# homopolymer/RAMBL

Measured on AMD Instinct MI355X. Metric: reads/sec into POA (150bp, ~1.5k-node graph), higher is better.
Workload: dtype f64

## Files before the change

rambl_amd/capi.py:

```python
import ctypes as C
import os

_HERE = os.path.dirname(os.path.abspath(__file__))
LIB_PATH = os.path.join(_HERE, "libstraincall_hip.so")

SC_OK = 0
ERRORS = {-1: "SC_ERR_NO_DEVICE", -2: "SC_ERR_HIP", -3: "SC_ERR_ARG", -4: "SC_ERR_UNSUPPORTED",
          -5: "SC_ERR_CAPACITY", -6: "SC_ERR_INTERNAL"}


class ScParams(C.Structure):
    _fields_ = [("error_rate", C.c_float), ("tau", C.c_float), ("diff_rate", C.c_float),
                ("sweeps_cap", C.c_int), ("draw_budget", C.c_int), ("max_candidates", C.c_int),
                ("graph_only", C.c_int), ("want_trace", C.c_int), ("want_timing", C.c_int), ("want_graph", C.c_int)]


class ScStats(C.Structure):
    _fields_ = [("graph_ms", C.c_double), ("cluster_ms", C.c_double), ("sampler_kernel_ms", C.c_double),
                ("sampler_launches", C.c_long), ("sampler_read_copies", C.c_long), ("level_launches", C.c_long), ("draws", C.c_long),
                ("slow_draws", C.c_long), ("exact_draws", C.c_long), ("sampler_strains", C.c_long), ("chain_passes", C.c_long), ("chain_cycles", C.c_long), ("chain_wall_ticks", C.c_long), ("level_kernel_ticks", C.c_long), ("sampler_level_ticks", C.c_long), ("xcd_levels", C.c_long * 8), ("msa_calls", C.c_long), ("n_nodes", C.c_int), ("n_levels", C.c_int),
                ("n_unique_reads", C.c_int), ("n_read_copies", C.c_long), ("setup_ms", C.c_double), ("queue_ms", C.c_double), ("place_ms", C.c_double), ("mailbox_ms", C.c_double), ("host_us", C.c_double * 3), ("wake_us", C.c_double * 2), ("kind_levels", C.c_long * 17)]

    def as_dict(self):
        return {k: (list(getattr(self, k)) if k in ("xcd_levels", "kind_levels", "host_us", "wake_us") else getattr(self, k)) for k, _ in self._fields_}


class ScAlignStats(C.Structure):
    _fields_ = [("upload_ms", C.c_double), ("score_ms", C.c_double), ("trace_ms", C.c_double), ("total_ms", C.c_double),
                ("score_cells", C.c_long), ("trace_cells", C.c_long), ("n_traced", C.c_long)]

    def as_dict(self):
        return {k: getattr(self, k) for k, _ in self._fields_}


class ScProfileStats(C.Structure):
    _fields_ = [("upload_ms", C.c_double), ("score_ms", C.c_double), ("trace_ms", C.c_double), ("total_ms", C.c_double),
                ("score_cells", C.c_long), ("trace_cells", C.c_long), ("n_tiles", C.c_long), ("n_candidates", C.c_long),
                ("n_traced", C.c_long), ("n_hits", C.c_long)]

    def as_dict(self):
        return {k: getattr(self, k) for k, _ in self._fields_}


class ScProfileSeedStats(C.Structure):
    _fields_ = ScProfileStats._fields_ + [("seed_k", C.c_int), ("n_gene_kmers", C.c_long), ("n_pairs", C.c_long),
                                          ("index_ms", C.c_double), ("lookup_ms", C.c_double)]

    def as_dict(self):
        return {k: getattr(self, k) for k, _ in self._fields_}


class ScProfileCountStats(C.Structure):
    _fields_ = ScProfileSeedStats._fields_ + [("n_rounds", C.c_int), ("n_stretches", C.c_int), ("n_reads_counted", C.c_long),
                                              ("select_ms", C.c_double), ("count_ms", C.c_double)]

    def as_dict(self):
        return {k: getattr(self, k) for k, _ in self._fields_}


class ScTaxaStats(C.Structure):
    _fields_ = [("upload_ms", C.c_double), ("words_ms", C.c_double), ("table_ms", C.c_double), ("score_ms", C.c_double), ("total_ms", C.c_double),
                ("n_seqs", C.c_long), ("n_words", C.c_long), ("n_genera", C.c_long), ("table_bytes", C.c_long)]

    def as_dict(self):
        return {k: getattr(self, k) for k, _ in self._fields_}


class StrainCallError(RuntimeError):
    def __init__(self, code, msg=""):
        super().__init__("%s (%d)%s" % (ERRORS.get(code, "error"), code, (": " + msg) if msg else ""))
        self.code = code


def load_library():
    if not os.path.exists(LIB_PATH):
        raise ImportError("%s is missing: build it with `python -c 'import __graft_entry__ as g; g.build()'` "
                          "(hipcc --offload-arch=gfx950). There is no CPU fallback for the StrainCall path." % LIB_PATH)
    lib = C.CDLL(LIB_PATH)
    vp, ip, cp = C.c_void_p, C.POINTER(C.c_int), C.c_char_p
    lib.sc_ctx_create.argtypes = [C.c_int, C.c_int, C.POINTER(vp)]
    lib.sc_ctx_destroy.argtypes = [vp]
    lib.sc_ctx_destroy.restype = None
    lib.sc_last_error.argtypes = [vp]
    lib.sc_last_error.restype = cp
    lib.sc_roi_error.argtypes = [vp, C.c_int]
    lib.sc_roi_error.restype = cp
    lib.sc_host_plan.argtypes = [C.c_int, C.c_int, C.c_double, ip]
    lib.sc_host_plan.restype = C.c_int
    lib.sc_host_bind.argtypes = [C.c_int]
    lib.sc_host_bind.restype = C.c_int
    lib.sc_roi_submit.argtypes = [vp, cp, C.c_int, ip, cp, ip, cp, ip, ip, ip, ip, C.c_int, C.POINTER(ScParams), ip]
    lib.sc_roi_wait.argtypes = [vp, C.c_int]
    lib.sc_roi_result.argtypes = [vp, C.c_int, C.c_char_p, C.c_long, ip, C.POINTER(C.c_double), C.c_int, ip]
    lib.sc_roi_graph_dump.argtypes = [vp, C.c_int, C.c_char_p, C.c_long, C.POINTER(C.c_long)]
    lib.sc_roi_trace.argtypes = [vp, C.c_int, C.c_char_p, C.c_long, C.POINTER(C.c_long)]
    lib.sc_roi_stats.argtypes = [vp, C.c_int, C.POINTER(ScStats)]
    lib.sc_roi_release.argtypes = [vp, C.c_int]
    lib.sc_roi_edge_support.argtypes = [vp, C.c_int, ip, C.c_int, ip]
    lib.sc_msa_align.argtypes = [vp, cp, ip, C.c_int, C.c_char_p, C.c_long, ip]
    lib.sc_roi_thread_tables.argtypes = [vp, C.c_int, ip, ip, C.c_int, ip, C.c_long, C.c_char_p, ip, C.POINTER(C.c_long)]
    lib.sc_roi_thread_edges.argtypes = [vp, C.c_int, ip, ip, ip, C.c_int, ip]
    lib.sc_edge_support_tables.argtypes = [vp, C.c_int, ip, ip, ip, C.POINTER(C.c_ubyte), C.c_int, ip, ip, C.c_int, ip]
    dp, up = C.POINTER(C.c_double), C.POINTER(C.c_uint)
    lib.sc_sample_level.argtypes = [vp, C.c_int, dp, C.c_int, dp, C.POINTER(C.c_ubyte), C.c_int, C.c_int, ip, ip, ip, ip, ip,
                                    C.c_int, dp, C.c_int, up, up, C.POINTER(C.c_long)]
    pi, pc, pu = C.POINTER(ip), C.POINTER(C.c_char_p), C.POINTER(C.c_ubyte)
    lib.sc_aln_open.argtypes = [cp, C.POINTER(vp)]
    lib.sc_aln_open_filtered.argtypes = [cp, C.POINTER(C.c_char_p), C.c_int, C.POINTER(vp)]
    lib.sc_aln_open_filtered.restype = C.c_int
    lib.sc_aln_close.argtypes = [vp]
    lib.sc_aln_close.restype = None
    lib.sc_aln_error.argtypes = [vp]
    lib.sc_aln_error.restype = cp
    lib.sc_aln_records.argtypes = [vp]
    lib.sc_aln_records.restype = C.c_long
    lib.sc_aln_ref_stats.argtypes = [vp, cp, C.POINTER(C.c_long), C.POINTER(C.c_long)]
    lib.sc_aln_ref_stats.restype = C.c_int
    lib.sc_aln_pileup_flags.argtypes = [vp, cp, C.c_int, C.c_int, C.c_int, pu, pu, pu]
    lib.sc_aln_load_reads.argtypes = [vp, cp, C.c_int, C.c_int, C.c_int, C.c_int, C.c_int, C.c_int, C.POINTER(vp)]
    lib.sc_reads_get.argtypes = [vp, ip, pi, pc, pi, pc, pi, pi, pi, pi, C.POINTER(C.c_long), ip]
    lib.sc_reads_free.argtypes = [vp]
    lib.sc_reads_free.restype = None
    lib.sc_aln_walk.argtypes = [vp, C.c_long, C.c_long, C.c_char_p, C.c_long, C.POINTER(C.c_long), C.POINTER(C.c_long)]
    lp = C.POINTER(C.c_long)
    lib.sc_align_reads.argtypes = [C.c_int, cp, lp, C.c_int, cp, cp, lp, C.c_int, ip, ip, ip, ip, ip, ip, up, C.c_int, ip,
                                   C.POINTER(ScAlignStats)]
    lib.sc_align_error.argtypes = []
    lib.sc_align_error.restype = cp
    lib.sc_profile_hits.argtypes = [C.c_int, cp, lp, C.c_int, cp, lp, C.c_int, C.c_double, C.c_double, C.c_double, C.c_double, ip, ip, ip,
                                    dp, ip, ip, ip, ip, ip, ip, dp, C.c_long, lp, C.POINTER(ScProfileStats)]
    lib.sc_profile_error.argtypes = []
    lib.sc_profile_error.restype = cp
    lib.sc_profile_hits_seeded.argtypes = lib.sc_profile_hits.argtypes[:-1] + [C.POINTER(ScProfileSeedStats)]
    lib.sc_profile_seed_length.argtypes = [ip, C.c_int, C.c_long, C.c_double, C.c_double, C.c_double, C.c_double, ip]
    lib.sc_profile_counts.argtypes = [C.c_int, cp, lp, C.c_int, cp, lp, C.c_int, ip, C.c_int, C.c_double, C.c_double, C.c_double, C.c_double,
                                      C.c_int, C.c_long, ip, ip, ip, lp, C.c_long, lp, C.POINTER(ScProfileCountStats)]
    lib.sc_profile_evalue6.argtypes = [C.c_int, C.c_long, C.c_int, C.c_double, C.c_double]
    lib.sc_profile_evalue6.restype = C.c_double
    u64, u64p = C.c_ulonglong, C.POINTER(C.c_ulonglong)
    lib.sc_taxa_train.argtypes = [C.c_int, cp, lp, C.c_int, ip, C.c_int, C.c_int, C.c_int, C.POINTER(vp), C.POINTER(ScTaxaStats)]
    lib.sc_taxa_classify.argtypes = [vp, cp, lp, C.c_int, u64p, u64, C.c_int, C.c_int, ip, ip, ip, C.POINTER(ScTaxaStats)]
    lib.sc_taxa_model_counts.argtypes = [vp, C.c_int, up, up]
    lib.sc_taxa_model_table.argtypes = [vp, C.c_int, ip]
    lib.sc_taxa_free.argtypes = [vp]
    lib.sc_taxa_free.restype = None
    lib.sc_taxa_error.argtypes = []
    lib.sc_taxa_error.restype = cp
    lib.sc_taxa_draw.argtypes = [u64, u64, C.c_int, C.c_int, C.c_int]
    lib.sc_taxa_draw.restype = C.c_long
    for f in ("sc_taxa_train", "sc_taxa_classify", "sc_taxa_model_counts", "sc_taxa_model_table"):
        getattr(lib, f).restype = C.c_int
    for f in ("sc_aln_open", "sc_aln_pileup_flags", "sc_aln_load_reads", "sc_reads_get", "sc_aln_walk", "sc_align_reads", "sc_profile_hits",
              "sc_profile_hits_seeded", "sc_profile_seed_length", "sc_profile_counts"):
        getattr(lib, f).restype = C.c_int
    for f in ("sc_ctx_create", "sc_roi_submit", "sc_roi_wait", "sc_roi_result", "sc_roi_graph_dump", "sc_roi_trace",
              "sc_roi_stats", "sc_roi_release", "sc_roi_edge_support", "sc_msa_align", "sc_roi_thread_tables", "sc_sample_level", "sc_roi_thread_edges", "sc_edge_support_tables"):
        getattr(lib, f).restype = C.c_int
    return lib


EXPORTS = ["sc_ctx_create", "sc_ctx_destroy", "sc_last_error", "sc_roi_error", "sc_host_plan", "sc_host_bind", "sc_roi_submit", "sc_roi_wait", "sc_roi_result",
           "sc_roi_graph_dump", "sc_roi_trace", "sc_roi_stats", "sc_roi_release", "sc_roi_edge_support", "sc_msa_align",
           "sc_roi_thread_tables", "sc_roi_thread_edges", "sc_edge_support_tables", "sc_sample_level", "sc_aln_open", "sc_aln_open_filtered", "sc_aln_close", "sc_aln_error", "sc_aln_records", "sc_aln_ref_stats", "sc_aln_pileup_flags",
           "sc_aln_load_reads", "sc_reads_get", "sc_reads_free", "sc_depth_scan", "sc_depth_scan_runs", "sc_aln_walk", "sc_align_reads",
           "sc_align_error", "sc_profile_hits", "sc_profile_error", "sc_profile_hits_seeded", "sc_profile_seed_length",
           "sc_profile_counts", "sc_taxa_train", "sc_taxa_classify", "sc_taxa_model_counts", "sc_taxa_model_table", "sc_taxa_free", "sc_taxa_error",
           "sc_taxa_draw"]


def default_params(error_rate=0.01, tau=0.02, diff_rate=0.01, graph_only=False, want_trace=False, want_timing=False, want_graph=False):
    return ScParams(error_rate, tau, diff_rate, 5000, 40000, 80, int(graph_only), int(want_trace), int(want_timing), int(want_graph))


def _pack(strings):
    off = (C.c_int * (len(strings) + 1))()
    n = 0
    for i, s in enumerate(strings):
        off[i] = n
        n += len(s)
    off[len(strings)] = n
    return "".join(strings).encode("ascii"), off


def host_bind(device=0):
    return int(lib().sc_host_bind(int(device)))


def host_plan(streams, local_world=0, cpus=0.0):
    out = (C.c_int * 3)()
    rc = lib().sc_host_plan(streams, local_world, cpus, out)
    if rc != SC_OK:
        raise StrainCallError(rc)
    return tuple(out)


_LIB = None


def lib():
    global _LIB
    if _LIB is None:
        _LIB = load_library()
    return _LIB


class NativeReads:

    def __init__(self, handle, gene_seq):
        self._h = handle
        self.gene_seq = gene_seq
        n, depth, n_in = C.c_int(), C.c_int(), C.c_long()
        ip = C.POINTER(C.c_int)
        self._pos, self._cig_off, self._seq_off, self._cn, self._mate_idx, self._mate_off = ip(), ip(), ip(), ip(), ip(), ip()
        self._cig, self._seq = C.c_char_p(), C.c_char_p()
        rc = lib().sc_reads_get(handle, C.byref(n), C.byref(self._pos), C.byref(self._cig), C.byref(self._cig_off), C.byref(self._seq),
                                C.byref(self._seq_off), C.byref(self._cn), C.byref(self._mate_idx), C.byref(self._mate_off),
                                C.byref(n_in), C.byref(depth))
        if rc != SC_OK:
            raise StrainCallError(rc)
        self.n = n.value
        self.n_input = n_in.value
        self.depth = depth.value

    def __len__(self):
        return self.n

    def __del__(self):
        if getattr(self, "_h", None):
            try:
                lib().sc_reads_free(self._h)
            except TypeError:
                pass
            self._h = None

    def _texts(self, text, off):
        raw = C.string_at(text, off[self.n]) if self.n else b""
        return [raw[off[i]:off[i + 1]].decode("ascii") for i in range(self.n)]

    def _view(self, name, build):
        cache = self.__dict__.setdefault("_views", {})
        if name not in cache:
            cache[name] = build()
        return cache[name]

    @property
    def pos(self):
        return self._view("pos", lambda: [self._pos[i] for i in range(self.n)])

    @property
    def copies(self):
        return self._view("copies", lambda: [self._cn[i] for i in range(self.n)])

    @property
    def cigar(self):
        return self._view("cigar", lambda: self._texts(self._cig, self._cig_off))

    @property
    def seq(self):
        return self._view("seq", lambda: self._texts(self._seq, self._seq_off))

    @property
    def mates(self):
        return self._view("mates", lambda: [[self._mate_idx[k] for k in range(self._mate_off[i], self._mate_off[i + 1])] for i in range(self.n)])


class NativeAln:

    def __init__(self, path, only=None):
        self.path = path
        self._h = C.c_void_p()
        if only is None:
            rc = lib().sc_aln_open(path.encode(), C.byref(self._h))
        else:
            names = (C.c_char_p * max(len(only), 1))(*[n.encode() for n in only])
            rc = lib().sc_aln_open_filtered(path.encode(), names, len(only), C.byref(self._h))
        if rc != SC_OK:
            msg = lib().sc_aln_error(self._h).decode() if self._h else "cannot open"
            self.close()
            raise StrainCallError(rc, "%s: %s" % (path, msg))

    def close(self):
        if getattr(self, "_h", None):
            try:
                lib().sc_aln_close(self._h)
            except TypeError:
                pass
            self._h = C.c_void_p()

    def __del__(self):
        self.close()

    def records(self):
        return lib().sc_aln_records(self._h)

    def walk(self, chunk=1 << 24):
        buf = C.create_string_buffer(chunk)
        first, n_out, used = 0, C.c_long(), C.c_long()
        while True:
            rc = lib().sc_aln_walk(self._h, first, 1 << 20, buf, len(buf), C.byref(n_out), C.byref(used))
            if rc == -5:
                buf = C.create_string_buffer(len(buf) * 4)
                continue
            if rc != SC_OK:
                raise StrainCallError(rc, self.path)
            if n_out.value == 0:
                return
            for line in buf.raw[:used.value].split(b"\n")[:-1]:
                q, f, seq, qual = line.split(b"\t")
                yield q, int(f), seq, qual
            first += n_out.value

    def ref_stats(self, gene):
        n, b = C.c_long(), C.c_long()
        lib().sc_aln_ref_stats(self._h, gene.encode(), C.byref(n), C.byref(b))
        return n.value, b.value

    def pileup_flags(self, mq, gene, P, Q):
        import numpy as np
        n = Q - P + 1
        if n <= 0:
            return {}
        cov, ins, dele = (np.zeros(n, dtype=np.uint8) for _ in range(3))
        pu = C.POINTER(C.c_ubyte)
        rc = lib().sc_aln_pileup_flags(self._h, gene.encode(), P, Q, mq, cov.ctypes.data_as(pu), ins.ctypes.data_as(pu),
                                       dele.ctypes.data_as(pu))
        if rc != SC_OK:
            raise StrainCallError(rc)
        idx = np.nonzero(cov)[0]
        return {int(k) + P: (bool(ins[k]), bool(dele[k])) for k in idx}

    def load_reads(self, gene_seq, gene, p0, p1, mq, rl, max_ins, max_depth):
        h = C.c_void_p()
        rc = lib().sc_aln_load_reads(self._h, gene.encode(), p0, p1, mq, rl, max_ins, max_depth, C.byref(h))
        if rc != SC_OK:
            raise StrainCallError(rc, lib().sc_aln_error(self._h).decode())
        return NativeReads(h, gene_seq)


class RegionResult:
    def __init__(self, seqs, abundance, graph, trace, stats):
        self.seqs = seqs
        self.abundance = abundance
        self.graph = graph
        self.trace = trace
        self.stats = stats


class Context:

    def __init__(self, device=0, streams=1):
        self.lib = load_library()
        self.h = C.c_void_p()
        rc = self.lib.sc_ctx_create(device, streams, C.byref(self.h))
        if rc != SC_OK:
            raise StrainCallError(rc, "no gfx950 HIP device %d (the StrainCall path has no CPU fallback)" % device)

    def close(self):
        if self.h:
            self.lib.sc_ctx_destroy(self.h)
            self.h = C.c_void_p()

    def __enter__(self):
        return self

    def __exit__(self, *a):
        self.close()

    def _err(self, rc):
        msg = self.lib.sc_last_error(self.h)
        return StrainCallError(rc, msg.decode("utf-8", "replace") if msg else "")

    def submit(self, region, params):
        n = len(region)
        if isinstance(region, NativeReads):
            ref = region.gene_seq.encode("ascii")
            handle = C.c_int()
            rc = self.lib.sc_roi_submit(self.h, ref, len(ref), region._pos, region._cig, region._cig_off, region._seq, region._seq_off,
                                        region._cn, region._mate_idx, region._mate_off, n, C.byref(params), C.byref(handle))
            if rc != SC_OK:
                raise self._err(rc)
            return handle.value
        pos = (C.c_int * max(n, 1))(*region.pos)
        cn = (C.c_int * max(n, 1))(*region.copies)
        cig, cig_off = _pack(region.cigar)
        seq, seq_off = _pack(region.seq)
        mate_off = (C.c_int * (n + 1))()
        flat = []
        for i, m in enumerate(region.mates):
            mate_off[i] = len(flat)
            flat.extend(m)
        mate_off[n] = len(flat)
        mate_idx = (C.c_int * max(len(flat), 1))(*flat)
        ref = region.gene_seq.encode("ascii")
        handle = C.c_int()
        rc = self.lib.sc_roi_submit(self.h, ref, len(ref), pos, cig, cig_off, seq, seq_off, cn, mate_idx, mate_off, n,
                                    C.byref(params), C.byref(handle))
        if rc != SC_OK:
            raise self._err(rc)
        return handle.value

    def wait(self, handle, want_graph=False, want_trace=False, release=True):
        rc = self.lib.sc_roi_wait(self.h, handle)
        graph = trace = None
        stats = ScStats()
        self.lib.sc_roi_stats(self.h, handle, C.byref(stats))
        if want_graph or rc != SC_OK:
            ln = C.c_long()
            self.lib.sc_roi_graph_dump(self.h, handle, None, 0, C.byref(ln))
            buf = C.create_string_buffer(ln.value + 1)
            if self.lib.sc_roi_graph_dump(self.h, handle, buf, ln.value, C.byref(ln)) == SC_OK:
                graph = buf.raw[:ln.value].decode("ascii")
        if rc != SC_OK:
            msg = self.lib.sc_roi_error(self.h, handle)
            err = StrainCallError(rc, msg.decode("utf-8", "replace") if msg else "")
            if release:
                self.lib.sc_roi_release(self.h, handle)
            err.graph = graph
            raise err
        nst = C.c_int()
        cap, maxs = 1 << 16, 256
        while True:
            buf = C.create_string_buffer(cap)
            off = (C.c_int * (maxs + 1))()
            ab = (C.c_double * maxs)()
            rc = self.lib.sc_roi_result(self.h, handle, buf, cap, off, ab, maxs, C.byref(nst))
            if rc == -5 and cap < (1 << 30):
                cap *= 8
                maxs *= 4
                continue
            break
        if rc != SC_OK:
            raise self._err(rc)
        seqs = [buf.raw[off[i]:off[i + 1]].decode("ascii") for i in range(nst.value)]
        abundance = [ab[i] for i in range(nst.value)]
        if want_trace:
            ln = C.c_long()
            self.lib.sc_roi_trace(self.h, handle, None, 0, C.byref(ln))
            tb = C.create_string_buffer(ln.value + 1)
            if self.lib.sc_roi_trace(self.h, handle, tb, ln.value, C.byref(ln)) == SC_OK:
                trace = tb.raw[:ln.value].decode("ascii")
        if release:
            self.lib.sc_roi_release(self.h, handle)
        return RegionResult(seqs, abundance, graph, trace, stats.as_dict())

    def run(self, region, params, want_graph=False, want_trace=False):
        return self.wait(self.submit(region, params), want_graph, want_trace)

    def edge_support(self, handle):
        n = C.c_int()
        self.lib.sc_roi_edge_support(self.h, handle, None, 0, C.byref(n))
        arr = (C.c_int * max(n.value, 1))()
        rc = self.lib.sc_roi_edge_support(self.h, handle, arr, n.value, C.byref(n))
        if rc != SC_OK:
            raise self._err(rc)
        return list(arr[:n.value])

    def thread_tables(self, handle):
        ncls, npool = C.c_int(), C.c_long()
        self.lib.sc_roi_thread_tables(self.h, handle, None, None, 0, None, 0, None, C.byref(ncls), C.byref(npool))
        cnt = (C.c_int * max(ncls.value, 1))()
        first = (C.c_int * max(ncls.value, 1))()
        pool = (C.c_int * max(npool.value, 1))()
        sym = C.create_string_buffer(8)
        rc = self.lib.sc_roi_thread_tables(self.h, handle, cnt, first, ncls.value, pool, npool.value, sym, C.byref(ncls),
                                           C.byref(npool))
        if rc != SC_OK:
            raise self._err(rc)
        return list(cnt[:ncls.value]), list(first[:ncls.value]), list(pool[:npool.value]), sym.raw

    def thread_edges(self, handle):
        ncls = C.c_int()
        self.lib.sc_roi_thread_edges(self.h, handle, None, None, None, 0, C.byref(ncls))
        n = ncls.value
        smin, emin, tmin = (C.c_int * max(n, 1))(), (C.c_int * max(n, 1))(), (C.c_int * max(8 * n, 1))()
        rc = self.lib.sc_roi_thread_edges(self.h, handle, smin, emin, tmin, n, C.byref(ncls))
        if rc != SC_OK:
            raise self._err(rc)
        return list(smin[:n]), list(emin[:n]), list(tmin[:8 * n])

    def edge_support_tables(self, pool_ptr, pool_rid, pool_cn, node_is_end, edge_src, edge_dst, sorted_pools):
        import numpy as np
        ptr_, rid, cn, src, dst = (np.ascontiguousarray(x, dtype=np.int32) for x in (pool_ptr, pool_rid, pool_cn, edge_src, edge_dst))
        end = np.ascontiguousarray(node_is_end, dtype=np.uint8)
        assert rid.shape == cn.shape and src.shape == dst.shape and ptr_.size == end.size + 1
        out = np.zeros(max(src.size, 1), dtype=np.int32)

        def ptr(x):
            return x.ctypes.data_as(C.POINTER(C.c_ubyte if x.dtype == np.uint8 else C.c_int))
        rc = self.lib.sc_edge_support_tables(self.h, end.size, ptr(ptr_), ptr(rid), ptr(cn), ptr(end), src.size, ptr(src), ptr(dst),
                                             int(sorted_pools), ptr(out))
        if rc != SC_OK:
            raise self._err(rc)
        return out[:src.size].tolist()

    def sample_level(self, a0, ll, has, ent_rid, ent_cn, ent_sym, mates, n_sweeps, U, e0=1):
        import numpy as np
        a0 = np.ascontiguousarray(a0, dtype=np.float64)
        ll = np.ascontiguousarray(ll, dtype=np.float64)
        S, n_reads = ll.shape
        assert a0.shape == (S,)
        has = np.ascontiguousarray(has, dtype=np.uint8)
        assert has.shape == (n_reads,)
        ent = [np.ascontiguousarray(x, dtype=np.int32) for x in (ent_rid, ent_cn, ent_sym)]
        assert ent[0].shape == ent[1].shape == ent[2].shape
        mate_off = np.zeros(n_reads + 1, dtype=np.int32)
        mate_off[1:] = np.cumsum([len(mates[r]) if r < len(mates) else 0 for r in range(n_reads)])
        mate_idx = np.array([m for r in range(min(len(mates), n_reads)) for m in mates[r]] or [0], dtype=np.int32)
        U = np.ascontiguousarray(U, dtype=np.float64)
        kdraw = np.zeros(S, dtype=np.uint32)
        cnt = np.zeros((S, 16), dtype=np.uint32)
        out = (C.c_long * 5)()

        def ptr(x, t):
            return x.ctypes.data_as(C.POINTER(t))
        rc = self.lib.sc_sample_level(self.h, S, ptr(a0, C.c_double), n_reads, ptr(ll, C.c_double), ptr(has, C.c_ubyte),
                                      len(ent[0]), e0, ptr(ent[0], C.c_int), ptr(ent[1], C.c_int), ptr(ent[2], C.c_int),
                                      ptr(mate_off, C.c_int), ptr(mate_idx, C.c_int), n_sweeps, ptr(U, C.c_double), len(U),
                                      ptr(kdraw, C.c_uint), ptr(cnt, C.c_uint), out)
        if rc != SC_OK:
            raise self._err(rc)
        return dict(kdraw=kdraw, cnt=cnt, n_draws=out[0], n_slow=out[1], n_exact=out[2], n_pass=out[3], kind=out[4])

    def msa_align(self, seqs):
        txt, off = _pack(seqs)
        cap = (len(txt) + 2) * max(len(seqs), 1) + 16
        out = C.create_string_buffer(cap)
        ncol = C.c_int()
        rc = self.lib.sc_msa_align(self.h, txt, off, len(seqs), out, cap, C.byref(ncol))
        if rc != SC_OK:
            raise self._err(rc)
        w = ncol.value + 1
        return [out.raw[i * w:i * w + ncol.value].decode("ascii") for i in range(len(seqs))]


class AlignResult:

    def __init__(self, as_, xs, seed, strand, pos, nm, cigar, stats):
        self.as_, self.xs, self.seed, self.strand, self.pos, self.nm, self.cigar, self.stats = as_, xs, seed, strand, pos, nm, cigar, stats


def align_reads(seeds, reads, quals=None, device=0):
    import numpy as np
    n = len(reads)
    sl = np.array([0] + [len(x) for x in seeds], dtype=np.int64).cumsum()
    rl = np.array([0] + [len(x) for x in reads], dtype=np.int64).cumsum()
    qtext = None
    if quals is not None:
        qtext = b"".join(q if (q != b"*" and len(q) == len(r)) else b"I" * len(r) for r, q in zip(reads, quals))
    stride = max([len(x) for x in reads] + [0]) // 2 + 4
    as_, xs, seed, strand, pos, nm, ncig = (np.zeros(max(n, 1), dtype=np.int32) for _ in range(7))
    cig = np.zeros(max(n, 1) * stride, dtype=np.uint32)
    st = ScAlignStats()
    ip, lp, up = C.POINTER(C.c_int), C.POINTER(C.c_long), C.POINTER(C.c_uint)
    rc = lib().sc_align_reads(device, b"".join(seeds), sl.ctypes.data_as(lp), len(seeds), b"".join(reads), qtext, rl.ctypes.data_as(lp), n,
                              as_.ctypes.data_as(ip), xs.ctypes.data_as(ip), seed.ctypes.data_as(ip), strand.ctypes.data_as(ip),
                              pos.ctypes.data_as(ip), nm.ctypes.data_as(ip), cig.ctypes.data_as(up), stride, ncig.ctypes.data_as(ip),
                              C.byref(st))
    if rc != SC_OK:
        raise StrainCallError(rc, lib().sc_align_error().decode())
    cigars = []
    for r in range(n):
        ops = cig[r * stride:r * stride + ncig[r]]
        cigars.append("".join("%d%s" % (int(v) >> 4, "MIDNSHP=X"[int(v) & 15]) for v in ops) if ncig[r] else "*")
    return AlignResult(as_[:n], xs[:n], seed[:n], strand[:n], pos[:n], nm[:n], cigars, st)


class ProfileHits:
    FIELDS = ("seg", "gene", "strand", "score", "identity", "align_len", "qfrom", "qto", "hfrom", "hto", "evalue")

    def __init__(self, arrays, stats):
        for k, v in zip(self.FIELDS, arrays):
            setattr(self, k, v)
        self.stats = stats

    def __len__(self):
        return len(self.seg)


def _profile_call(gtext, gl, n_genes, segs, thresholds, device, cap, seeded=False):
    import numpy as np
    n = len(segs)
    sl = np.array([0] + [len(x) for x in segs], dtype=np.int64).cumsum()
    stext = b"".join(segs)
    ip, lp, dp = C.POINTER(C.c_int), C.POINTER(C.c_long), C.POINTER(C.c_double)
    while True:
        ints = [np.zeros(max(cap, 1), dtype=np.int32) for _ in range(9)]
        score, ev = np.zeros(max(cap, 1), dtype=np.float64), np.zeros(max(cap, 1), dtype=np.float64)
        st, nh = (ScProfileSeedStats if seeded else ScProfileStats)(), C.c_long()
        iptr = [a.ctypes.data_as(ip) for a in ints]
        rc = (lib().sc_profile_hits_seeded if seeded else lib().sc_profile_hits)(device, gtext, gl.ctypes.data_as(lp), n_genes, stext, sl.ctypes.data_as(lp), n, *thresholds, iptr[0],
                                   iptr[1], iptr[2], score.ctypes.data_as(dp), iptr[3], iptr[4], iptr[5], iptr[6], iptr[7], iptr[8],
                                   ev.ctypes.data_as(dp), cap, C.byref(nh), C.byref(st))
        if rc == -5 and nh.value > cap:
            cap = nh.value
            continue
        if rc != SC_OK:
            raise StrainCallError(rc, lib().sc_profile_error().decode())
        k = nh.value
        seg, gene, strand, identity, align_len, qfrom, qto, hfrom, hto = (a[:k] for a in ints)
        return [seg, gene, strand, score[:k], identity, align_len, qfrom, qto, hfrom, hto, ev[:k]], st


def profile_seed_length(seg_lens, gene_bases, min_identity=95.0, max_evalue=1e-10, ka_lambda=1.28, ka_k=0.46, lossless=False):
    import numpy as np
    lens = np.ascontiguousarray(seg_lens, dtype=np.int32)
    raw = C.c_int()
    k = lib().sc_profile_seed_length(lens.ctypes.data_as(C.POINTER(C.c_int)), len(lens), int(gene_bases), float(min_identity), float(max_evalue),
                                     float(ka_lambda), float(ka_k), C.byref(raw))
    if k < 0:
        raise StrainCallError(k)
    return (raw.value or None) if lossless else k


def profile_hits(genes, segs, min_identity=95.0, max_evalue=1e-10, ka_lambda=1.28, ka_k=0.46, device=0, cap=None, seeded=False):
    import numpy as np
    gl = np.array([0] + [len(x) for x in genes], dtype=np.int64).cumsum()
    gtext = b"".join(genes)
    thresholds = (float(min_identity), float(max_evalue), float(ka_lambda), float(ka_k))
    step = max(1, (1 << 30) // (2 * max(len(genes), 1)))
    parts, total, seed_ks = [], (ScProfileSeedStats if seeded else ScProfileStats)(), []
    for a in range(0, max(len(segs), 1), step):
        chunk = segs[a:a + step]
        arrays, st = _profile_call(gtext, gl, len(genes), chunk, thresholds, device, max(1 << 16, 4 * len(chunk)) if cap is None else int(cap),
                                   seeded)
        arrays[0] = arrays[0] + a
        parts.append(arrays)
        for k, _ in total._fields_:
            setattr(total, k, getattr(total, k) + getattr(st, k))
        if seeded:
            seed_ks.append(st.seed_k)
    if seeded:
        total.seed_k = min(seed_ks)
    return ProfileHits([np.concatenate([p[f] for p in parts]) for f in range(11)], total)


class ProfileCounts:

    def __init__(self, triples, stats):
        self.triples = triples
        self.stats = stats

    def __len__(self):
        return len(self.triples)


def profile_evalue6(seg_len, gene_bases, score2, ka_lambda=1.28, ka_k=0.46):
    return float(lib().sc_profile_evalue6(int(seg_len), int(gene_bases), int(score2), float(ka_lambda), float(ka_k)))


def profile_counts(genes, segs, seg_read, min_identity=95.0, max_evalue=1e-10, ka_lambda=1.28, ka_k=0.46, device=0, cap=None, seeded=False,
                   cand_room=0):
    import numpy as np
    gl = np.array([0] + [len(x) for x in genes], dtype=np.int64).cumsum()
    sl = np.array([0] + [len(x) for x in segs], dtype=np.int64).cumsum()
    gtext, stext = b"".join(genes), b"".join(segs)
    reads = np.ascontiguousarray(seg_read, dtype=np.int32)
    if len(reads) != len(segs):
        raise ValueError("%d read indices for %d segments" % (len(reads), len(segs)))
    n_reads = int(reads.max()) + 1 if len(reads) else 0
    ip, lp = C.POINTER(C.c_int), C.POINTER(C.c_long)
    cap = 1 << 16 if cap is None else int(cap)
    while True:
        gene, times, share = (np.zeros(max(cap, 1), dtype=np.int32) for _ in range(3))
        n_behind = np.zeros(max(cap, 1), dtype=np.int64)
        st, n = ScProfileCountStats(), C.c_long()
        rc = lib().sc_profile_counts(device, gtext, gl.ctypes.data_as(lp), len(genes), stext, sl.ctypes.data_as(lp), len(segs),
                                     reads.ctypes.data_as(ip), n_reads, float(min_identity), float(max_evalue), float(ka_lambda), float(ka_k),
                                     int(bool(seeded)), int(cand_room), gene.ctypes.data_as(ip), times.ctypes.data_as(ip),
                                     share.ctypes.data_as(ip), n_behind.ctypes.data_as(lp), cap, C.byref(n), C.byref(st))
        if rc == -5 and n.value > cap:
            cap = n.value
            continue
        if rc != SC_OK:
            raise StrainCallError(rc, lib().sc_profile_error().decode())
        k = n.value
        return ProfileCounts([(int(gene[i]), int(times[i]), int(share[i]), int(n_behind[i])) for i in range(k)], st)


TAXA_WORDS = 65536
TAXA_TRIALS = 100


def taxa_draw(seed, key, trial, draw, n_words):
    return int(lib().sc_taxa_draw(int(seed), int(key), int(trial), int(draw), int(n_words)))


def _pack_long(seqs):
    import numpy as np
    return b"".join(seqs), np.array([0] + [len(x) for x in seqs], dtype=np.int64).cumsum()


class TaxaModel:

    def __init__(self, seqs, genus, n_genera, device=0, grid_cap=0, keep_counts=False):
        import numpy as np
        if len(genus) != len(seqs):
            raise ValueError("%d genus indices for %d sequences" % (len(genus), len(seqs)))
        text, off = _pack_long(seqs)
        gi = np.ascontiguousarray(genus, dtype=np.int32)
        self.n_genera = int(n_genera)
        self._h = C.c_void_p()
        self.stats = ScTaxaStats()
        rc = lib().sc_taxa_train(int(device), text, off.ctypes.data_as(C.POINTER(C.c_long)), len(seqs), gi.ctypes.data_as(C.POINTER(C.c_int)),
                                 self.n_genera, int(grid_cap), int(bool(keep_counts)), C.byref(self._h), C.byref(self.stats))
        if rc != SC_OK:
            raise StrainCallError(rc, lib().sc_taxa_error().decode())

    def close(self):
        if getattr(self, "_h", None):
            try:
                lib().sc_taxa_free(self._h)
            except TypeError:
                pass
            self._h = C.c_void_p()

    def __del__(self):
        self.close()

    def __enter__(self):
        return self

    def __exit__(self, *a):
        self.close()

    def classify(self, queries, keys, seed=0, n_trials=TAXA_TRIALS, grid_cap=0):
        import numpy as np
        n = len(queries)
        if len(keys) != n:
            raise ValueError("%d keys for %d queries" % (len(keys), n))
        text, off = _pack_long(queries)
        key = np.ascontiguousarray(keys, dtype=np.uint64)
        best, words = np.zeros(max(n, 1), dtype=np.int32), np.zeros(max(n, 1), dtype=np.int32)
        winner = np.zeros((max(n, 1), max(int(n_trials), 1)), dtype=np.int32)
        st = ScTaxaStats()
        ip = C.POINTER(C.c_int)
        rc = lib().sc_taxa_classify(self._h, text, off.ctypes.data_as(C.POINTER(C.c_long)), n, key.ctypes.data_as(C.POINTER(C.c_ulonglong)),
                                    int(seed), int(n_trials), int(grid_cap), best.ctypes.data_as(ip), winner.ctypes.data_as(ip),
                                    words.ctypes.data_as(ip), C.byref(st))
        if rc != SC_OK:
            raise StrainCallError(rc, lib().sc_taxa_error().decode())
        return best[:n], winner[:n], words[:n], st

    def counts(self, genus):
        import numpy as np
        m, n = np.zeros(TAXA_WORDS, dtype=np.uint32), np.zeros(TAXA_WORDS, dtype=np.uint32)
        up = C.POINTER(C.c_uint)
        rc = lib().sc_taxa_model_counts(self._h, int(genus), m.ctypes.data_as(up), n.ctypes.data_as(up))
        if rc != SC_OK:
            raise StrainCallError(rc, lib().sc_taxa_error().decode())
        return m, n

    def table(self, genus):
        import numpy as np
        q = np.zeros(TAXA_WORDS, dtype=np.int32)
        rc = lib().sc_taxa_model_table(self._h, int(genus), q.ctypes.data_as(C.POINTER(C.c_int)))
        if rc != SC_OK:
            raise StrainCallError(rc, lib().sc_taxa_error().decode())
        return q
```

rambl_amd/csrc/sc_api.cpp:

```cpp
#include <malloc.h>

#include <cmath>

#include "sc_ctx.hpp"

using namespace sc;
struct sc_ctx { Ctx c; sc_ctx(int device, const CtxPlan& plan) : c(device, plan) {} };

extern "C" {

int sc_host_plan(int stream_count, int local_world, double cpus, int* out) {
    if (!out || stream_count < 1) return SC_ERR_ARG;
    host_plan(stream_count, local_world > 0 ? local_world : local_world_size(), cpus > 0 ? cpus : cpu_budget_host(), out);
    return SC_OK;
}

int sc_ctx_create(int device, int stream_count, sc_ctx** out) {
    if (!out) return SC_ERR_ARG;
    *out = nullptr;
    setenv("GPU_MAX_HW_QUEUES", "16", 0);
    int ndev = 0;
    if (hipGetDeviceCount(&ndev) != hipSuccess || ndev <= 0 || device < 0 || device >= ndev) return SC_ERR_NO_DEVICE;
    hipDeviceProp_t prop;
    if (hipGetDeviceProperties(&prop, device) != hipSuccess) return SC_ERR_NO_DEVICE;
    if (std::strncmp(prop.gcnArchName, "gfx950", 6) != 0) return SC_ERR_NO_DEVICE;
    if (hipSetDevice(device) != hipSuccess) return SC_ERR_HIP;
    if (init_kernels() != 0) return SC_ERR_HIP;
    const Options opt = read_options();
    struct Near {
        cpu_set_t before; bool moved = false;
        Near(int dev, bool bind) {
            cpu_set_t local;
            if (bind && sched_getaffinity(0, sizeof before, &before) == 0 && sc::gpu_local_cpus(dev, &local)) moved = sched_setaffinity(0, sizeof local, &local) == 0;
        }
        ~Near() { if (moved) (void)sched_setaffinity(0, sizeof before, &before); }
    } near{device, !opt.off(opt.numa_bind)};
    {
        static std::once_flag once;
        std::call_once(once, [&opt] {
            if (opt.off(opt.malloc_tune)) return;
            mallopt(M_MMAP_THRESHOLD, 32 << 20);
            mallopt(M_TRIM_THRESHOLD, 1 << 30);
            mallopt(M_TOP_PAD, 64 << 20);
        });
    }
    try {
        *out = new sc_ctx(device, plan_context(opt, stream_count, prop.multiProcessorCount, cpu_budget_host(), local_world_size()));
    } catch (const std::exception&) {
        return SC_ERR_HIP;
    }
    return SC_OK;
}

void sc_ctx_destroy(sc_ctx* h) { delete h; }

const char* sc_last_error(sc_ctx* h) {
    if (!h) return "";
    std::lock_guard<std::mutex> lk(h->c.mu);
    static thread_local std::string copy;
    copy = h->c.last_error;
    return copy.c_str();
}

const char* sc_roi_error(sc_ctx* h, int handle) {
    if (!h) return "";
    std::lock_guard<std::mutex> lk(h->c.mu);
    auto it = h->c.jobs.find(handle);
    return (it == h->c.jobs.end() || it->second->status != 1) ? "" : it->second->err.c_str();
}

int sc_roi_submit(sc_ctx* h, const char* ref_bases, int ref_len, const int* read_pos, const char* cigar_text,
                  const int* cigar_off, const char* seq_text, const int* seq_off, const int* read_copies,
                  const int* mate_idx, const int* mate_off, int n_reads, const sc_params* params, int* handle_out) {
    if (!h || !ref_bases || ref_len < 0 || n_reads < 0 || !params || !handle_out) return SC_ERR_ARG;
    if (n_reads > 0 && (!read_pos || !cigar_text || !cigar_off || !seq_text || !seq_off || !read_copies || !mate_off)) return SC_ERR_ARG;
    if (params->draw_budget < 1 || params->draw_budget > MAX_DRAWS || params->sweeps_cap < 0 || params->max_candidates < 1 ||
        params->max_candidates > MAXS)
        return SC_ERR_ARG;
    if (n_reads > 0 && (cigar_off[0] < 0 || seq_off[0] < 0 || mate_off[0] != 0)) return SC_ERR_ARG;
    for (int i = 0; i < n_reads; i++)
        if (read_copies[i] < 1 || cigar_off[i + 1] < cigar_off[i] || seq_off[i + 1] < seq_off[i] || mate_off[i + 1] < mate_off[i])
            return SC_ERR_ARG;
    auto job = std::make_shared<Job>();
    job->t_submit = now_ms();
    job->ref.assign(ref_bases, (size_t)ref_len);
    job->reads.resize((size_t)n_reads);
    for (int i = 0; i < n_reads; i++) {
        if (read_pos[i] < 0 || read_pos[i] > ref_len) return SC_ERR_ARG;
        job->reads[i].pos = read_pos[i];
        job->reads[i].cigar.assign(cigar_text + cigar_off[i], (size_t)(cigar_off[i + 1] - cigar_off[i]));
        job->reads[i].seq.assign(seq_text + seq_off[i], (size_t)(seq_off[i + 1] - seq_off[i]));
        job->reads[i].cn = read_copies[i];
    }
    job->mate_off.assign(mate_off ? mate_off : nullptr, mate_off ? mate_off + n_reads + 1 : nullptr);
    if (job->mate_off.empty()) job->mate_off.assign(1, 0);
    const int nm = job->mate_off.back();
    if (nm > 0 && !mate_idx) return SC_ERR_ARG;
    job->mate_idx.assign(mate_idx, mate_idx + nm);
    for (int v : job->mate_idx) if (v < -1 || v >= n_reads) return SC_ERR_ARG;
    job->params = *params;
    Ctx* ctx = &h->c;
    Worker* wake = nullptr;
    {
        std::lock_guard<std::mutex> lk(ctx->mu);
        job->handle = ctx->next_handle++;
        ctx->jobs[job->handle] = job;
        ctx->queue.push_back(job);
        ctx->regions_active.fetch_add(1, std::memory_order_acq_rel);
        *handle_out = job->handle;
        if (!ctx->idle.empty()) { wake = ctx->idle.back(); ctx->idle.pop_back(); }
    }
    if (wake) ctx->pool->make_ready(wake->fib);
    return SC_OK;
}

static std::shared_ptr<Job> find_job(sc_ctx* h, int handle) {
    std::lock_guard<std::mutex> lk(h->c.mu);
    auto it = h->c.jobs.find(handle);
    return it == h->c.jobs.end() ? nullptr : it->second;
}

int sc_roi_wait(sc_ctx* h, int handle) {
    if (!h) return SC_ERR_ARG;
    auto job = find_job(h, handle);
    if (!job) return SC_ERR_ARG;
    std::unique_lock<std::mutex> lk(h->c.mu);
    h->c.cv_done.wait(lk, [&] { return job->status == 1; });
    if (job->rc != SC_OK) h->c.last_error = job->err;
    return job->rc;
}

int sc_roi_result(sc_ctx* h, int handle, char* seq_buf, long seq_cap, int* seq_off, double* abundance, int max_strains,
                  int* n_strains) {
    if (!h || !n_strains) return SC_ERR_ARG;
    auto job = find_job(h, handle);
    if (!job || job->status != 1) return SC_ERR_ARG;
    if (job->rc != SC_OK) return job->rc;
    const int n = (int)job->seqs.size();
    *n_strains = n;
    long tot = 0;
    for (auto& s : job->seqs) tot += (long)s.size();
    if (n > max_strains || tot > seq_cap || !seq_buf || !seq_off || !abundance) return SC_ERR_CAPACITY;
    long o = 0;
    for (int i = 0; i < n; i++) {
        seq_off[i] = (int)o;
        std::memcpy(seq_buf + o, job->seqs[i].data(), job->seqs[i].size());
        o += (long)job->seqs[i].size();
        abundance[i] = job->abund[i];
    }
    seq_off[n] = (int)o;
    return SC_OK;
}

static int copy_text(const std::string& s, char* buf, long cap, long* len_out) {
    if (len_out) *len_out = (long)s.size();
    if (!buf || cap < (long)s.size()) return SC_ERR_CAPACITY;
    std::memcpy(buf, s.data(), s.size());
    return SC_OK;
}
int sc_roi_graph_dump(sc_ctx* h, int handle, char* buf, long cap, long* len_out) {
    if (!h) return SC_ERR_ARG;
    auto job = find_job(h, handle);
    if (!job || job->status != 1) return SC_ERR_ARG;
    if (job->rc != SC_OK && job->graph_dump.empty()) return job->rc;
    return copy_text(job->graph_dump, buf, cap, len_out);
}
int sc_roi_trace(sc_ctx* h, int handle, char* buf, long cap, long* len_out) {
    if (!h) return SC_ERR_ARG;
    auto job = find_job(h, handle);
    if (!job || job->status != 1) return SC_ERR_ARG;
    if (job->rc != SC_OK) return job->rc;
    return copy_text(job->trace, buf, cap, len_out);
}
int sc_roi_stats(sc_ctx* h, int handle, sc_stats* out) {
    if (!h || !out) return SC_ERR_ARG;
    auto job = find_job(h, handle);
    if (!job || job->status != 1) return SC_ERR_ARG;
    *out = job->stats;
    return SC_OK;
}
int sc_roi_edge_support(sc_ctx* h, int handle, int* support, int cap, int* n_edges) {
    if (!h || !n_edges) return SC_ERR_ARG;
    auto job = find_job(h, handle);
    if (!job || job->status != 1) return SC_ERR_ARG;
    if (job->rc != SC_OK) return job->rc;
    *n_edges = (int)job->edge_support.size();
    if (!support || cap < *n_edges) return SC_ERR_CAPACITY;
    std::memcpy(support, job->edge_support.data(), sizeof(int) * job->edge_support.size());
    return SC_OK;
}
int sc_roi_thread_tables(sc_ctx* h, int handle, int* count, int* first_read, int cls_cap, int* pool, long pool_cap,
                         char* symbols, int* n_cls, long* n_pool) {
    if (!h || !n_cls || !n_pool) return SC_ERR_ARG;
    auto job = find_job(h, handle);
    if (!job || job->status != 1) return SC_ERR_ARG;
    *n_cls = (int)job->thr_count.size();
    *n_pool = (long)job->thr_pool.size();
    if (!count || !first_read || !pool || !symbols || cls_cap < *n_cls || pool_cap < *n_pool) return SC_ERR_CAPACITY;
    std::memcpy(count, job->thr_count.data(), sizeof(int) * job->thr_count.size());
    std::memcpy(first_read, job->thr_first.data(), sizeof(int) * job->thr_first.size());
    std::memcpy(pool, job->thr_pool.data(), sizeof(int) * job->thr_pool.size());
    std::memset(symbols, 0, 8);
    std::memcpy(symbols, job->thr_sym.data(), std::min<size_t>(8, job->thr_sym.size()));
    return SC_OK;
}
int sc_roi_thread_edges(sc_ctx* h, int handle, int* smin, int* emin, int* tmin, int cls_cap, int* n_cls) {
    if (!h || !n_cls) return SC_ERR_ARG;
    auto job = find_job(h, handle);
    if (!job || job->status != 1) return SC_ERR_ARG;
    *n_cls = (int)job->thr_smin.size();
    if (!smin || !emin || !tmin || cls_cap < *n_cls) return SC_ERR_CAPACITY;
    std::memcpy(smin, job->thr_smin.data(), sizeof(int) * job->thr_smin.size());
    std::memcpy(emin, job->thr_emin.data(), sizeof(int) * job->thr_emin.size());
    std::memcpy(tmin, job->thr_tmin.data(), sizeof(int) * job->thr_tmin.size());
    return SC_OK;
}
int sc_edge_support_tables(sc_ctx* h, int n_nodes, const int* pool_ptr, const int* pool_rid, const int* pool_cn,
                           const unsigned char* node_is_end, int n_edges, const int* edge_src, const int* edge_dst, int sorted,
                           int* support_out) {
    if (!h || n_nodes < 1 || n_edges < 0 || !pool_ptr || !node_is_end || (sorted != 0 && sorted != 1)) return SC_ERR_ARG;
    if (n_edges > 0 && (!edge_src || !edge_dst || !support_out)) return SC_ERR_ARG;
    if (pool_ptr[0] != 0) return SC_ERR_ARG;
    for (int a = 0; a < n_nodes; a++) if (pool_ptr[a + 1] < pool_ptr[a]) return SC_ERR_ARG;
    const int np = pool_ptr[n_nodes];
    if (np > 0 && (!pool_rid || !pool_cn)) return SC_ERR_ARG;
    for (int e = 0; e < n_edges; e++)
        if (edge_src[e] < 0 || edge_src[e] >= n_nodes || edge_dst[e] < 0 || edge_dst[e] >= n_nodes) return SC_ERR_ARG;
    if (sorted)
        for (int a = 0; a < n_nodes; a++)
            for (int x = pool_ptr[a] + 1; x < pool_ptr[a + 1]; x++) if (pool_rid[x] < pool_rid[x - 1]) return SC_ERR_ARG;
    if (n_edges == 0) return SC_OK;
    Ctx* ctx = &h->c;
    try {
        Worker w;
        w.init_private(ctx);
        const hipStream_t st = w.st;
        const std::vector<int> pptr(pool_ptr, pool_ptr + n_nodes + 1), prid(pool_rid, pool_rid + np), pcn(pool_cn, pool_cn + np);
        const std::vector<int> esrc(edge_src, edge_src + n_edges), edst(edge_dst, edge_dst + n_edges);
        const std::vector<uint8_t> isend(node_is_end, node_is_end + n_nodes);
        DevBuf b_ptr, b_rid, b_cn, b_end, b_src, b_dst, b_sup;
        const int* d_ptr = upload(w.passthrough, b_ptr, pptr, st);
        const int* d_rid = upload(w.passthrough, b_rid, prid, st);
        const int* d_cn = upload(w.passthrough, b_cn, pcn, st);
        const uint8_t* d_end = upload(w.passthrough, b_end, isend, st);
        const int* d_src = upload(w.passthrough, b_src, esrc, st);
        const int* d_dst = upload(w.passthrough, b_dst, edst, st);
        int* d_sup = (int*)b_sup.ensure(sizeof(int) * (size_t)n_edges);
        launch_edge_support(st, nullptr, d_dst, d_ptr, d_rid, d_cn, d_end, d_src, n_edges, sorted, d_sup);
        HIPCHK(hipGetLastError());
        HIPCHK(hipMemcpyAsync(support_out, d_sup, sizeof(int) * (size_t)n_edges, hipMemcpyDeviceToHost, st));
        HIPCHK(hipStreamSynchronize(st));
        return SC_OK;
    } catch (const ScError& ex) { std::lock_guard<std::mutex> lk(ctx->mu); ctx->last_error = ex.what(); return ex.code; }
    catch (const std::exception& ex) { std::lock_guard<std::mutex> lk(ctx->mu); ctx->last_error = ex.what(); return SC_ERR_HIP; }
}
int sc_sample_level(sc_ctx* h, int S, const double* a0, int n_reads, const double* ll, const unsigned char* has, int n_ent,
                    int e0, const int* ent_rid, const int* ent_cn, const int* ent_sym, const int* mate_off, const int* mate_idx,
                    int n_sweeps, const double* U, int n_u, unsigned* kdraw, unsigned* cnt, long* out) {
    if (!h || !a0 || !ll || !has || !ent_rid || !ent_cn || !ent_sym || !mate_off || !U || !kdraw || !cnt || !out) return SC_ERR_ARG;
    Ctx* ctx = &h->c;
    if (ctx->resident || ctx->workers.size() != 1) return SC_ERR_ARG;
    if (S < 2 || S > MAXS || n_reads < 1 || n_ent < 1 || e0 < 0 || e0 > (1 << 20) || n_sweeps < 1) return SC_ERR_ARG;
    for (int s = 0; s < S; s++) if (!(a0[s] >= 0.0) || !std::isfinite(a0[s])) return SC_ERR_ARG;
    long Q = 0;
    for (int r = 0; r < n_ent; r++) {
        const bool sym_ok = (ent_sym[r] >= 0 && ent_sym[r] < KMAX) || ent_sym[r] == 0xFF;
        if (ent_rid[r] < 0 || ent_rid[r] >= n_reads || ent_cn[r] < 1 || !sym_ok) return SC_ERR_ARG;
        Q += ent_cn[r];
    }
    if (Q * n_sweeps > MAX_DRAWS || n_u < Q * n_sweeps) return SC_ERR_ARG;
    for (long t = 0; t < Q * n_sweeps; t++) if (!(U[t] >= 0.0 && U[t] <= 1.0)) return SC_ERR_ARG;
    if (mate_off[0] != 0) return SC_ERR_ARG;
    for (int r = 0; r < n_reads; r++) if (mate_off[r + 1] < mate_off[r]) return SC_ERR_ARG;
    const int nm = mate_off[n_reads];
    if (nm > 0 && !mate_idx) return SC_ERR_ARG;
    for (int i = 0; i < nm; i++) if (mate_idx[i] < -1 || mate_idx[i] >= n_reads) return SC_ERR_ARG;
    try {
        Worker w;
        w.init_private(ctx);
        const int E = e0 + n_ent;
        FlatGraph f;
        f.K = KMAX; f.code_N = KMAX;
        f.ent_rid.resize((size_t)E); f.ent_cn.assign((size_t)E, 1); f.ent_lab_off.resize((size_t)E); f.ent_lab_len.assign((size_t)E, 1);
        f.ent_first.assign((size_t)E, 1);
        f.labels.assign((size_t)E + 1, 0);
        std::vector<int> qoff((size_t)E, 0);
        for (int e = 0; e < E; e++) {
            const int r = e - e0;
            f.ent_rid[(size_t)e] = r >= 0 ? ent_rid[r] : n_reads - 1 - e % n_reads;
            f.ent_lab_off[(size_t)e] = e;
            f.labels[(size_t)e] = (uint8_t)(r >= 0 ? ent_sym[r] : 0);
        }
        for (int r = 0, q = 0; r < n_ent; r++) { f.ent_cn[(size_t)(e0 + r)] = ent_cn[r]; qoff[(size_t)(e0 + r)] = q; q += ent_cn[r]; }
        const hipStream_t st = w.st;
        const std::vector<int> mptr(mate_off, mate_off + n_reads + 1), midx(mate_idx, mate_idx + nm);
        JobDev jd = w.job_dev(w.passthrough, f, qoff, mptr, midx, n_reads, std::max<long>(Q, 1), n_ent, Q * n_sweeps);
        auto slot = [](int s) { return (s * 37 + 5) % MAXS; };
        std::vector<double> rows((size_t)jd.ll_stride * MAXS, 0.0);
        for (int s = 0; s < S; s++) std::memcpy(&rows[(size_t)slot(s) * jd.ll_stride], ll + (size_t)s * n_reads, sizeof(double) * n_reads);
        jd.ll = upload(w.passthrough, w.b_ll, rows, st);
        std::vector<uint8_t> hv(has, has + n_reads);
        hv.resize((size_t)n_reads + 8, 0);
        jd.has = upload(w.passthrough, w.b_has, hv, st);
        std::vector<double> u(U, U + Q * n_sweeps);
        u.resize((size_t)(Q * n_sweeps + 2048), 0.5);
        std::vector<float> uf(u.begin(), u.end());
        DevBuf b_u, b_uf;
        jd.U = upload(w.passthrough, b_u, u, st);
        jd.Uf = upload(w.passthrough, b_uf, uf, st);
        const JobDev* jd_dev = (const JobDev*)w.b_jobdev.ensure(sizeof(JobDev));
        HIPCHK(hipMemcpyAsync((void*)jd_dev, &jd, sizeof jd, hipMemcpyHostToDevice, st));

        LevelParams& P = *w.Ph;
        for (int s = 0; s < S; s++) P.sp[s] = StrainParam{slot(s), E, 1, 0, a0[s], 0.0};
        LevelHdr H{};
        H.mode = MODE_SAMPLE; H.S = S; H.e0 = e0; H.e1 = E; H.Q = (int)Q; H.n_sweeps = n_sweeps;
        H.n_copy = 0; H.do_update = 0; H.seq = 1;
        std::memset(w.Rh, 0, sizeof(LevelResult));
        LevelBatch batch;
        batch.it[0] = w.level_item(jd_dev, H, KMAX);
        const int kind = item_kind(batch.it[0].kind);
        launch_level_batch(st, kind, batch, 1);
        HIPCHK(hipGetLastError());
        HIPCHK(hipStreamSynchronize(st));
        const LevelResult& R = *w.Rh;
        if (R.seq != 1u || R.error) throw ScError(SC_ERR_INTERNAL, "the sampler level did not complete");
        for (int s = 0; s < S; s++) kdraw[s] = R.kdraw[s];
        std::memcpy(cnt, R.cnt, sizeof(unsigned) * (size_t)S * KMAX);
        out[0] = (long)R.n_draws; out[1] = (long)R.n_slow; out[2] = (long)R.n_exact; out[3] = (long)R.n_pass; out[4] = kind;
        return SC_OK;
    } catch (const ScError& ex) { std::lock_guard<std::mutex> lk(ctx->mu); ctx->last_error = ex.what(); return ex.code; }
    catch (const std::exception& ex) { std::lock_guard<std::mutex> lk(ctx->mu); ctx->last_error = ex.what(); return SC_ERR_HIP; }
}
int sc_roi_release(sc_ctx* h, int handle) {
    if (!h) return SC_ERR_ARG;
    std::lock_guard<std::mutex> lk(h->c.mu);
    auto it = h->c.jobs.find(handle);
    if (it == h->c.jobs.end() || it->second->status != 1) return SC_ERR_ARG;
    h->c.jobs.erase(it);
    return SC_OK;
}

int sc_msa_align(sc_ctx* h, const char* seq_text, const int* seq_off, int n, char* rows_out, long cap, int* ncol_out) {
    if (!h || !seq_text || !seq_off || n < 1 || !ncol_out) return SC_ERR_ARG;
    Ctx* ctx = &h->c;
    try {
        Worker w;
        w.init_private(ctx);
        std::vector<std::string> seqs((size_t)n), rows;
        for (int i = 0; i < n; i++) seqs[i].assign(seq_text + seq_off[i], (size_t)(seq_off[i + 1] - seq_off[i]));
        int ncol;
        if (n == 1) { ncol = (int)seqs[0].size(); rows = seqs; }
        else ncol = w.msa_device(seqs, rows);
        *ncol_out = ncol;
        int rc = SC_OK;
        if (!rows_out || (long)n * (ncol + 1) > cap) rc = SC_ERR_CAPACITY;
        else for (int i = 0; i < n; i++) { std::memcpy(rows_out + (long)i * (ncol + 1), rows[i].data(), (size_t)ncol); rows_out[(long)i * (ncol + 1) + ncol] = 0; }
        return rc;
    } catch (const ScError& ex) { std::lock_guard<std::mutex> lk(ctx->mu); ctx->last_error = ex.what(); return ex.code; }
    catch (const std::exception& ex) { std::lock_guard<std::mutex> lk(ctx->mu); ctx->last_error = ex.what(); return SC_ERR_HIP; }
}

}
```

rambl_amd/csrc/sc_ctx.hpp:

```cpp
#pragma once
#include <atomic>
#include <condition_variable>
#include <deque>
#include <map>
#include <memory>
#include <mutex>
#include <thread>

#include "../../include/straincall_hip.h"
#include "sc_device.hpp"
#include "sc_fiber.hpp"
#include "sc_graph.hpp"
#include "sc_host.hpp"
#include "sc_plan.hpp"

namespace sc {

void launch_edge_support(hipStream_t st, const int* out_ptr, const int* out_node, const int* pool_ptr, const int* pool_rid,
                         const int* pool_cn, const uint8_t* node_is_end, const int* edge_src, int n_edges, int sorted,
                         int* support);
void launch_msa(hipStream_t st, const MsaDev& d);
void launch_thread(hipStream_t st, const ThreadDev& d, int* pool_sorted);
int init_graph_kernels();
bool level_wants_grid(const JobDev& job, const LevelHdr& h);
int launch_level_grid(hipStream_t st, const JobDev& job, const LevelHdr& h, const LevelParams* Pd, LevelResult* R);
int level_kind(const LevelHdr& h);
int level_lds_kb(const LevelHdr& h, int K);
int level_table_capacity();
void launch_level_batch(hipStream_t st, int kind, const LevelBatch& b, int n);
void launch_level_any(hipStream_t st, const LevelBatch& b, int n);
void launch_resident(hipStream_t st, const ResidentArgs& a, int slots);
int init_level_kernels();
inline int init_kernels() { return init_level_kernels() | init_graph_kernels(); }

struct Job {
    int handle = 0;
    std::string ref;
    std::vector<AlignedRead> reads;
    std::vector<int> mate_off, mate_idx;
    sc_params params{};
    std::vector<std::string> seqs;
    std::vector<double> abund;
    std::string graph_dump, trace;
    std::vector<int> edge_support;
    std::vector<int> thr_count, thr_first, thr_pool;
    std::vector<int> thr_smin, thr_emin, thr_tmin;
    std::string thr_sym;
    sc_stats stats{};
    double t_submit = 0;
    int status = 0;
    int rc = SC_OK;
    std::string err;
};

typedef long double ld;

struct Ctx;
struct Worker;
struct ArenaPool {
    explicit ArenaPool(int limit) : limit(limit) {}
    PinnedArena* lease(PinnedArena* passthrough);
    void release(PinnedArena* a);
private:
    const int limit;
    std::mutex mu;
    std::vector<std::unique_ptr<PinnedArena>> arenas;
    std::vector<PinnedArena*> free_arenas;
};
struct SetupGate {
    SetupGate(int limit, bool split_exec, const std::unique_ptr<FiberPool>& pool) : split_exec(split_exec), limit(limit), pool(pool) {}
    void enter(Worker* w);
    void leave();
    const bool split_exec;
private:
    const int limit;
    const std::unique_ptr<FiberPool>& pool;
    std::mutex mu;
    int setups = 0;
    std::deque<Worker*> waiters;
};
struct LevelRequest { Worker* w; LevelItem item; int kind; bool timed; };
struct LevelServer {
    LevelServer(int device, int n_streams, bool sweep_log);
    ~LevelServer();
    void submit(const LevelRequest& rq);
private:
    struct LaunchStream { Stream s; int busy = 0; int unretired = 0; };
    struct Flying { Worker* w; int stream; };
    void serve();
    const int device;
    const bool sweep_log;
    std::vector<LaunchStream> lstreams;
    sc::SpinLock plk;
    std::deque<LevelRequest> pending;
    std::atomic<int> n_pending{0};
    std::mutex dmu;
    std::condition_variable dcv;
    std::atomic<bool> asleep{false};
    std::atomic<bool> stop{false};
    std::thread thread;
};
struct ResidentGrid {
    ResidentGrid(Ctx& ctx, int slots, bool watch_stamps, int n_workers);
    ~ResidentGrid();
    void ensure(int m);
    void idle();
    void shutdown();
    int acquire_mailbox(Worker* w);
    void release_mailbox(int m);
    bool poll_stamps();
    void poll_health();
    const int slots;
    HostMapped<Mailbox> mail;
    std::vector<unsigned> mail_seq, mail_done;
    const std::unique_ptr<StampWatch> watch;
private:
    enum { GEN_STOPPED = 0, GEN_RUNNING = 1, GEN_STOPPING = 2 };
    Ctx& ctx;
    Stream rstream;
    HostMapped<ResidentCtl> ctl;
    std::mutex mmu;
    std::vector<int> free_mail;
    std::deque<Worker*> mail_waiters;
    std::mutex gen_mu;
    std::atomic<int> gen_state{GEN_STOPPED};
    std::thread heart;
    std::atomic<bool> heart_stop{false};
};
struct ServerLog {
    double t_created = 0; int n_fast = 0, n_long = 0;
    std::atomic<long> wake_hist[24] = {};
};

struct Uniforms {
    DevMem<double> d; DevMem<float> f;
    explicit Uniforms(const std::vector<double>& u) : d(u), f(std::vector<float>(u.begin(), u.end())) {}
};
struct Ctx {
    Ctx(int device, const CtxPlan& plan);
    ~Ctx();
    const int device;
    const CtxPlan plan;
    const bool resident;
    const Uniforms U;
    ArenaPool arenas;
    std::vector<Stream> setup_streams;
    std::unique_ptr<Stream> launch;
    HostMapped<LevelParams> P_all;
    HostMapped<LevelResult> R_all;
    DevMem<LevelParams> Pd_all;
    std::string last_error;
    std::mutex mu;
    std::condition_variable cv_done;
    std::deque<std::shared_ptr<Job>> queue;
    std::map<int, std::shared_ptr<Job>> jobs;
    int next_handle = 1;
    bool stop = false;
    std::atomic<int> regions_active{0};
    std::vector<std::unique_ptr<Worker>> workers;
    std::vector<Worker*> idle;
    std::atomic<int> fibers_left{0};
    std::unique_ptr<ResidentGrid> grid;
    std::unique_ptr<FiberPool> pool;
    std::unique_ptr<LevelServer> server;
    SetupGate gate;
    std::unique_ptr<ServerLog> log;
};

struct Worker {
    Ctx* ctx = nullptr;
    ResidentGrid* grid = nullptr;
    Fiber* fib = nullptr;
    int slot = 0;
    hipStream_t st = nullptr;
    bool own_stream = false;
    hipEvent_t sync_ev = nullptr;
    std::atomic<int> level_state{0};
    std::string level_err;
    double t_seen = 0, wake_acc[2] = {0, 0};
    std::atomic<int> mslot{-1};
    std::atomic<double> t_posted{0};
    double t_batch_launched = 0;
    int batch_n = 0;
    hipEvent_t ev0 = nullptr, ev1 = nullptr;
    std::vector<hipEvent_t> ev_pool;
    size_t ev_used = 0;
    LevelParams* Ph = nullptr;
    LevelParams* Pm = nullptr;
    LevelParams* Pd = nullptr;
    LevelResult* Rh = nullptr;
    LevelResult* Rd = nullptr;
    bool own_blocks = false;
    unsigned seq = 0;
    DevBuf b_ent_rid, b_ent_cn, b_ent_lab_off, b_ent_lab_len, b_ent_first, b_ent_qoff, b_labels, b_mate_ptr, b_mate_idx,
        b_ll, b_has, b_isnew, b_tabA, b_tabLf, b_qcode, b_qent, b_quid, b_dlog, b_out_ptr, b_out_node, b_pool_ptr, b_pool_rid,
        b_pool_cn, b_isend, b_esrc, b_support, b_jobdev;
    DevBuf m_seqs, m_off, m_cols0, m_cols1, m_counts, m_moves, m_trace, m_out, m_edge;
    PinnedArena* stage = nullptr;
    PinnedArena passthrough;
    DevBuf t_ref, t_pos, t_seqoff, t_seq, t_cigoff, t_cigop, t_ciglen, t_lut, t_tabs, t_pool, t_pool2;
    FlatGraph flat;
    std::vector<int> ent_qoff_buf;
    bool setup_held = false;
    std::vector<ld> cnt_scratch;

    ~Worker();
    void init();
    void init_private(Ctx* c);
    void run();
    void process(Job& job);
    void complete_level(const LevelItem& it, bool timed);
    void wait_level();
    void finish_level(int state, const char* err = nullptr);
    void sync_stream();
    int msa_device(const std::vector<std::string>& seqs, std::vector<std::string>& rows);
    void thread_device(const std::string& G, const std::vector<AlignedRead>& R, const std::vector<std::vector<CigarOp>>& cig,
                       ThreadTables& T);
    JobDev job_dev(PinnedArena& ar, const FlatGraph& f, const std::vector<int>& ent_qoff, const std::vector<int>& mate_off,
                   const std::vector<int>& mate_idx, int n_reads, long qcap, int max_entries, long max_draws);
    LevelItem level_item(const JobDev* job, const LevelHdr& H, int K) const {
        return LevelItem{job, H, pack_kind(level_kind(H), level_lds_kb(H, K)), Pm, Rd};
    }
    void cluster(Job& job, const PoGraph& g, FlatGraph& f);
};
inline int level_sweeps(const sc_params& pa, long Q) { return (int)std::min<long>(pa.sweeps_cap, pa.draw_budget / std::max<long>(Q, 1)); }
struct MailHold {
    Worker* w;
    void drop() { const int m = w->mslot.load(std::memory_order_relaxed); if (m >= 0) { w->mslot.store(-1, std::memory_order_release); w->grid->release_mailbox(m); } }
    ~MailHold() { drop(); }
};

void walk_levels(Worker& w, Job& job, const FlatGraph& f, const JobDev& jd, const JobDev* jd_dev, const std::vector<int>& level_hi,
                 int final_e0, long total_copies, MailHold& mail);
bool gpu_local_cpus(int device, cpu_set_t* out);

}
```

rambl_amd/csrc/sc_device.hpp:

```cpp
#pragma once
#include <hip/hip_runtime.h>

#include <cstdint>
#include <type_traits>

namespace sc {

constexpr int MAXS = 128;
constexpr int KMAX = 16;
constexpr int KK = KMAX * KMAX;
constexpr int MAX_DRAWS = 40000;

enum LevelMode { MODE_HARD = 0, MODE_SAMPLE = 1 };

struct JobDev {
    const int* ent_rid;
    const int* ent_cn;
    const int* ent_lab_off;
    const int* ent_lab_len;
    const uint8_t* ent_first;
    const int* ent_qoff;
    const uint8_t* labels;
    const int* mate_ptr;
    const int* mate_idx;
    int n_reads;
    int K;
    int code_N;
    double* ll;
    long ll_stride;
    uint8_t* has;
    const double* U;
    const float* Uf;
    uint8_t* isnew;
    double* tabA;
    float* tabLf;
    uint8_t* qcode;
    int* qent;
    int* quid;
    long qcap;
    uint8_t* dlog;
    long dlog_cap;
};

struct LevelHdr {
    int mode;
    int S;
    int e0, e1;
    int has_dups;
    int any_multi;
    int Q;
    int n_sweeps;
    int n_copy;
    int do_update;
    int done;
    int copy_n;
    unsigned seq;
};
struct StrainParam {
    int slot;
    int lab_off, lab_len;
    int pad;
    double a0;
    double logpri;
};
struct LevelParams {
    int copy_src[MAXS], copy_dst[MAXS];
    StrainParam sp[MAXS];
    double lpt[MAXS * KK];
};

constexpr int N_SAMPLER_KINDS = 16;
__host__ __device__ constexpr int sampler_kind(int nb, bool rows_lds) { return 2 * nb - 1 + (rows_lds ? 1 : 0); }
__host__ __device__ constexpr bool kind_has_sampler(int kind) { return kind != 0; }
__host__ __device__ constexpr int kind_nb(int kind) { return (kind + 1) / 2; }
__host__ __device__ constexpr bool kind_rows_lds(int kind) { return kind % 2 == 0; }
__host__ __device__ constexpr int pack_kind(int kind, int lds_kb) { return kind | (lds_kb << 8); }
__host__ __device__ constexpr int item_kind(int word) { return word & 0xFF; }
__host__ __device__ constexpr int item_lds_kb(int word) { return (word >> 8) & 0xFFFF; }
static_assert(sampler_kind(1, false) == 1 && sampler_kind(8, true) == N_SAMPLER_KINDS && kind_nb(sampler_kind(5, true)) == 5 &&
              kind_rows_lds(sampler_kind(5, true)) && !kind_rows_lds(sampler_kind(5, false)) &&
              item_kind(pack_kind(13, 157)) == 13 && item_lds_kb(pack_kind(13, 157)) == 157, "level kind");
template <int NB = 1, class F>
__host__ __device__ __forceinline__ void with_sampler_variant(int kind, F&& f) {
    if constexpr (NB < 8) {
        if (kind_nb(kind) != NB) { with_sampler_variant<NB + 1>(kind, f); return; }
    }
    if (kind_rows_lds(kind)) f(std::integral_constant<int, NB>{}, std::true_type{});
    else f(std::integral_constant<int, NB>{}, std::false_type{});
}

struct LevelResult;
struct LevelItem {
    const JobDev* job;
    LevelHdr h;
    int kind;
    const LevelParams* P;
    LevelResult* R;
};
constexpr int MAXB = 48;
struct LevelBatch { LevelItem it[MAXB]; };
static_assert(sizeof(LevelItem) == 80 && sizeof(LevelBatch) <= 4096, "kernel-argument segment");

struct alignas(128) Mailbox {
    LevelItem item;
    unsigned seq;
    unsigned ack;
    unsigned state;
    unsigned levels;
    unsigned pad[8];
};
static_assert(sizeof(Mailbox) == 128, "one mailbox per 128 bytes");
struct ResidentCtl {
    unsigned stop;
    unsigned heartbeat;
    unsigned pad[30];
};
struct ResidentArgs {
    Mailbox* mail;
    const ResidentCtl* ctl;
    unsigned long long idle_ticks;
    const LevelParams* P_base;
    LevelResult* R_base;
    int n_blocks;
};

struct LevelResult {
    double abund[MAXS];
    double subst[MAXS * KK];
    unsigned cnt[MAXS * KMAX];
    unsigned kdraw[MAXS];
    unsigned long long n_draws;
    unsigned long long n_slow;
    unsigned long long n_pass;
    unsigned long long chain_cycles, chain_wall;
    unsigned long long n_exact;
    unsigned long long level_wall;
    unsigned phase_ticks[6];
    int error;
    int xcc;
    unsigned seq;
};

struct ThreadDev {
    const char* ref; int glen;
    int n_reads;
    const int* pos; const int* seq_off; const char* seq;
    const int* cig_off; const char* cig_op; const int* cig_len;
    const uint8_t* lut;
    int* count; int* minrid;
    int* tmin;
    int* smin; int* emin;
    int* off; int* cursor;
    int* pool;
    int* err;
    int* big;
};

struct MsaDev {
    const char* seqs;
    const int* seq_off;
    int n;
    int cmax;
    char* cols[2];
    int* counts;
    uint8_t* moves;
    int mv_stride;
    int* edge;
    int* trace;
    int* ncol_out;
    int* err_out;
};

}
```

rambl_amd/csrc/sc_level.hip:

```cpp
#include <hip/hip_runtime.h>
#include <math.h>
#include <stdint.h>
#include <stdlib.h>

#include <type_traits>

#include "sc_device.hpp"
#include "sc_sampler.hpp"

namespace sc {

constexpr int LDS_TOTAL = 160 * 1024 - 256;
constexpr int LDS_SMALL = 18 * 1024;
constexpr int LDS_BIG = LDS_TOTAL - LDS_SMALL;
static_assert(LDS_SMALL >= (int)(sizeof(double) * 2 * MAXS + sizeof(StrainParam) * MAXS + sizeof(unsigned) * MAXS * KMAX + sizeof(int) * 6 * MAXS + 64), "LDS_SMALL");
static_assert(LDS_BIG >= (int)(sizeof(double) * MAXS * 64), "LDS_BIG");

enum { LV_COPIES_DONE = 1, LV_ITEMS_DONE = 2, LV_HAS_DONE = 4, LV_HARD_DONE = 8 };
typedef const __attribute__((address_space(4))) JobDev KJob;

__device__ __forceinline__ void stage_params(const LevelHdr& h, const LevelParams* __restrict__ P, StrainParam* s_sp, int* s_copy,
                                             double* s_lpt, bool want_lpt, int K2, int tid, int nt) {
    const i4v* src_sp = reinterpret_cast<const i4v*>(P->sp);
    i4v* dst_sp = reinterpret_cast<i4v*>(s_sp);
    for (int i = tid; i < h.S * 2; i += nt) dst_sp[i] = src_sp[i];
    for (int i = tid; i < h.n_copy; i += nt) { s_copy[i] = P->copy_src[i]; s_copy[MAXS + i] = P->copy_dst[i]; }
    if (want_lpt) {
        const double2* s = reinterpret_cast<const double2*>(P->lpt);
        double2* d = reinterpret_cast<double2*>(s_lpt);
        for (int i = tid; i < (h.S * K2 + 1) / 2; i += nt) d[i] = s[i];
    }
}

template <class JD>
__device__ __forceinline__ void phase_copies(const JD& job, const LevelHdr& h, const int* s_copy, int tid, int nt) {
    const long stride = job.ll_stride;
    for (int c = 0; c < ((h.done & LV_COPIES_DONE) ? 0 : h.n_copy); c++) {
        const double2* src = reinterpret_cast<const double2*>(job.ll + (long)s_copy[c] * stride);
        double2* dst = reinterpret_cast<double2*>(job.ll + (long)s_copy[MAXS + c] * stride);
        const int n2 = ((h.copy_n < job.n_reads ? h.copy_n : job.n_reads) + 1) >> 1;
        int i = tid;
        for (; i + 3 * nt < n2; i += 4 * nt) {
            const double2 v0 = src[i], v1 = src[i + nt], v2 = src[i + 2 * nt], v3 = src[i + 3 * nt];
            dst[i] = v0; dst[i + nt] = v1; dst[i + 2 * nt] = v2; dst[i + 3 * nt] = v3;
        }
        for (; i < n2; i += nt) dst[i] = src[i];
    }
    __syncthreads();
}


template <class JD>
__device__ __forceinline__ void mark_present(const JD& job, const LevelHdr& h, int first, int step) {
    const int e0 = h.e0, Rn = h.e1 - h.e0;
    for (int r = first; r < Rn; r += step) job.has[job.ent_rid[e0 + r]] = 1;
}

template <class JD>
__device__ __forceinline__ void phase_update(const JD& job, const LevelHdr& h, const StrainParam* s_sp, const int* s_lab,
                                             const double* s_lpt, int tid, int nt) {
    const int S = h.S, K = job.K, K2 = K * K, e0 = h.e0, Rn = h.e1 - h.e0;
    const long stride = job.ll_stride;
    const bool plain_labels = !h.has_dups && !h.any_multi && !(h.done & LV_ITEMS_DONE);
    if (!plain_labels && !(h.done & LV_ITEMS_DONE)) {
        for (int r = tid; r < Rn; r += nt) {
            const int e = e0 + r;
            job.isnew[r] = (job.ent_first[e] && !job.has[job.ent_rid[e]]) ? 1 : 0;
        }
        __syncthreads();
    }
    const int codeN = job.code_N;
    auto item = [&](int s, int r) {
        const int e = e0 + r;
        const int rid = job.ent_rid[e];
        const uint8_t* sb = job.labels + s_sp[s].lab_off;
        const uint8_t* rb = job.labels + job.ent_lab_off[e];
        const int ls = s_sp[s].lab_len, lr = job.ent_lab_len[e];
        const double* lp = s_lpt + s * K2;
        double val;
        if (ls == 1) {
            int a = sb[0], b = rb[0];
            if (lr == 1) {
                if (a == codeN) a = b;
                val = (a < K && b < K) ? lp[a * K + b] : __longlong_as_double(0x7ff8000000000000ll);
            } else {
                val = (a < 6 && a != codeN) ? -INFINITY : __longlong_as_double(0x7ff8000000000000ll);
            }
        } else {
            val = 0.0;
            if (job.isnew[r]) {
                int ii = ls, jj = lr;
                while (ii > 0 && jj > 0) {
                    int a = sb[--ii], b = rb[--jj];
                    if (a == codeN) a = b;
                    val += lp[a * K + b];
                }
            } else {
                int ii = 0, jj = 0;
                while (ii < ls && jj < lr) {
                    int a = sb[ii++], b = rb[jj++];
                    if (a == codeN) a = b;
                    val += lp[a * K + b];
                }
            }
        }
        double* cell = job.ll + (long)s_sp[s].slot * stride + rid;
        const bool fresh = job.ent_first[e] && !job.has[rid];
        *cell = fresh ? val : (*cell + val);
    };
    if (h.done & LV_ITEMS_DONE) {
    } else if (!h.has_dups && !h.any_multi) {
        constexpr int U = 16;
        const double qnan = __longlong_as_double(0x7ff8000000000000ll);
        const int nch = (S + U - 1) / U;
        const int items = Rn * nch;
        for (int idx = tid; idx < items; idx += nt) {
            const int ch = idx / Rn, r = idx - ch * Rn;
            const int e = e0 + r;
            const int rid = job.ent_rid[e];
            const int b = job.labels[job.ent_lab_off[e]];
            const bool fresh = job.ent_first[e] && !job.has[rid];
            if (ch == 0) job.isnew[r] = fresh ? 1 : 0;
            const int s0 = ch * U;
            long off[U];
            double old[U];
#pragma unroll
            for (int k = 0; k < U; k++) {
                const int sx = (s0 + k < S) ? s0 + k : S - 1;
                off[k] = (long)s_sp[sx].slot * stride + rid;
                old[k] = fresh ? 0.0 : job.ll[off[k]];
            }
#pragma unroll
            for (int k = 0; k < U; k++) {
                const int sx = s0 + k;
                if (sx < S) {
                    int a = s_lab[sx];
                    if (a == codeN) a = b;
                    const double val = (a < K && b < K) ? s_lpt[sx * K2 + a * K + b] : qnan;
                    job.ll[off[k]] = fresh ? val : (old[k] + val);
                }
            }
        }
    } else if (!h.has_dups) {
        const long total = (long)S * Rn;
        for (long idx = tid; idx < total; idx += nt) item((int)(idx / Rn), (int)(idx % Rn));
    } else {
        if (tid < S) for (int r = 0; r < Rn; r++) item(tid, r);
    }
    if (h.done & LV_HAS_DONE) { __syncthreads(); return; }
    __syncthreads();
    mark_present(job, h, tid, nt);
    __syncthreads();
}

template <bool BARRIER = true, class JD>
__device__ __forceinline__ void phase_slots(const JD& job, const LevelHdr& h, int tid, int nt) {
    const int e0 = h.e0, Rn = h.e1 - h.e0;
    for (int r = tid; r < Rn; r += nt) {
        const int e = e0 + r;
        const int rid = job.ent_rid[e], cn = job.ent_cn[e];
        const int qb = job.ent_qoff[e];
        const int mb = job.mate_ptr[rid], mn = job.mate_ptr[rid + 1] - mb;
        const uint8_t code = (job.ent_lab_len[e] == 1) ? job.labels[job.ent_lab_off[e]] : (uint8_t)0xFF;
        for (int i = 0; i < cn; i++) {
            const int k = cn - 1 - i;
            const int uid = (k < mn) ? job.mate_idx[mb + k] : -1;
            job.qent[qb + i] = r;
            job.quid[qb + i] = uid;
            job.qcode[qb + i] = code;
        }
    }
    if (BARRIER) __syncthreads();
}

__device__ __forceinline__ void finish_level(const LevelHdr& h, LevelResult* __restrict__ R, unsigned long long wall0, int tid) {
    __threadfence_system();
    __syncthreads();
    if (tid == 0) {
        R->level_wall = wall_clock64() - wall0;
        R->xcc = (int)(__builtin_amdgcn_s_getreg(20 | (3 << 11)) & 0xF);
        __hip_atomic_store(&R->seq, h.seq, __ATOMIC_RELEASE, __HIP_MEMORY_SCOPE_SYSTEM);
    }
}


template <class JD>
__device__ __forceinline__ void zero_unseen_mates(const JD& job, const LevelHdr& h, const StrainParam* sp, int first, int step) {
    const long stride = job.ll_stride;
    for (int q = first; q < h.Q; q += step) {
        const int uid = job.quid[q];
        if (uid >= 0 && !job.has[uid])
            for (int s = 0; s < h.S; s++) job.ll[(long)sp[s].slot * stride + uid] = 0.0;
    }
}

__device__ __forceinline__ void normalise_column(double* col, long cs, int S, double m) {
    double norm = 0;
    for (int s = 0; s < S; s++) norm += exp(col[(long)s * cs] - m);
    for (int s = 0; s < S; s++) {
        double* cell = col + (long)s * cs;
        *cell = exp(*cell - m) / norm;
    }
}

__device__ __forceinline__ void strain_sums(const double* prow, const uint8_t* qcode, int Q, int lane, double (&acc)[KMAX + 1]) {
#pragma unroll
    for (int b = 0; b <= KMAX; b++) acc[b] = 0.0;
    for (int q = lane; q < Q; q += 64) {
        const double p = prow[q];
        const int code = qcode[q];
        acc[KMAX] += p;
#pragma unroll
        for (int b = 0; b < KMAX; b++) acc[b] += (code == b) ? p : 0.0;
    }
#pragma unroll
    for (int b = 0; b <= KMAX; b++) {
        double v = acc[b];
        for (int off = 32; off > 0; off >>= 1) v += __shfl_down(v, off);
        acc[b] = v;
    }
}

struct LevelLds {
    double* s_a; double* s_p; unsigned* s_cnt; int* s_slot; unsigned* s_kf; float* s_a0f; int* s_x; int* s_copy; int* s_lab;
    StrainParam* s_sp; unsigned char* s_big;
};
__device__ __forceinline__ LevelLds level_lds(unsigned char* raw) {
    LevelLds l;
    l.s_a = reinterpret_cast<double*>(raw);
    l.s_p = l.s_a + MAXS;
    l.s_sp = reinterpret_cast<StrainParam*>(l.s_p + MAXS);
    l.s_cnt = reinterpret_cast<unsigned*>(l.s_sp + MAXS);
    l.s_slot = reinterpret_cast<int*>(l.s_cnt + MAXS * KMAX);
    l.s_kf = reinterpret_cast<unsigned*>(l.s_slot + MAXS);
    l.s_a0f = reinterpret_cast<float*>(l.s_kf + MAXS);
    l.s_copy = reinterpret_cast<int*>(l.s_a0f + MAXS);
    l.s_lab = l.s_copy + 2 * MAXS;
    l.s_x = l.s_lab + MAXS;
    l.s_big = raw + LDS_SMALL;
    return l;
}

constexpr int CHAINW_ROWS_BYTES = LDS_BIG - UWIN * 4;
constexpr int CHAIN_THREADS = 512;
template <class IT>
__device__ __forceinline__ LevelHdr load_hdr(const IT& it) {
    LevelHdr h;
    h.mode = it.h.mode; h.S = it.h.S; h.e0 = it.h.e0; h.e1 = it.h.e1; h.has_dups = it.h.has_dups; h.any_multi = it.h.any_multi;
    h.Q = it.h.Q; h.n_sweeps = it.h.n_sweeps; h.n_copy = it.h.n_copy; h.do_update = it.h.do_update; h.done = it.h.done;
    h.copy_n = it.h.copy_n; h.seq = it.h.seq;
    return h;
}
template <class IT>
__device__ __forceinline__ LevelHdr begin_level(const IT& it, const LevelLds& l, unsigned long long wall0, int tid, int nt) {
    const LevelHdr h = load_hdr(it);
    KJob& job = *(KJob*)it.job;
    LevelResult* __restrict__ R = it.R;
    const bool upd = h.do_update && h.e1 > h.e0;
    stage_params(h, it.P, l.s_sp, l.s_copy, reinterpret_cast<double*>(l.s_big), upd && !(h.done & LV_ITEMS_DONE), job.K * job.K, tid, nt);
    if (tid == 0) { R->error = 0; R->n_draws = 0; R->n_exact = 0; R->n_slow = 0; R->n_pass = 0; R->chain_cycles = 0; R->chain_wall = 0; }
    __syncthreads();
    if (tid == 0) R->phase_ticks[0] = (unsigned)(wall_clock64() - wall0);
    return h;
}
template <int NB, bool ROWS_LDS, bool STAY, class IT>
__device__ __forceinline__ void level_sample_body(const IT& it, unsigned char* s_raw) {
    const unsigned long long wall0 = wall_clock64();
    KJob& job = *(KJob*)it.job;
    LevelResult* __restrict__ R = it.R;
    const LevelLds l = level_lds(s_raw);
    float* s_uwin = reinterpret_cast<float*>(l.s_big);
    float* s_rows = s_uwin + UWIN;
    const int tid = threadIdx.x;
    int nt = blockDim.x;
    const LevelHdr h = begin_level(it, l, wall0, tid, nt);
    const int S = h.S, Q = h.Q, e0 = h.e0, Rn = h.e1 - h.e0;
    const int stride = chain_w_stride(S);
    const bool upd = h.do_update && Rn > 0;
    for (int i = tid; i < MAXS * KMAX; i += nt) l.s_cnt[i] = 0;
    if (tid < MAXS) {
        l.s_slot[tid] = tid < S ? l.s_sp[tid].slot : 0;
        l.s_kf[tid] = 0u;
        l.s_a0f[tid] = tid < S ? (float)l.s_sp[tid].a0 : 0.0f;
        l.s_lab[tid] = tid < S ? (int)job.labels[l.s_sp[tid].lab_off] : 0;
    }
    phase_copies(job, h, l.s_copy, tid, nt);
    if (tid == 0) R->phase_ticks[1] = (unsigned)(wall_clock64() - wall0);
    if (upd) {
        phase_slots<false>(job, h, tid, nt);
        phase_update(job, h, l.s_sp, l.s_lab, reinterpret_cast<const double*>(l.s_big), tid, nt);
    }
    if (tid == 0) R->phase_ticks[2] = (unsigned)(wall_clock64() - wall0);
    if (!upd) phase_slots(job, h, tid, nt);
    if (tid == 0) R->phase_ticks[3] = (unsigned)(wall_clock64() - wall0);

    {
        constexpr int SR = (NB <= 2) ? 16 * NB : 16;
        const long lstride = job.ll_stride;
        SC_GLOBAL float* rows_g = (SC_GLOBAL float*)job.tabLf;
        auto put4 = [&](long idx, f4v v) __attribute__((always_inline)) {
            if (ROWS_LDS) *(f4v*)(s_rows + idx) = v; else *(SC_GLOBAL f4v*)(rows_g + idx) = v;
        };
        const float qnanf = __int_as_float(0x7fc00000);
        for (int q = tid; q < Q; q += nt) {
            const int rid = job.ent_rid[e0 + job.qent[q]], uid = job.quid[q];
            const bool hr = h.do_update ? true : job.has[rid] != 0;
            const bool hu = uid >= 0 && job.has[uid] != 0;
            const long Lf = (long)q * stride;
            auto cell = [&](int sx) __attribute__((always_inline)) -> double {
                const double* row = job.ll + (long)l.s_slot[sx] * lstride;
                double v = hr ? row[rid] : 0.0;
                if (hu) v += row[uid];
                return v;
            };
            double m = -INFINITY;
            double x[SR];
            if (NB <= 2) {
#pragma unroll
                for (int i = 0; i < SR; i++) { x[i] = -INFINITY; if (i < S) { x[i] = cell(i); m = fmax(m, x[i]); } }
            } else {
                for (int s0 = 0; s0 < S; s0 += SR) {
#pragma unroll
                    for (int i = 0; i < SR; i++) if (s0 + i < S) m = fmax(m, cell(s0 + i));
                }
            }
            const bool flag = !(m >= -600.0);
            for (int s0 = 0; s0 < stride; s0 += SR) {
                if (NB > 2) {
#pragma unroll
                    for (int i = 0; i < SR; i++) x[i] = (s0 + i < S) ? cell(s0 + i) : -INFINITY;
                }
#pragma unroll
                for (int i = 0; i < SR; i += 4) {
                    if (s0 + i < stride) {
                        f4v w;
#pragma unroll
                        for (int k = 0; k < 4; k++) {
                            const int sx = s0 + i + k;
                            const float wk = sx < S ? (flag ? qnanf : exp_weight(x[i + k] - m)) : 0.0f;
                            if (k == 0) w.x = wk; else if (k == 1) w.y = wk; else if (k == 2) w.z = wk; else w.w = wk;
                        }
                        put4(Lf + s0 + i, w);
                    }
                }
            }
            if (q == Q - 1) for (int i = 0; i < 16; i += 4) put4(Lf + stride + i, f4v{0.0f, 0.0f, 0.0f, 0.0f});
        }
    }
    __syncthreads();
    if (tid == 0) R->phase_ticks[4] = (unsigned)(wall_clock64() - wall0);
    constexpr int NW = chain_nw(NB);
    if (tid >= 64 * NW) {
        if (!STAY) return;
        urn_chain_shadow<NW>(h, l.s_x);
    } else {
        urn_chain_q<NB, ROWS_LDS, NW>(job, h, l.s_sp, R, l.s_slot, l.s_a, l.s_p, l.s_kf, l.s_a0f, l.s_x, s_uwin, s_rows, stride, tid);
    }
    if (!STAY) nt = 64 * NW;
    draw_log_counts(job, h, l.s_cnt, tid, nt);
    __syncthreads();
    for (int i = tid; i < S * KMAX; i += nt) R->cnt[i] = l.s_cnt[i];
    finish_level(h, R, wall0, tid);
}

template <class IT>
__device__ __forceinline__ void level_plain_body(const IT& it, unsigned char* s_raw) {
    const unsigned long long wall0 = wall_clock64();
    KJob& job = *(KJob*)it.job;
    LevelResult* __restrict__ R = it.R;
    const LevelLds l = level_lds(s_raw);
    double* s_tab = reinterpret_cast<double*>(l.s_big);
    const int tid = threadIdx.x, nt = blockDim.x;
    const LevelHdr h = begin_level(it, l, wall0, tid, nt);
    const int S = h.S, K = job.K, K2 = K * K, e0 = h.e0, Rn = h.e1 - h.e0;
    const long stride = job.ll_stride;
    const bool upd = h.do_update && Rn > 0;
    if (tid < S) l.s_lab[tid] = (int)job.labels[l.s_sp[tid].lab_off];
    phase_copies(job, h, l.s_copy, tid, nt);
    if (tid == 0) R->phase_ticks[1] = (unsigned)(wall_clock64() - wall0);
    if (upd) phase_update(job, h, l.s_sp, l.s_lab, s_tab, tid, nt);
    if (tid == 0) R->phase_ticks[2] = (unsigned)(wall_clock64() - wall0);
    if (Rn <= 0 || S <= 0 || h.mode != MODE_HARD || (h.done & LV_HARD_DONE)) { finish_level(h, R, wall0, tid); return; }
    phase_slots(job, h, tid, nt);
    if (tid == 0) R->phase_ticks[3] = (unsigned)(wall_clock64() - wall0);

    const int Q = h.Q;
    zero_unseen_mates(job, h, l.s_sp, tid, nt);
    __syncthreads();
    for (int q = tid; q < Q; q += nt) { const int uid = job.quid[q]; if (uid >= 0) job.has[uid] = 1; }
    __syncthreads();
    for (long idx = tid; idx < (long)S * Q; idx += nt) {
        const int s = (int)(idx / Q), q = (int)(idx % Q);
        const int rid = job.ent_rid[e0 + job.qent[q]], uid = job.quid[q];
        const double* row = job.ll + (long)l.s_sp[s].slot * stride;
        double x = l.s_sp[s].logpri + row[rid];
        if (uid >= 0) x += row[uid];
        job.tabA[(long)s * job.qcap + q] = x;
    }
    __syncthreads();
    for (int q = tid; q < Q; q += nt) {
        double* col = job.tabA + q;
        double m = -INFINITY;
        for (int s = 0; s < S; s++) m = fmax(m, col[(long)s * job.qcap]);
        normalise_column(col, job.qcap, S, m);
    }
    for (int i = tid; i < S * K2; i += nt) s_tab[i] = 0.0;
    __syncthreads();
    if (tid == 0) R->phase_ticks[4] = (unsigned)(wall_clock64() - wall0);
    if (!h.any_multi) {
        const int lane = tid & 63, wv = tid >> 6, nw = nt >> 6;
        for (int s = wv; s < S; s += nw) {
            double acc[KMAX + 1];
            strain_sums(job.tabA + (long)s * job.qcap, job.qcode, Q, lane, acc);
            if (lane == 0) {
                R->abund[s] = acc[KMAX];
                const int a = l.s_lab[s];
                if (a < K)
                    for (int b = 0; b < K; b++) s_tab[s * K2 + a * K + b] = acc[b];
            }
        }
    } else {
        if (tid < S) {
            const int s = tid;
            const double* prow = job.tabA + (long)s * job.qcap;
            double* hist = s_tab + s * K2;
            const uint8_t* sb = job.labels + l.s_sp[s].lab_off;
            const int ls = l.s_sp[s].lab_len;
            double acc = 0;
            for (int q = 0; q < Q; q++) {
                const double p = prow[q];
                acc += p;
                const int r = job.qent[q], e = e0 + r;
                const uint8_t* rb = job.labels + job.ent_lab_off[e];
                const int lr = job.ent_lab_len[e];
                if (lr == 1) {
                    if (ls == 1) hist[sb[0] * K + rb[0]] += p;
                } else if (job.isnew[r]) {
                    int i = ls, j = lr;
                    while (i > 0 && j > 0) { int a = sb[--i], b = rb[--j]; hist[a * K + b] += p; }
                } else {
                    int i = 0, j = 0;
                    while (i < ls && j < lr) { int a = sb[i++], b = rb[j++]; hist[a * K + b] += p; }
                }
            }
            R->abund[s] = acc;
        }
    }
    __syncthreads();
    for (int i = tid; i < S * K2; i += nt) R->subst[i] = s_tab[i];
    finish_level(h, R, wall0, tid);
}

template <int NB, bool ROWS_LDS>
__global__ __launch_bounds__(CHAIN_THREADS) void k_level_sample(LevelBatch batch) {
    extern __shared__ __attribute__((aligned(16))) unsigned char s_raw[];
    level_sample_body<NB, ROWS_LDS, false>(batch.it[blockIdx.x], s_raw);
}
__global__ __launch_bounds__(512) void k_level(LevelBatch batch) {
    extern __shared__ __attribute__((aligned(16))) unsigned char s_raw[];
    level_plain_body(batch.it[blockIdx.x], s_raw);
}
typedef const __attribute__((address_space(4))) LevelItem KItem;
template <int NB, bool ROWS_LDS>
__device__ __noinline__ void level_sample_call(const LevelItem* it) {
    extern __shared__ __attribute__((aligned(16))) unsigned char s_raw[];
    level_sample_body<NB, ROWS_LDS, true>(*it, s_raw);
}
__device__ __noinline__ void level_plain_call(const LevelItem* it) {
    extern __shared__ __attribute__((aligned(16))) unsigned char s_raw[];
    level_plain_body(*it, s_raw);
}
__device__ __forceinline__ void level_dispatch(const LevelItem* it) {
    const int kind = item_kind(it->kind);
    if (!kind_has_sampler(kind)) { level_plain_call(it); return; }
    with_sampler_variant(kind, [&](auto nb, auto rows_lds) { level_sample_call<decltype(nb)::value, decltype(rows_lds)::value>(it); });
}
__global__ __launch_bounds__(CHAIN_THREADS) void k_level_any(LevelBatch batch) {
    __shared__ LevelItem s_item;
    KItem* it = (KItem*)__builtin_amdgcn_kernarg_segment_ptr() + blockIdx.x;
    if (threadIdx.x < sizeof(LevelItem) / 4) reinterpret_cast<unsigned*>(&s_item)[threadIdx.x] = reinterpret_cast<const __attribute__((address_space(4))) unsigned*>(it)[threadIdx.x];
    __syncthreads();
    level_dispatch(&s_item);
    (void)batch;
}

__global__ __launch_bounds__(CHAIN_THREADS) void k_level_resident(ResidentArgs a) {
    __shared__ __attribute__((aligned(16))) LevelItem s_item;
    __shared__ int s_cmd;
    Mailbox* mb = a.mail + blockIdx.x;
    const int tid = threadIdx.x;
    unsigned last = 0, served = 0;
    if (tid == 0) {
        last = __hip_atomic_load(&mb->ack, __ATOMIC_RELAXED, __HIP_MEMORY_SCOPE_SYSTEM);
        __hip_atomic_store(&mb->state, 1u, __ATOMIC_RELAXED, __HIP_MEMORY_SCOPE_SYSTEM);
    }
    for (;;) {
        if (tid == 0) {
            int cmd = 0;
            unsigned naps = 0;
            unsigned long long t_hb = wall_clock64();
            unsigned hb0 = __hip_atomic_load(&a.ctl->heartbeat, __ATOMIC_RELAXED, __HIP_MEMORY_SCOPE_SYSTEM);
            for (;;) {
                const unsigned sq = __hip_atomic_load(&mb->seq, __ATOMIC_RELAXED, __HIP_MEMORY_SCOPE_SYSTEM);
                if (sq != last) { cmd = 1; break; }
                if ((naps & 15u) == 15u) {
                    if (__hip_atomic_load(&a.ctl->stop, __ATOMIC_RELAXED, __HIP_MEMORY_SCOPE_SYSTEM)) break;
                    const unsigned hb = __hip_atomic_load(&a.ctl->heartbeat, __ATOMIC_RELAXED, __HIP_MEMORY_SCOPE_SYSTEM);
                    const unsigned long long now = wall_clock64();
                    if (hb != hb0) { hb0 = hb; t_hb = now; }
                    else if (now - t_hb > a.idle_ticks) break;
                }
                naps++;
                if (naps < 32) __builtin_amdgcn_s_sleep(4);
                else if (naps < 256) __builtin_amdgcn_s_sleep(32);
                else __builtin_amdgcn_s_sleep(127);
            }
            if (cmd) {
                __builtin_amdgcn_fence(__ATOMIC_ACQUIRE, "");
                __builtin_amdgcn_s_dcache_inv();
                asm volatile("s_waitcnt vmcnt(0) lgkmcnt(0)" ::: "memory");
                const volatile u4v* src = reinterpret_cast<const volatile u4v*>(&mb->item);
                u4v* dst = reinterpret_cast<u4v*>(&s_item);
                static_assert(sizeof(LevelItem) == 80 && alignof(Mailbox) >= 8, "mailbox item");
#pragma unroll
                for (int i = 0; i < 5; i++) dst[i] = src[i];
                last = s_item.h.seq;
                served++;
                const long ip = s_item.P - a.P_base, ir = s_item.R - a.R_base;
                if (ip < 0 || ip >= a.n_blocks || ir != ip || a.P_base + ip != s_item.P || s_item.job == nullptr) cmd = 2;
            }
            s_cmd = cmd;
        }
        __syncthreads();
        if (s_cmd != 1) break;
        level_dispatch(&s_item);
        __syncthreads();
    }
    if (tid == 0) {
        __hip_atomic_store(&mb->levels, served, __ATOMIC_RELAXED, __HIP_MEMORY_SCOPE_SYSTEM);
        __hip_atomic_store(&mb->state, s_cmd == 2 ? 3u : 2u, __ATOMIC_RELEASE, __HIP_MEMORY_SCOPE_SYSTEM);
    }
}
__global__ __launch_bounds__(256) void k_level_copy(JobDev job, const LevelParams* __restrict__ P) {
    const int c = blockIdx.y;
    const double2* src = reinterpret_cast<const double2*>(job.ll + (long)P->copy_src[c] * job.ll_stride);
    double2* dst = reinterpret_cast<double2*>(job.ll + (long)P->copy_dst[c] * job.ll_stride);
    const int n2 = (job.n_reads + 1) >> 1;
    for (int i = blockIdx.x * blockDim.x + threadIdx.x; i < n2; i += gridDim.x * blockDim.x) dst[i] = src[i];
}

__global__ __launch_bounds__(256) void k_level_update(JobDev job, LevelHdr h, const LevelParams* __restrict__ P) {
    __shared__ double s_row[MAXS * KMAX];
    __shared__ double s_diag[MAXS * KMAX];
    __shared__ int s_slot[MAXS], s_lab[MAXS];
    const int tid = threadIdx.x;
    const int S = h.S, K = job.K, e0 = h.e0, Rn = h.e1 - h.e0, codeN = job.code_N;
    for (int s = tid; s < S; s += blockDim.x) { s_slot[s] = P->sp[s].slot; s_lab[s] = job.labels[P->sp[s].lab_off]; }
    __syncthreads();
    for (int i = tid; i < S * KMAX; i += blockDim.x) {
        const int sx = i / KMAX, b = i % KMAX, a = s_lab[sx];
        const double* lp = P->lpt + (long)sx * K * K;
        s_row[i] = (a < K && b < K) ? lp[a * K + b] : 0.0;
        s_diag[i] = (b < K) ? lp[b * K + b] : 0.0;
    }
    __syncthreads();
    const long total = (long)S * Rn;
    const long stride = job.ll_stride;
    for (long idx = (long)blockIdx.x * blockDim.x + tid; idx < total; idx += (long)gridDim.x * blockDim.x) {
        const int sx = (int)(idx / Rn), e = e0 + (int)(idx % Rn);
        const int rid = job.ent_rid[e];
        const int b = job.labels[job.ent_lab_off[e]];
        const bool fresh = job.ent_first[e] && !job.has[rid];
        if (sx == 0) job.isnew[e - e0] = fresh ? 1 : 0;
        int a = s_lab[sx];
        const bool wild = (a == codeN);
        if (wild) a = b;
        const double val = (a < K && b < K) ? (wild ? s_diag[sx * KMAX + b] : s_row[sx * KMAX + b]) : __longlong_as_double(0x7ff8000000000000ll);
        double* cell = job.ll + (long)s_slot[sx] * stride + rid;
        *cell = fresh ? val : (*cell + val);
    }
}

__global__ __launch_bounds__(256) void k_level_has(JobDev job, LevelHdr h) {
    mark_present(job, h, blockIdx.x * blockDim.x + threadIdx.x, gridDim.x * blockDim.x);
}

__global__ __launch_bounds__(256) void k_hard_slots(JobDev job, LevelHdr h) {
    phase_slots<false>(job, h, blockIdx.x * blockDim.x + threadIdx.x, gridDim.x * blockDim.x);
}
__global__ __launch_bounds__(256) void k_hard_mates(JobDev job, LevelHdr h, const LevelParams* __restrict__ P) {
    zero_unseen_mates(job, h, P->sp, blockIdx.x * blockDim.x + threadIdx.x, gridDim.x * blockDim.x);
}
__global__ __launch_bounds__(256) void k_hard_resp(JobDev job, LevelHdr h, const LevelParams* __restrict__ P) {
    __shared__ int s_slot[MAXS];
    __shared__ double s_logpri[MAXS];
    const int S = h.S, e0 = h.e0;
    for (int s = threadIdx.x; s < S; s += blockDim.x) { s_slot[s] = P->sp[s].slot; s_logpri[s] = P->sp[s].logpri; }
    __syncthreads();
    const long stride = job.ll_stride;
    for (int q = blockIdx.x * blockDim.x + threadIdx.x; q < h.Q; q += gridDim.x * blockDim.x) {
        const int rid = job.ent_rid[e0 + job.qent[q]], uid = job.quid[q];
        if (uid >= 0) job.has[uid] = 1;
        double* col = job.tabA + q;
        double m = -INFINITY;
        for (int s = 0; s < S; s++) {
            const double* row = job.ll + (long)s_slot[s] * stride;
            double x = s_logpri[s] + row[rid];
            if (uid >= 0) x += row[uid];
            col[(long)s * job.qcap] = x;
            m = fmax(m, x);
        }
        normalise_column(col, job.qcap, S, m);
    }
}
__global__ __launch_bounds__(64) void k_hard_sums(JobDev job, LevelHdr h, const LevelParams* __restrict__ P, LevelResult* __restrict__ R) {
    const int s = blockIdx.x, lane = threadIdx.x, K = job.K, K2 = K * K, Q = h.Q;
    double acc[KMAX + 1];
    strain_sums(job.tabA + (long)s * job.qcap, job.qcode, Q, lane, acc);
    const int a = (int)job.labels[P->sp[s].lab_off];
    double row[KMAX];
#pragma unroll
    for (int b = 0; b < KMAX; b++) row[b] = __shfl(acc[b], 0);
    for (int i = lane; i < K2; i += 64) {
        double v = 0.0;
#pragma unroll
        for (int b = 0; b < KMAX; b++) if (a < K && b < K && i == a * K + b) v = row[b];
        R->subst[(long)s * K2 + i] = v;
    }
    if (lane == 0) R->abund[s] = acc[KMAX];
}

static int allow_lds(const void* kernel) { return (int)hipFuncSetAttribute(kernel, hipFuncAttributeMaxDynamicSharedMemorySize, LDS_TOTAL); }
int init_level_kernels() {
    int rc = allow_lds(reinterpret_cast<const void*>(k_level));
    rc |= allow_lds(reinterpret_cast<const void*>(k_level_any));
    rc |= allow_lds(reinterpret_cast<const void*>(k_level_resident));
    for (int kind = 1; kind <= N_SAMPLER_KINDS; kind++)
        with_sampler_variant(kind, [&](auto nb, auto rows_lds) { rc |= allow_lds(reinterpret_cast<const void*>(&k_level_sample<decltype(nb)::value, decltype(rows_lds)::value>)); });
    return rc;
}
int level_table_capacity() { return LDS_BIG / (int)sizeof(double); }
constexpr long GRID_ITEMS = 1L << 17;
constexpr long GRID_COPY_WORDS = 1L << 19;
constexpr long GRID_HARD = 1L << 18;
static long grid_min(long dflt) {
    static const long forced = [] { const char* e = getenv("SC_GRID_MIN"); return e ? atol(e) : -1L; }();
    return forced >= 0 ? forced : dflt;
}
static bool hard_on_grid(const LevelHdr& h) {
    return h.mode == MODE_HARD && h.do_update && (long)h.S * (h.e1 - h.e0) > grid_min(GRID_ITEMS) && !h.has_dups && !h.any_multi &&
           (long)h.S * h.Q > grid_min(GRID_HARD) && h.e1 > h.e0;
}
bool level_wants_grid(const JobDev& job, const LevelHdr& h) {
    const long items = (long)h.S * (h.e1 - h.e0);
    return (h.do_update && items > grid_min(GRID_ITEMS) && !h.has_dups && !h.any_multi) || (long)h.n_copy * job.n_reads > grid_min(GRID_COPY_WORDS);
}
int launch_level_grid(hipStream_t st, const JobDev& job, const LevelHdr& h, const LevelParams* Pd, LevelResult* R) {
    const int S = h.S, Rn = h.e1 - h.e0;
    int done = 0;
    const bool update_on_grid = h.do_update && (long)S * Rn > grid_min(GRID_ITEMS) && !h.has_dups && !h.any_multi;
    if (h.n_copy > 0 && ((long)h.n_copy * job.n_reads > grid_min(GRID_COPY_WORDS) || update_on_grid)) {
        const int n2 = (job.n_reads + 1) >> 1;
        int bx = (n2 + 1023) / 1024;
        bx = bx < 1 ? 1 : (bx > 256 ? 256 : bx);
        hipLaunchKernelGGL(k_level_copy, dim3(bx, h.n_copy), dim3(256), 0, st, job, Pd);
        done |= LV_COPIES_DONE;
    }
    const long items = (long)S * Rn;
    if (update_on_grid) {
        int g = (int)((items + 511) / 512);
        g = g < 1 ? 1 : (g > 1024 ? 1024 : g);
        hipLaunchKernelGGL(k_level_update, dim3(g), dim3(256), 0, st, job, h, Pd);
        done |= LV_ITEMS_DONE;
        int gh = (Rn + 255) / 256;
        hipLaunchKernelGGL(k_level_has, dim3(gh < 1 ? 1 : (gh > 1024 ? 1024 : gh)), dim3(256), 0, st, job, h);
        done |= LV_HAS_DONE;
        if (hard_on_grid(h)) {
            int gq = (h.Q + 255) / 256;
            gq = gq < 1 ? 1 : (gq > 2048 ? 2048 : gq);
            hipLaunchKernelGGL(k_hard_slots, dim3(gh < 1 ? 1 : (gh > 1024 ? 1024 : gh)), dim3(256), 0, st, job, h);
            hipLaunchKernelGGL(k_hard_mates, dim3(gq), dim3(256), 0, st, job, h, Pd);
            hipLaunchKernelGGL(k_hard_resp, dim3(gq), dim3(256), 0, st, job, h, Pd);
            hipLaunchKernelGGL(k_hard_sums, dim3(S), dim3(64), 0, st, job, h, Pd, R);
            done |= LV_HARD_DONE;
        }
    }
    return done;
}
int level_kind(const LevelHdr& h) {
    const int S = h.S, Q = h.Q, Rn = h.e1 - h.e0;
    const bool chain = h.mode == MODE_SAMPLE && h.n_sweeps > 0 && S > 1 && Rn > 0;
    if (!chain) return 0;
    const bool wl = ((long)Q * chain_w_stride(S) + 16) * 4 <= (long)CHAINW_ROWS_BYTES;
    int nb = (S + 15) / 16;
    nb = nb < 1 ? 1 : (nb > 8 ? 8 : nb);
    return sampler_kind(nb, wl);
}
int level_lds_kb(const LevelHdr& h, int K) {
    const int kind = level_kind(h);
    const long S = h.S, Rn = h.e1 - h.e0;
    long big = 0;
    if ((h.do_update && Rn > 0) || h.mode == MODE_HARD) big = (long)sizeof(double) * S * K * K;
    if (kind_has_sampler(kind)) {
        long rows = (long)UWIN * 4;
        if (kind_rows_lds(kind)) rows += ((long)h.Q * chain_w_stride(h.S) + 16) * 4;
        if (rows > big) big = rows;
    }
    long need = LDS_SMALL + big + 64;
    if (need > LDS_TOTAL) need = LDS_TOTAL;
    return (int)((need + 1023) / 1024);
}
static size_t batch_lds(const LevelBatch& b, int n) {
    int kb = 0;
    for (int i = 0; i < n; i++) { const int k = item_lds_kb(b.it[i].kind); kb = k > kb ? k : kb; }
    size_t bytes = (size_t)kb * 1024;
    if (kb == 0 || bytes > (size_t)LDS_TOTAL) bytes = LDS_TOTAL;
    return bytes;
}
void launch_level_any(hipStream_t st, const LevelBatch& b, int n) {
    hipLaunchKernelGGL(k_level_any, dim3(n), dim3(CHAIN_THREADS), batch_lds(b, n), st, b);
}
void launch_level_batch(hipStream_t st, int kind, const LevelBatch& b, int n) {
    const size_t lds = batch_lds(b, n);
    if (!kind_has_sampler(kind)) {
        hipLaunchKernelGGL(k_level, dim3(n), dim3(512), lds, st, b);
        return;
    }
    with_sampler_variant(kind, [&](auto nb, auto rows_lds) {
        hipLaunchKernelGGL((k_level_sample<decltype(nb)::value, decltype(rows_lds)::value>), dim3(n), dim3(CHAIN_THREADS), lds, st, b);
    });
}
void launch_resident(hipStream_t st, const ResidentArgs& a, int slots) {
    hipLaunchKernelGGL(k_level_resident, dim3(slots), dim3(CHAIN_THREADS), LDS_TOTAL, st, a);
}
}
#ifdef SC_CHAIN_PROF
extern "C" int sc_debug_chain_prof(unsigned long long* out) {
    return (int)hipMemcpyFromSymbol(out, HIP_SYMBOL(sc::g_chain_prof), sizeof(unsigned long long) * 12);
}
#endif
```

rambl_amd/csrc/sc_region.cpp:

```cpp
#include "sc_ctx.hpp"

namespace sc {

int Worker::msa_device(const std::vector<std::string>& seqs, std::vector<std::string>& rows) {
    const int n = (int)seqs.size();
    std::vector<int> off(n + 1, 0);
    std::string packed;
    for (int i = 0; i < n; i++) { packed += seqs[i]; off[i + 1] = (int)packed.size(); }
    const int cmax = (int)packed.size() + 1;
    size_t longest = 0;
    for (int i = 1; i < n; i++) longest = std::max(longest, seqs[i].size());
    MsaDev d;
    char* dseq = (char*)m_seqs.ensure(packed.size() + 1);
    int* doff = (int*)m_off.ensure(sizeof(int) * (n + 1));
    stage->h2d(dseq, packed.data(), packed.size(), st);
    stage->h2d(doff, off.data(), sizeof(int) * (n + 1), st);
    d.seqs = dseq; d.seq_off = doff; d.n = n; d.cmax = cmax;
    d.cols[0] = (char*)m_cols0.ensure((size_t)cmax * n);
    d.cols[1] = (char*)m_cols1.ensure((size_t)cmax * n);
    d.counts = (int*)m_counts.ensure(sizeof(int) * 11 * (size_t)cmax);
    d.mv_stride = (int)((longest + 1 + 63) / 64) * 64;
    d.moves = (uint8_t*)m_moves.ensure((size_t)(cmax + 1) * (size_t)d.mv_stride);
    d.edge = (int*)m_edge.ensure(sizeof(int) * 2 * (size_t)(cmax + 1));
    d.trace = (int*)m_trace.ensure(sizeof(int) * 2 * (size_t)(cmax + 64));
    int* dout = (int*)m_out.ensure(sizeof(int) * 2);
    d.ncol_out = dout; d.err_out = dout + 1;
    launch_msa(st, d);
    int out[2];
    stage->d2h(out, dout, sizeof(out), st);
    sync_stream();
    stage->land();
    if (out[1] & 0xFF) {
        size_t longest = 0;
        for (auto& q : seqs) longest = std::max(longest, q.size());
        throw ScError(SC_ERR_UNSUPPORTED, "MSA kernel capacity exceeded (" + std::string((out[1] & 1) ? "a sequence longer than 63; " : "") +
                      std::string((out[1] & 2) ? "more than 1024 columns; " : "") + std::string((out[1] & 4) ? "column buffer; " : "") +
                      std::string((out[1] & 8) ? "more than 65535 sequences; " : "") + std::to_string(n) + " sequences, longest " +
                      std::to_string(longest) + ", columns so far " + std::to_string(out[0]) + ")");
    }
    const int ncol = out[0], cur = out[1] >> 8;
    std::vector<char> cols((size_t)ncol * n);
    if (ncol > 0) {
        stage->d2h(cols.data(), d.cols[cur], (size_t)ncol * n, st);
        sync_stream();
        stage->land();
    }
    rows.assign(n, std::string((size_t)ncol, '-'));
    for (int c = 0; c < ncol; c++)
        for (int k = 0; k < n; k++) rows[k][c] = cols[(size_t)c * n + k];
    return ncol;
}


void Worker::thread_device(const std::string& G, const std::vector<AlignedRead>& R, const std::vector<std::vector<CigarOp>>& cig,
                           ThreadTables& T) {
    const int glen = (int)G.size(), n = (int)R.size();
#ifdef SC_GRAPH_TIMING
    double tdp_ = now_ms();
#define SC_DPHASE(name) do { HIPCHK(hipStreamSynchronize(st)); const double t_ = now_ms(); fprintf(stderr, "      thread_device %-12s %.2f ms\n", name, t_ - tdp_); tdp_ = t_; } while (0)
#else
#define SC_DPHASE(name) do {} while (0)
#endif
    bool present[256] = {false};
    for (const auto& r : R) for (unsigned char c : r.seq) present[c] = true;
    std::memset(T.lut, 0xFF, sizeof T.lut);
    T.sym.clear();
    for (char c : {'A', 'C', 'G', 'T'}) { T.lut[(unsigned char)c] = (uint8_t)T.sym.size(); T.sym.push_back(c); }
    for (int c = 0; c < 256; c++)
        if (present[c] && T.lut[c] == 0xFF) {
            if (T.sym.size() >= 8) throw ScError(SC_ERR_UNSUPPORTED, "more than 8 distinct symbols in the reads");
            T.lut[c] = (uint8_t)T.sym.size(); T.sym.push_back((char)c);
        }
    std::vector<int> pos(n), seq_off(n + 1, 0), cig_off(n + 1, 0), cig_len;
    std::string seq, cig_op;
    long m_bases = 0;
    for (int r = 0; r < n; r++) {
        pos[r] = R[r].pos;
        seq += R[r].seq; seq_off[r + 1] = (int)seq.size();
        for (const CigarOp& c : cig[r]) { cig_op.push_back(c.op); cig_len.push_back(c.len); if (c.op == 'M') m_bases += c.len; }
        cig_off[r + 1] = (int)cig_op.size();
    }
    SC_DPHASE("pack");
    const int ncls = glen * 8;
    ThreadDev d{};
    d.glen = glen; d.n_reads = n;
    char* dref = (char*)t_ref.ensure((size_t)glen + 1);
    stage->h2d(dref, G.data(), (size_t)glen, st);
    d.ref = dref;
    d.pos = upload(*stage, t_pos, pos, st);
    d.seq_off = upload(*stage, t_seqoff, seq_off, st);
    char* dseq = (char*)t_seq.ensure(seq.size() + 1);
    stage->h2d(dseq, seq.data(), seq.size(), st);
    d.seq = dseq;
    d.cig_off = upload(*stage, t_cigoff, cig_off, st);
    char* dop = (char*)t_cigop.ensure(cig_op.size() + 1);
    stage->h2d(dop, cig_op.data(), cig_op.size(), st);
    d.cig_op = dop;
    d.cig_len = upload(*stage, t_ciglen, cig_len, st);
    uint8_t* dlut = (uint8_t*)t_lut.ensure(256);
    stage->h2d(dlut, T.lut, 256, st);
    d.lut = dlut;
    const size_t words = (size_t)ncls * 4 + (size_t)ncls * 8 + (size_t)ncls + 1 + (size_t)ncls + 1 + 1 + (size_t)ncls;
    int* tabs = (int*)t_tabs.ensure(sizeof(int) * words);
    d.count = tabs; d.minrid = tabs + ncls; d.smin = tabs + 2 * (size_t)ncls; d.emin = tabs + 3 * (size_t)ncls;
    d.tmin = tabs + 4 * (size_t)ncls; d.off = tabs + 12 * (size_t)ncls; d.cursor = d.off + ncls + 1; d.err = d.cursor + ncls; d.big = d.err + 1;
    HIPCHK(hipMemsetAsync(d.count, 0, sizeof(int) * (size_t)ncls, st));
    HIPCHK(hipMemsetAsync(d.minrid, 0x7f, sizeof(int) * (size_t)ncls * 11, st));
    HIPCHK(hipMemsetAsync(d.off, 0, sizeof(int) * ((size_t)ncls * 2 + 3), st));
    d.pool = (int*)t_pool.ensure(sizeof(int) * (size_t)std::max<long>(m_bases, 1));
    int* pool_sorted = (int*)t_pool2.ensure(sizeof(int) * (size_t)std::max<long>(m_bases, 1));
    SC_DPHASE("uploads");
    launch_thread(st, d, pool_sorted);
    SC_DPHASE("kernels");
    T.count.resize(ncls); T.minrid.resize(ncls); T.smin.resize(ncls); T.emin.resize(ncls);
    T.tmin.resize((size_t)ncls * 8); T.off.resize((size_t)ncls + 1); T.pool.resize((size_t)m_bases);
    int err = 0;
    stage->d2h(T.count.data(), d.count, sizeof(int) * (size_t)ncls, st);
    stage->d2h(T.minrid.data(), d.minrid, sizeof(int) * (size_t)ncls, st);
    stage->d2h(T.smin.data(), d.smin, sizeof(int) * (size_t)ncls, st);
    stage->d2h(T.emin.data(), d.emin, sizeof(int) * (size_t)ncls, st);
    stage->d2h(T.tmin.data(), d.tmin, sizeof(int) * (size_t)ncls * 8, st);
    stage->d2h(T.off.data(), d.off, sizeof(int) * ((size_t)ncls + 1), st);
    stage->d2h(T.pool.data(), pool_sorted, sizeof(int) * (size_t)std::max<long>(m_bases, 0), st);
    stage->d2h(&err, d.err, sizeof(int), st);
    const double t_sync0 = now_ms();
    sync_stream();
    stage->land();
    if (ctx->plan.opt.sync_log) fprintf(stderr, "sync thread_device %.3f ms\n", now_ms() - t_sync0);
    SC_DPHASE("downloads");
#undef SC_DPHASE
    if (err) throw ScError(SC_ERR_ARG, "a read runs outside the window or past its own bases");
    const int INF = 0x7fffffff;
    auto fix = [&](std::vector<int>& v) { for (int& x : v) if (x == 0x7f7f7f7f) x = INF; };
    fix(T.minrid); fix(T.smin); fix(T.emin); fix(T.tmin);
}

JobDev Worker::job_dev(PinnedArena& ar, const FlatGraph& f, const std::vector<int>& ent_qoff, const std::vector<int>& mate_off,
                       const std::vector<int>& mate_idx, int n_reads, long qcap, int max_entries, long max_draws) {
    JobDev jd{};
    jd.ent_rid = upload(ar, b_ent_rid, f.ent_rid, st);
    jd.ent_cn = upload(ar, b_ent_cn, f.ent_cn, st);
    jd.ent_lab_off = upload(ar, b_ent_lab_off, f.ent_lab_off, st);
    jd.ent_lab_len = upload(ar, b_ent_lab_len, f.ent_lab_len, st);
    jd.ent_first = upload(ar, b_ent_first, f.ent_first, st);
    jd.ent_qoff = upload(ar, b_ent_qoff, ent_qoff, st);
    jd.labels = upload(ar, b_labels, f.labels, st);
    jd.mate_ptr = upload(ar, b_mate_ptr, mate_off, st);
    jd.mate_idx = upload(ar, b_mate_idx, mate_idx, st);
    jd.n_reads = n_reads; jd.K = f.K; jd.code_N = f.code_N;
    jd.ll_stride = ((long)n_reads + 3) & ~3L;
    jd.isnew = (uint8_t*)b_isnew.ensure((size_t)max_entries + 8);
    jd.qcap = qcap;
    jd.tabA = (double*)b_tabA.ensure(sizeof(double) * (size_t)qcap * MAXS);
    jd.tabLf = (float*)b_tabLf.ensure(sizeof(float) * (size_t)(std::min<long>(qcap, MAX_DRAWS) + 4) * 136);
    jd.qcode = (uint8_t*)b_qcode.ensure((size_t)qcap + 8);
    jd.qent = (int*)b_qent.ensure(sizeof(int) * (size_t)qcap);
    jd.quid = (int*)b_quid.ensure(sizeof(int) * (size_t)qcap);
    jd.dlog_cap = std::max<long>(max_draws, 1);
    jd.dlog = (uint8_t*)b_dlog.ensure((size_t)jd.dlog_cap + 8);
    return jd;
}

void Worker::cluster(Job& job, const PoGraph& g, FlatGraph& f) {
    const int n_reads = (int)job.reads.size();
    const double t_cluster0 = now_ms();

    const int final_e0 = (int)f.ent_rid.size();
    long total_copies = 0;
    {
        int qo = 0;
        for (int i = 0; i < n_reads; i++) {
            f.ent_rid.push_back(i); f.ent_cn.push_back(job.reads[i].cn); f.ent_lab_off.push_back(0);
            f.ent_lab_len.push_back(0); f.ent_first.push_back(1);
            qo += job.reads[i].cn;
        }
        total_copies = qo;
    }
    std::vector<int>& ent_qoff = ent_qoff_buf;
    ent_qoff.assign(f.ent_rid.size(), 0);
    int max_level_entries = n_reads, max_level_q = 0;
    for (int l = 0; l < f.n_levels; l++) {
        int qo = 0;
        for (int x = f.level_ent_ptr[l]; x < f.level_ent_ptr[l + 1]; x++) { ent_qoff[x] = qo; qo += f.ent_cn[x]; }
        max_level_entries = std::max(max_level_entries, f.level_ent_ptr[l + 1] - f.level_ent_ptr[l]);
        max_level_q = std::max(max_level_q, qo);
    }
    { int qo = 0; for (int i = 0; i < n_reads; i++) { ent_qoff[final_e0 + i] = qo; qo += job.reads[i].cn; } }
    const long qcap = std::max<long>(std::max<long>(max_level_q, total_copies), 1);
    auto level_draws = [&](long Q) { return (long)level_sweeps(job.params, Q) * Q; };
    long max_draws = level_draws(total_copies);
    for (int l = 0; l < f.n_levels; l++) max_draws = std::max(max_draws, level_draws(f.level_read_count[(size_t)l]));
    std::vector<int> level_hi((size_t)f.n_levels + 1, 0);
    for (int l = 0; l < f.n_levels; l++) {
        int hi = level_hi[(size_t)l];
        for (int x = f.level_ent_ptr[l]; x < f.level_ent_ptr[l + 1]; x++) {
            const int rid = f.ent_rid[x];
            hi = std::max(hi, rid + 1);
            for (int k = job.mate_off[(size_t)rid]; k < job.mate_off[(size_t)rid + 1]; k++) hi = std::max(hi, job.mate_idx[(size_t)k] + 1);
        }
        level_hi[(size_t)l + 1] = hi;
    }

    JobDev jd = job_dev(*stage, f, ent_qoff, job.mate_off, job.mate_idx, n_reads, qcap, max_level_entries, max_draws);
    jd.ll = (double*)b_ll.ensure(sizeof(double) * (size_t)jd.ll_stride * MAXS);
    jd.has = (uint8_t*)b_has.ensure((size_t)n_reads + 8);
    HIPCHK(hipMemsetAsync(jd.has, 0, (size_t)n_reads + 8, st));
    jd.U = ctx->U.d.p;
    jd.Uf = ctx->U.f.p;
    const JobDev* jd_dev = (const JobDev*)b_jobdev.ensure(sizeof(JobDev));
    stage->h2d((void*)jd_dev, &jd, sizeof jd, st);

    {
        std::vector<int> esrc(f.out_node.size());
        for (int a = 0; a < f.n_nodes; a++) for (int x = f.out_ptr[a]; x < f.out_ptr[a + 1]; x++) esrc[x] = a;
        int* d_out_ptr = upload(*stage, b_out_ptr, f.out_ptr, st);
        int* d_out_node = upload(*stage, b_out_node, f.out_node, st);
        int* d_pool_ptr = upload(*stage, b_pool_ptr, f.pool_ptr, st);
        int* d_pool_rid = upload(*stage, b_pool_rid, f.pool_rid, st);
        int* d_pool_cn = upload(*stage, b_pool_cn, f.pool_cn, st);
        uint8_t* d_isend = upload(*stage, b_isend, f.node_is_end, st);
        int* d_esrc = upload(*stage, b_esrc, esrc, st);
        int* d_sup = (int*)b_support.ensure(sizeof(int) * std::max<size_t>(esrc.size(), 1));
        launch_edge_support(st, d_out_ptr, d_out_node, d_pool_ptr, d_pool_rid, d_pool_cn, d_isend, d_esrc, (int)esrc.size(),
                            f.pools_sorted ? 1 : 0, d_sup);
        if (!esrc.empty())
            stage->d2h(f.out_support.data(), d_sup, sizeof(int) * esrc.size(), st);
        const double t_sync0 = now_ms();
        sync_stream();
        stage->land();
        if (stage != &passthrough) ctx->arenas.release(stage);
        stage = &passthrough;
        if (ctx->plan.opt.sync_log) fprintf(stderr, "sync uploads+edge_support %.3f ms (since cluster start %.3f)\n", now_ms() - t_sync0, now_ms() - t_cluster0);
        job.edge_support = f.out_support;
    }

    if (setup_held) { ctx->gate.leave(); setup_held = false; }
    job.stats.setup_ms = now_ms() - t_cluster0;
    MailHold mail_hold{this};
    if (grid) {
        const double t_m0 = now_ms();
        mslot.store(grid->acquire_mailbox(this), std::memory_order_release);
        job.stats.mailbox_ms = now_ms() - t_m0;
        __atomic_store_n(&Rh->seq, 0u, __ATOMIC_RELEASE);
    }
    walk_levels(*this, job, f, jd, jd_dev, level_hi, final_e0, total_copies, mail_hold);
}

void Worker::process(Job& job) {
    const double t0 = now_ms();
    struct Lease {
        Worker* w;
        ~Lease() { if (w->stage && w->stage != &w->passthrough) w->ctx->arenas.release(w->stage); w->stage = nullptr; }
    } lease{this};
    struct Setup {
        Worker* w;
        ~Setup() { if (w->setup_held) { w->ctx->gate.leave(); w->setup_held = false; } }
    } setup{this};
    job.stats.queue_ms = t0 - job.t_submit;
    if (ctx->gate.split_exec) FiberPool::yield();
    ctx->gate.enter(this);
    setup_held = true;
    job.stats.place_ms = now_ms() - t0;
    stage = ctx->arenas.lease(&passthrough);
    MsaFn msa = [this](const std::vector<std::string>& seqs, std::vector<std::string>& rows) { return msa_device(seqs, rows); };
    ThreadFn thr = [this, &job](const std::string& G, const std::vector<AlignedRead>& R, const std::vector<std::vector<CigarOp>>& cg,
                          ThreadTables& T) {
        thread_device(G, R, cg, T);
        if (job.params.graph_only || job.params.want_graph) {
            job.thr_count = T.count; job.thr_first = T.minrid; job.thr_pool = T.pool; job.thr_sym.assign(T.sym.begin(), T.sym.end());
            job.thr_smin = T.smin; job.thr_emin = T.emin; job.thr_tmin = T.tmin;
        }
    };
    sc::set_graph_threads(ctx->workers.size() == 1 ? std::min(8, std::max(1, (int)(sc::cpu_budget_host() / sc::local_world_size()))) : 1);
    PoGraph g(job.ref, job.reads, msa, thr);
    job.stats.msa_calls = g.msa_calls;
    if (job.params.graph_only || job.params.want_graph) job.graph_dump = g.dump();
    FlatGraph& f = flat;
    f.reset();
    flatten(g, (int)job.reads.size(), f);
    job.stats.n_nodes = f.n_nodes; job.stats.n_levels = f.n_levels; job.stats.n_unique_reads = (int)job.reads.size();
    long copies = 0;
    for (auto& r : job.reads) copies += r.cn;
    job.stats.n_read_copies = copies;
    const double t1 = now_ms();
    job.stats.graph_ms = t1 - t0;
    if (!job.params.graph_only) {
        if (!f.unsupported.empty()) throw ScError(SC_ERR_UNSUPPORTED, f.unsupported);
        cluster(job, g, f);
    }
    job.stats.cluster_ms = now_ms() - t1;
}

}
```

rambl_amd/csrc/sc_sched.cpp:

```cpp
#include "sc_ctx.hpp"

namespace sc {

PinnedArena* ArenaPool::lease(PinnedArena* passthrough) {
    if (limit <= 0) { passthrough->on = false; return passthrough; }
    for (;;) {
        {
            std::lock_guard<std::mutex> lk(mu);
            if (!free_arenas.empty()) { PinnedArena* a = free_arenas.back(); free_arenas.pop_back(); a->reset(); return a; }
            if ((int)arenas.size() < limit) { arenas.emplace_back(new PinnedArena()); return arenas.back().get(); }
        }
        if (FiberPool::in_fiber()) FiberPool::yield(); else std::this_thread::yield();
    }
}
void ArenaPool::release(PinnedArena* a) {
    std::lock_guard<std::mutex> lk(mu);
    free_arenas.push_back(a);
}
void SetupGate::enter(Worker* w) {
    {
        std::lock_guard<std::mutex> lk(mu);
        if (setups < limit) { setups++; return; }
        waiters.push_back(w);
    }
    FiberPool::park();
}
void SetupGate::leave() {
    Worker* next = nullptr;
    {
        std::lock_guard<std::mutex> lk(mu);
        if (!waiters.empty()) { next = waiters.front(); waiters.pop_front(); }
        else setups--;
    }
    if (next) pool->make_ready(next->fib, split_exec);
}

LevelServer::LevelServer(int device, int n_streams, bool sweep_log) : device(device), sweep_log(sweep_log), lstreams((size_t)n_streams) {
    thread = std::thread([this] { serve(); });
}
LevelServer::~LevelServer() {
    { std::lock_guard<std::mutex> lk(dmu); stop.store(true, std::memory_order_seq_cst); }
    dcv.notify_all();
    if (thread.joinable()) thread.join();
}
void LevelServer::serve() {
    (void)hipSetDevice(device);
    std::deque<LevelRequest> waiting;
    std::vector<Flying> flying;
    std::string dead;
    auto stamped = [](Worker* w) { return __atomic_load_n(&w->Rh->seq, __ATOMIC_ACQUIRE) == w->seq; };
    unsigned idle_spins = 0;
    double sweep_t0 = 0, sweep_sum = 0, sweep_max = 0; long sweep_n = 0, sweep_fly = 0;
    for (;;) {
        if (n_pending.load(std::memory_order_seq_cst) > 0) {
            plk.lock();
            const int took = (int)pending.size();
            waiting.insert(waiting.end(), pending.begin(), pending.end());
            pending.clear();
            plk.unlock();
            n_pending.fetch_sub(took, std::memory_order_seq_cst);
        } else if (waiting.empty() && flying.empty()) {
            std::unique_lock<std::mutex> lk(dmu);
            asleep.store(true, std::memory_order_seq_cst);
            if (n_pending.load(std::memory_order_seq_cst) == 0 && !stop.load(std::memory_order_seq_cst)) dcv.wait_for(lk, std::chrono::milliseconds(50));
            asleep.store(false, std::memory_order_seq_cst);
            if (stop.load(std::memory_order_seq_cst)) break;
            continue;
        }
        bool progressed = false;
        if (sweep_log) {
            const double t = now_ms();
            if (sweep_t0 > 0 && !flying.empty()) { const double d = t - sweep_t0; sweep_sum += d; sweep_max = std::max(sweep_max, d); sweep_n++; sweep_fly += (long)flying.size(); }
            sweep_t0 = t;
        }
        for (size_t i = 0; i < flying.size();) {
            Worker* w = flying[i].w;
            if (stamped(w)) {
                lstreams[(size_t)flying[i].stream].busy--;
                flying[i] = flying.back(); flying.pop_back();
                w->finish_level(2);
                progressed = true;
            } else {
                ++i;
            }
        }
        while (!waiting.empty()) {
            if (!dead.empty()) { waiting.front().w->finish_level(3, dead.c_str()); waiting.pop_front(); progressed = true; continue; }
            int fs = -1;
            for (size_t i = 0; i < lstreams.size(); i++) if (lstreams[i].busy == 0) { fs = (int)i; break; }
            if (fs < 0) break;
            const int kind = waiting.front().kind;
            LevelBatch batch;
            Worker* who[MAXB];
            int n = 0;
            bool timed = false, mixed = false;
            for (auto it = waiting.begin(); it != waiting.end() && n < MAXB;) {
                mixed = mixed || it->kind != kind;
                batch.it[n] = it->item;
                who[n++] = it->w;
                timed = timed || it->timed;
                it = waiting.erase(it);
            }
            hipStream_t st = lstreams[(size_t)fs].s.st;
            (void)hipGetLastError();
            if (timed) for (int i = 0; i < n; i++) (void)hipEventRecord(who[i]->ev0, st);
            if (mixed) launch_level_any(st, batch, n);
            else launch_level_batch(st, kind, batch, n);
            const hipError_t le = hipGetLastError();
            if (le != hipSuccess) {
                const std::string msg = std::string("level kernel launch: ") + hipGetErrorString(le);
                for (int i = 0; i < n; i++) who[i]->finish_level(3, msg.c_str());
                progressed = true;
                continue;
            }
            if (timed) for (int i = 0; i < n; i++) (void)hipEventRecord(who[i]->ev1, st);
            lstreams[(size_t)fs].busy = n;
            lstreams[(size_t)fs].unretired++;
            const double tl = now_ms();
            for (int i = 0; i < n; i++) { who[i]->t_batch_launched = tl; who[i]->batch_n = n; flying.push_back(Flying{who[i], fs}); }
            progressed = true;
        }
        if (progressed) { idle_spins = 0; continue; }
        if (idle_spins % 256u == 0) {
            for (auto& ls : lstreams)
                if (ls.busy == 0 && ls.unretired > 0) { if (hipStreamQuery(ls.s.st) == hipSuccess) ls.unretired = 0; break; }
        }
        __builtin_ia32_pause();
        if (++idle_spins % (1u << 20) == 0) {
            for (size_t si = 0; si < lstreams.size(); si++) {
                LaunchStream& ls = lstreams[si];
                if (ls.busy == 0) continue;
                const hipError_t e = hipStreamQuery(ls.s.st);
                if (e == hipErrorNotReady) continue;
                if (e != hipSuccess) { dead = std::string("level kernel: ") + hipGetErrorString(e); break; }
                for (size_t i = 0; i < flying.size();) {
                    Worker* w = flying[i].w;
                    if (flying[i].stream != (int)si || stamped(w)) { ++i; continue; }
                    ls.busy--;
                    flying[i] = flying.back(); flying.pop_back();
                    w->finish_level(3, "a level kernel ended without its completion stamp");
                }
            }
            if (!dead.empty()) {
                for (const Flying& fl : flying) { lstreams[(size_t)fl.stream].busy = 0; fl.w->finish_level(3, dead.c_str()); }
                flying.clear();
            }
        }
    }
    if (sweep_log && sweep_n) fprintf(stderr, "level server: %ld rounds with levels flying, %.2f us each (longest %.1f us), %.1f levels flying on average\n",
                                      sweep_n, 1e3 * sweep_sum / sweep_n, 1e3 * sweep_max, (double)sweep_fly / sweep_n);
    for (const Flying& fl : flying) fl.w->finish_level(3, "context destroyed");
    for (auto& rq : waiting) rq.w->finish_level(3, "context destroyed");
}
void LevelServer::submit(const LevelRequest& rq) {
    rq.w->level_state.store(1, std::memory_order_release);
    plk.lock();
    pending.push_back(rq);
    plk.unlock();
    n_pending.fetch_add(1, std::memory_order_seq_cst);
    if (asleep.load(std::memory_order_seq_cst)) {
        { std::lock_guard<std::mutex> lk(dmu); }
        dcv.notify_one();
    }
}

static int top_priority() {
    int lo = 0, hi = 0;
    (void)hipDeviceGetStreamPriorityRange(&lo, &hi);
    return hi;
}
ResidentGrid::ResidentGrid(Ctx& ctx, int slots, bool watch_stamps, int n_workers)
    : slots(slots), mail((size_t)slots), mail_seq((size_t)slots, 0u), mail_done((size_t)slots, 0u),
      watch(watch_stamps ? new StampWatch((size_t)n_workers) : nullptr), ctx(ctx), rstream(top_priority()), ctl(1) {
    for (int m = slots - 1; m >= 0; m--) free_mail.push_back(m);
    std::memset(mail.p, 0, (size_t)slots * sizeof(Mailbox));
    std::memset(ctl.p, 0, sizeof(ResidentCtl));
    heart = std::thread([this] {
        unsigned beats = 0;
        while (!heart_stop.load(std::memory_order_acquire)) {
            __atomic_fetch_add(&ctl.p->heartbeat, 1u, __ATOMIC_RELEASE);
            if (watch && (++beats % 50u) == 0) poll_health();
            std::this_thread::sleep_for(std::chrono::milliseconds(20));
        }
    });
}
ResidentGrid::~ResidentGrid() {
    shutdown();
    heart_stop.store(true, std::memory_order_release);
    if (heart.joinable()) heart.join();
}
int ResidentGrid::acquire_mailbox(Worker* w) {
    {
        std::lock_guard<std::mutex> lk(mmu);
        if (!free_mail.empty()) { const int m = free_mail.back(); free_mail.pop_back(); return m; }
        w->mslot.store(-1, std::memory_order_release);
        mail_waiters.push_back(w);
    }
    FiberPool::park();
    return w->mslot.load(std::memory_order_acquire);
}
void ResidentGrid::release_mailbox(int m) {
    Worker* next = nullptr;
    {
        std::lock_guard<std::mutex> lk(mmu);
        if (!mail_waiters.empty()) { next = mail_waiters.front(); mail_waiters.pop_front(); next->mslot.store(m, std::memory_order_release); }
        else free_mail.push_back(m);
    }
    if (next) ctx.pool->make_ready(next->fib);
}
void ResidentGrid::ensure(int m) {
    if (gen_state.load(std::memory_order_acquire) == GEN_RUNNING && __atomic_load_n(&mail.p[m].state, __ATOMIC_ACQUIRE) < 2u) return;
    const double t0 = now_ms();
    for (;;) {
        if (now_ms() - t0 > 60000.0) throw HipError("resident level workers: the previous grid has not left after a minute");
        {
            std::lock_guard<std::mutex> lk(gen_mu);
            if (gen_state == GEN_RUNNING) {
                if (__atomic_load_n(&mail.p[m].state, __ATOMIC_ACQUIRE) < 2u) return;
                __atomic_store_n(&ctl.p->stop, 1u, __ATOMIC_RELEASE);
                gen_state = GEN_STOPPING;
            }
            if (gen_state == GEN_STOPPING) {
                const hipError_t e = hipStreamQuery(rstream.st);
                if (e == hipSuccess) gen_state = GEN_STOPPED;
                else if (e != hipErrorNotReady) throw HipError(std::string("resident level workers: ") + hipGetErrorString(e));
            }
            if (gen_state == GEN_STOPPED) {
                __atomic_store_n(&ctl.p->stop, 0u, __ATOMIC_RELEASE);
                for (int i = 0; i < slots; i++) { mail.p[i].ack = __atomic_load_n(&mail_done[(size_t)i], __ATOMIC_ACQUIRE); mail.p[i].state = 0; }
                __atomic_thread_fence(__ATOMIC_RELEASE);
                ResidentArgs ra{mail.d, ctl.d, 300000000ull, ctx.workers[0]->Pm, ctx.workers[0]->Rd, (int)ctx.workers.size()};
                (void)hipGetLastError();
                launch_resident(rstream.st, ra, slots);
                const hipError_t le = hipGetLastError();
                if (le != hipSuccess) throw HipError(std::string("resident level workers, launch: ") + hipGetErrorString(le));
                gen_state = GEN_RUNNING;
                return;
            }
        }
        if (FiberPool::in_fiber() && ctx.workers.size() > 1) FiberPool::yield(); else std::this_thread::yield();
    }
}
void ResidentGrid::idle() {
    std::lock_guard<std::mutex> lk(gen_mu);
    if (gen_state == GEN_RUNNING && ctx.regions_active.load(std::memory_order_acquire) == 0) {
        __atomic_store_n(&ctl.p->stop, 1u, __ATOMIC_RELEASE);
        gen_state = GEN_STOPPING;
    }
}
void ResidentGrid::shutdown() {
    {
        std::lock_guard<std::mutex> lk(gen_mu);
        __atomic_store_n(&ctl.p->stop, 1u, __ATOMIC_RELEASE);
        if (gen_state == GEN_RUNNING) gen_state = GEN_STOPPING;
    }
    const double t0 = now_ms();
    while (hipStreamQuery(rstream.st) == hipErrorNotReady && now_ms() - t0 < 10000.0) std::this_thread::sleep_for(std::chrono::microseconds(100));
    gen_state = GEN_STOPPED;
}
static const char* resident_failure(const Mailbox& mb, const unsigned* stamp, unsigned want, double t_posted) {
    const unsigned ms = __atomic_load_n(&mb.state, __ATOMIC_ACQUIRE);
    const bool never = ms == 0u && now_ms() - t_posted > 20000.0;
    if ((ms < 2u && !never) || __atomic_load_n(stamp, __ATOMIC_ACQUIRE) == want) return nullptr;
    return never ? "the slot's resident level worker has not started within 20 s (more slots than the GPU holds resident workgroups?)"
         : ms == 3u ? "the slot's resident level worker received an item that was not its own"
                    : "the slot's resident level worker has left before the level was done";
}
bool ResidentGrid::poll_stamps() {
    Ctx* c = &ctx;
    return watch->poll([c](size_t i) { return &c->workers[i]->Rh->seq; }, [c](size_t i) { c->workers[i]->finish_level(2); });
}
void ResidentGrid::poll_health() {
    watch->check(
        [this](size_t i, unsigned want) -> const char* {
            const Worker* w = ctx.workers[i].get();
            const int m = w->mslot.load(std::memory_order_acquire);
            return m < 0 ? nullptr : resident_failure(mail.p[m], &w->Rh->seq, want, w->t_posted.load(std::memory_order_acquire));
        },
        [this](size_t i, const char* why) { ctx.workers[i]->finish_level(3, why); });
}

void Worker::init() {
    HIPCHK(hipSetDevice(ctx->device));
    if (!st) { HIPCHK(hipStreamCreateWithFlags(&st, hipStreamNonBlocking)); own_stream = true; }
    HIPCHK(hipEventCreateWithFlags(&sync_ev, hipEventDisableTiming));
    if (!Ph) {
        own_blocks = true;
        HIPCHK(hipHostMalloc((void**)&Ph, sizeof(LevelParams), hipHostMallocMapped | hipHostMallocCoherent));
        HIPCHK(hipMalloc((void**)&Pd, sizeof(LevelParams)));
        HIPCHK(hipHostMalloc((void**)&Rh, sizeof(LevelResult), hipHostMallocMapped | hipHostMallocCoherent));
    }
    HIPCHK(hipHostGetDevicePointer((void**)&Pm, Ph, 0));
    HIPCHK(hipHostGetDevicePointer((void**)&Rd, Rh, 0));
    std::memset(Rh, 0, sizeof(LevelResult));
    cnt_scratch.assign((size_t)MAXS * KMAX, 0);
}
void Worker::init_private(Ctx* c) {
    ctx = c;
    init();
    stage = &passthrough;
    passthrough.on = false;
}
Worker::~Worker() {
    for (hipEvent_t e : ev_pool) (void)hipEventDestroy(e);
    if (sync_ev) (void)hipEventDestroy(sync_ev);
    if (st && own_stream) (void)hipStreamDestroy(st);
    if (own_blocks) { (void)hipHostFree(Ph); (void)hipFree(Pd); (void)hipHostFree(Rh); }
}

void Worker::sync_stream() {
    if (!FiberPool::in_fiber() || ctx->workers.size() <= 1) { HIPCHK(hipStreamSynchronize(st)); return; }
    HIPCHK(hipEventRecord(sync_ev, st));
    const double t0 = now_ms();
    for (unsigned spins = 0;; spins++) {
        const hipError_t e = hipEventQuery(sync_ev);
        if (e == hipSuccess) return;
        if (e != hipErrorNotReady) throw HipError(std::string("set-up stream: ") + hipGetErrorString(e));
        if ((spins & 0x3FFu) == 0x3FFu && now_ms() - t0 > 180000.0) throw HipError("set-up stream: no progress for 3 minutes");
        if (ctx->pool->ready_now() == 0) std::this_thread::sleep_for(std::chrono::microseconds(40));
        FiberPool::yield();
    }
}

void Worker::wait_level() {
    const double t_park = now_ms();
    FiberPool::park();
    const double t_back = now_ms();
    wake_acc[0] += t_park - t_posted.load(std::memory_order_relaxed);
    wake_acc[1] += t_back - t_seen;
    if (ctx->log) { const double us = 1e3 * (t_back - t_seen); int b = 0; while (b < 23 && us >= (double)(1 << b)) b++; ctx->log->wake_hist[b].fetch_add(1, std::memory_order_relaxed); }
    const int state = level_state.load(std::memory_order_acquire);
    if (state == 3) throw HipError(level_err);
    if (state != 2) throw HipError("a region was resumed before its level was done");
}
void Worker::finish_level(int state, const char* err) {
    if (err) level_err = err;
    t_seen = now_ms();
    level_state.store(state, std::memory_order_release);
    ctx->pool->make_ready(fib);
}
void Worker::complete_level(const LevelItem& it, bool timed) {
    const unsigned want = it.h.seq;
    const bool alone = ctx->workers.size() == 1;
    if (grid) {
        const int m = mslot.load(std::memory_order_relaxed);
        grid->ensure(m);
        Mailbox& mb = grid->mail.p[m];
        mb.item = it;
        __atomic_store_n(&mb.seq, want, __ATOMIC_RELEASE);
        const double t = now_ms();
        t_posted.store(t, std::memory_order_release);
        t_batch_launched = t; batch_n = 1;
        if (alone) {
            for (unsigned spins = 0; __atomic_load_n(&Rh->seq, __ATOMIC_ACQUIRE) != want;) {
                __builtin_ia32_pause();
                if (++spins % (1u << 20) == 0)
                    if (const char* why = resident_failure(mb, &Rh->seq, want, t)) throw HipError(why);
            }
        } else {
            level_state.store(1, std::memory_order_release);
            grid->watch->arm((size_t)slot, want);
            ctx->pool->ensure_poller();
            wait_level();
        }
        __atomic_store_n(&grid->mail_done[(size_t)m], want, __ATOMIC_RELEASE);
    } else if (alone) {
        LevelBatch batch;
        batch.it[0] = it;
        hipStream_t ls = ctx->launch->st;
        if (timed) HIPCHK(hipEventRecord(ev0, ls));
        (void)hipGetLastError();
        launch_level_batch(ls, item_kind(it.kind), batch, 1);
        { const hipError_t le = hipGetLastError(); if (le != hipSuccess) throw HipError(std::string("level kernel launch: ") + hipGetErrorString(le)); }
        if (timed) HIPCHK(hipEventRecord(ev1, ls));
        t_batch_launched = now_ms(); batch_n = 1;
        (void)hipStreamQuery(ls);
        for (unsigned spins = 0; __atomic_load_n(&Rh->seq, __ATOMIC_ACQUIRE) != want;) {
            __builtin_ia32_pause();
            if ((++spins & 0x3FFFFu) == 0) {
                const hipError_t e = hipStreamQuery(ls);
                if (e == hipSuccess) { if (__atomic_load_n(&Rh->seq, __ATOMIC_ACQUIRE) != want) throw HipError("a level kernel ended without its completion stamp"); }
                else if (e != hipErrorNotReady) throw HipError(std::string("level kernel: ") + hipGetErrorString(e));
            }
        }
    } else {
        t_posted.store(now_ms(), std::memory_order_release);
        ctx->server->submit(LevelRequest{this, it, item_kind(it.kind), timed});
        wait_level();
    }
}

void Worker::run() {
    for (;;) {
        std::shared_ptr<Job> job;
        bool parked = false;
        {
            std::lock_guard<std::mutex> lk(ctx->mu);
            if (!ctx->queue.empty()) { job = ctx->queue.front(); ctx->queue.pop_front(); }
            else if (ctx->stop) break;
            else { ctx->idle.push_back(this); parked = true; }
        }
        if (parked) { FiberPool::park(); continue; }
        try {
            if (!st || !Ph) throw HipError("the slot's stream or host-mapped blocks were not created");
            process(*job);
            job->rc = SC_OK;
        } catch (const ScError& ex) { job->rc = ex.code; job->err = ex.what(); }
        catch (const HipError& ex) { job->rc = SC_ERR_HIP; job->err = ex.what(); }
        catch (const std::exception& ex) { job->rc = SC_ERR_INTERNAL; job->err = ex.what(); }
        catch (...) { job->rc = SC_ERR_INTERNAL; job->err = "unknown exception"; }
        if (ctx->regions_active.fetch_sub(1, std::memory_order_acq_rel) == 1 && grid) grid->idle();
        {
            std::lock_guard<std::mutex> lk(ctx->mu);
            job->status = 1;
            if (job->rc != SC_OK) ctx->last_error = job->err;
        }
        ctx->cv_done.notify_all();
    }
    ctx->fibers_left.fetch_sub(1, std::memory_order_release);
}

bool gpu_local_cpus(int device, cpu_set_t* out) {
    char bdf[64] = {0};
    if (hipDeviceGetPCIBusId(bdf, (int)sizeof bdf, device) != hipSuccess) return false;
    for (char* c = bdf; *c; c++) *c = (char)tolower((unsigned char)*c);
    FILE* f = fopen((std::string("/sys/bus/pci/devices/") + bdf + "/local_cpulist").c_str(), "r");
    if (!f) return false;
    char line[4096] = {0};
    const bool got = fgets(line, sizeof line, f) != nullptr;
    fclose(f);
    if (!got) return false;
    cpu_set_t allowed, local;
    CPU_ZERO(&local);
    if (sched_getaffinity(0, sizeof allowed, &allowed) != 0) return false;
    for (const char* c = line; *c && *c != '\n';) {
        char* end = nullptr;
        const long a = strtol(c, &end, 10);
        if (end == c) break;
        long b = a;
        c = end;
        if (*c == '-') { b = strtol(c + 1, &end, 10); c = end; }
        for (long k = a; k <= b && k < CPU_SETSIZE; k++) if (k >= 0 && CPU_ISSET((int)k, &allowed)) CPU_SET((int)k, &local);
        if (*c == ',') c++;
    }
    if (CPU_COUNT(&local) == 0) return false;
    *out = local;
    return true;
}

Ctx::Ctx(int device, const CtxPlan& p)
    : device(device), plan(p), resident(p.resident), U(uniform_stream(1234u, MAX_DRAWS + 2048)),
      arenas(p.arena_limit), P_all((size_t)p.workers), R_all((size_t)p.workers), Pd_all((size_t)p.workers),
      gate(p.setup_limit, p.long_threads > 0, pool) {
    DevBuf::keep = !p.opt.off(p.opt.devbuf_keep);
    if (p.resident) grid.reset(new ResidentGrid(*this, p.res_slots, p.watch, p.workers));
    if (p.server) server.reset(new LevelServer(device, p.launch_streams, p.opt.server_log));
    else launch.reset(new Stream());
    setup_streams.reserve((size_t)p.setup_streams);
    for (int i = 0; i < p.setup_streams; i++) setup_streams.emplace_back();
    for (int i = 0; i < p.workers; i++) {
        auto w = std::make_unique<Worker>();
        w->ctx = this;
        w->grid = grid.get();
        w->slot = i;
        w->st = setup_streams[(size_t)i % setup_streams.size()].st;
        w->Ph = P_all.p + i; w->Rh = R_all.p + i; w->Pd = Pd_all.p + i;
        workers.push_back(std::move(w));
    }
    for (auto& w : workers) w->init();
    const int dev = device;
    pool.reset(new FiberPool(p.exec_threads, [dev] { (void)hipSetDevice(dev); }, p.long_threads));
    if (p.opt.server_log) {
        pool->set_diag(true);
        log.reset(new ServerLog());
        log->t_created = now_ms(); log->n_fast = p.exec_threads - p.long_threads; log->n_long = p.long_threads;
    }
    if (p.watch) { ResidentGrid* g = grid.get(); pool->set_poll([g] { return g->poll_stamps(); }); }
    fibers_left.store(p.workers, std::memory_order_release);
    for (auto& w : workers) {
        Worker* q = w.get();
        q->fib = pool->create([q] { q->run(); });
        if (!q->fib) { last_error = "cannot map a fiber stack"; fibers_left.fetch_sub(1); continue; }
        pool->make_ready(q->fib);
    }
}
Ctx::~Ctx() {
    std::vector<Worker*> wake;
    { std::lock_guard<std::mutex> lk(mu); stop = true; wake.swap(idle); }
    for (Worker* w : wake) pool->make_ready(w->fib);
    while (fibers_left.load(std::memory_order_acquire) > 0) std::this_thread::sleep_for(std::chrono::microseconds(200));
    server.reset();
    pool->shutdown();
    if (log) {
        fprintf(stderr, "executors: %d continuation + %d set-up threads over %.1f ms; inside fibers %.1f / %.1f Mticks\n", log->n_fast, log->n_long,
                now_ms() - log->t_created, pool->busy_ticks(false) * 1e-6, pool->busy_ticks(true) * 1e-6);
        for (int l = 0; l < 2; l++) {
            fprintf(stderr, "  stretches on %s threads (log2 ticks: count):", l ? "set-up" : "continuation");
            for (int b = 0; b < 40; b++) if (pool->stretch_count(l, b)) fprintf(stderr, " %d:%ld", b, pool->stretch_count(l, b));
            fprintf(stderr, "\n");
        }
        fprintf(stderr, "  wake latency (below 2^b us: count):");
        for (int b = 0; b < 24; b++) if (log->wake_hist[b].load()) fprintf(stderr, " %d:%ld", b, log->wake_hist[b].load());
        fprintf(stderr, "\n");
    }
    (void)hipSetDevice(device);
    grid.reset();
}

}

extern "C" int sc_host_bind(int device) {
    int ndev = 0;
    if (hipGetDeviceCount(&ndev) != hipSuccess || device < 0 || device >= ndev) return 0;
    cpu_set_t local;
    const sc::Options opt = sc::read_options();
    if (opt.off(opt.numa_bind) || !sc::gpu_local_cpus(device, &local)) return 0;
    if (sched_setaffinity(0, sizeof local, &local) != 0) return 0;
    return CPU_COUNT(&local);
}
```

rambl_amd/csrc/sc_walk.cpp:

```cpp
#include <cmath>

#include "sc_ctx.hpp"

namespace sc {

struct Model {
    int ks = KMAX;
    ld sub[KK];
    ld comp[6]; ld Z;
    ld lsub[KK];
    double lpc[KK];
    uint16_t stale[KMAX];
    unsigned dirty;
    Model() = default;
    Model(const Model& o) { *this = o; }
    Model& operator=(const Model& o) {
        ks = o.ks; Z = o.Z; dirty = o.dirty;
        const size_t n = (size_t)ks * ks;
        std::memcpy(sub, o.sub, sizeof(ld) * n); std::memcpy(lsub, o.lsub, sizeof(ld) * n); std::memcpy(lpc, o.lpc, sizeof(double) * n);
        std::memcpy(comp, o.comp, sizeof comp); std::memcpy(stale, o.stale, sizeof stale);
        return *this;
    }
};
struct HStrain {
    ld abundance;
    int model;
    int slot;
    int tail;
    int node;
    uint64_t hash; int seqlen;
};
struct PathRec { int node, parent; };

static void recount_rows(Model& s, unsigned rows) {
    rows &= 0x3Fu;
    if (!rows) return;
    for (int i = 0; i < 6; i++) {
        if (!(rows & (1u << i))) continue;
        s.comp[i] = 0;
        for (int j = 0; j < 6; j++) s.comp[i] += s.sub[i * s.ks + j];
    }
    s.Z = 0;
    for (int i = 0; i < 6; i++) s.Z += s.comp[i];
}
static void recount(Model& s) {
    s.Z = 0;
    for (int i = 0; i < 6; i++) {
        s.comp[i] = 0;
        for (int j = 0; j < 6; j++) s.comp[i] += s.sub[i * s.ks + j];
        s.Z += s.comp[i];
    }
}
}
extern "C" long double sc_add_ones(long double a, unsigned long k) {
    if (!std::isfinite((double)a) && !(a == a && a - a == 0)) return a + (long double)k;
    while (k > 0) {
        if (!(a >= 1)) { a += 1; k--; continue; }
        {
            union { long double v; struct { uint64_t mant; uint16_t se; } b; } top;
            top.v = a;
            top.b.se = (uint16_t)((top.b.se & 0x7fffu) + 1u);
            top.b.mant = 0x8000000000000000ull;
            if ((top.b.se & 0x7fffu) <= 16383u + 64u && top.v - a > (long double)k) return a + (long double)k;
        }
        int e;
        (void)frexpl(a, &e);
        const long double top = ldexpl(1.0L, e);
        const long double room = top - a;
        if (!(room >= 1) && !(room > 0)) { a += 1; k--; continue; }
        const long double jr = ceill(room) - 1;
        if (jr >= (long double)k) return a + (long double)k;
        const unsigned long j = (unsigned long)jr;
        a += (long double)j; k -= j;
        a += 1; k--;
    }
    return a;
}
namespace sc {
static uint64_t hash_extend(uint64_t h, const std::string& lab) {
    for (unsigned char c : lab) { h ^= c; h *= 1099511628211ull; }
    return h;
}
static void fmt_g17(std::string& out, double v) {
    char b[64];
    snprintf(b, sizeof b, "%.17g", v);
    out += b;
}

struct LevelWalk {
    Worker& w;
    Job& job;
    const FlatGraph& f;
    const JobDev& jd;
    const JobDev* jd_dev;
    const std::vector<int>& level_hi;
    const int final_e0;
    const long total_copies;
    MailHold& mail;
    const sc_params& pa;
    const ld e, tau, diff;
    const int K, n_reads;
    const bool want_trace;
    const LevelResult* const Rh;

    std::vector<Model> models;
    std::vector<int> free_models, free_slots;
    std::vector<PathRec> arena;
    std::vector<HStrain> level_strains, final_strains;
    std::vector<std::pair<int, int>> pending_copies;
    bool branching = false;
    int cur_level = 0;
    struct Cand { int parent; int node; ld abundance; };
    std::vector<Cand> cands;
    std::vector<int> first_child;
    std::vector<HStrain> kept_buf, sub_strains;
    int la_cache[MAXS];
    double host_acc[3] = {0, 0, 0};
    double t_mark, t_last_done;
    FILE* level_log;

    LevelWalk(Worker& w, Job& job, const FlatGraph& f, const JobDev& jd, const JobDev* jd_dev, const std::vector<int>& level_hi,
              int final_e0, long total_copies, MailHold& mail)
        : w(w), job(job), f(f), jd(jd), jd_dev(jd_dev), level_hi(level_hi), final_e0(final_e0), total_copies(total_copies),
          mail(mail), pa(job.params), e((ld)pa.error_rate), tau((ld)pa.tau), diff((ld)pa.diff_rate), K(f.K),
          n_reads((int)job.reads.size()), want_trace(pa.want_trace != 0), Rh(w.Rh) {
        w.ev_used = 0;
        for (int i = MAXS - 1; i >= 0; i--) free_slots.push_back(i);
        {
            HStrain s{};
            s.model = model_new();
            Model& m = models[(size_t)s.model];
            m.ks = K;
            for (int i = 0; i < K * K; i++) m.sub[i] = 0;
            for (int i = 0; i < 6; i++) for (int j = 0; j < 6; j++) m.sub[i * K + j] = (i == j) ? 100 * (1 - e) : 100 * e;
            recount(m);
            constexpr unsigned all_symbols = (1u << KMAX) - 1u;
            m.dirty = all_symbols;
            for (int a = 0; a < KMAX; a++) m.stale[a] = (uint16_t)all_symbols;
            s.abundance = 0; s.slot = free_slots.back(); free_slots.pop_back();
            s.tail = -1; s.node = -1; s.hash = 1469598103934665603ull; s.seqlen = 0;
            level_strains.push_back(s);
        }
        t_mark = t_last_done = now_ms();
        const Options& opt = w.ctx->plan.opt;
        level_log = opt.level_log ? fopen((opt.level_log_path + "." + std::to_string(w.slot)).c_str(), "a") : nullptr;
    }
    ~LevelWalk() { if (level_log) fclose(level_log); }
    void run() {
        for (int level = 0; level < f.n_levels; level++) {
            visit_nodes(level);
            const int e0 = f.level_ent_ptr[level], e1 = f.level_ent_ptr[level + 1];
            const int Rn = e1 - e0;
            cur_level = level;
            if (Rn > 0 && !level_strains.empty()) {
                const int S = (int)level_strains.size();
                if (S > MAXS) throw ScError(SC_ERR_CAPACITY, "more than 128 candidate strains at one level");
                if ((long)S * K * K > (long)level_table_capacity())
                    throw ScError(SC_ERR_UNSUPPORTED, std::to_string(S) + " candidate strains over " + std::to_string(K) +
                                  " distinct symbols: their log tables do not fit the level kernel's LDS");
                bool has_dups = false, any_multi = false;
                for (int x = e0; x < e1; x++) { if (!f.ent_first[x]) has_dups = true; if (f.ent_lab_len[x] != 1) any_multi = true; }
                for (auto& s : level_strains) if (f.node_lab_len[s.node] != 1) any_multi = true;
                const int Q = f.level_read_count[level];
                if (branching) np_bayes_clustering(e0, e1, Q, has_dups, any_multi);
                else hard_clustering(e0, e1, Q, has_dups, any_multi);
            }
            trace_dump("after clustering", level, level_strains);
            lap(1);
            extend();
            lap(2);
        }
        read_assign();
        report();
    }
    void visit_nodes(int level) {
        const int n0 = f.level_node_ptr[level], n1 = f.level_node_ptr[level + 1];
        for (int x = n0; x < n1; x++) {
            trace_dump("before clustering", level, level_strains);
            const int u = f.level_nodes[x];
            if (u == 0) {
                if (level_strains.empty()) throw ScError(SC_ERR_INTERNAL, "no strain at the root");
                HStrain& s = level_strains[0];
                arena.push_back({0, s.tail});
                s.tail = (int)arena.size() - 1; s.node = 0;
                s.hash = hash_extend(s.hash, f.node_label_str[0]); s.seqlen += (int)f.node_label_str[0].size();
                s.abundance = 1;
            } else if (f.node_is_end[u]) {
                if (level_strains.empty()) { final_strains.clear(); continue; }
                sort_strains(level_strains);
                sort_strains(level_strains);
                std::vector<std::string> seqs;
                for (auto& s : level_strains) seqs.push_back(path_seq(s, false));
                std::vector<int> merged{0};
                for (int i = 1; i < (int)level_strains.size(); i++) {
                    size_t j;
                    for (j = 0; j < merged.size(); j++)
                        if (seq_identity(seqs[i], seqs[merged[j]]) > 1 - diff) {
                            level_strains[merged[j]].abundance += level_strains[i].abundance;
                            break;
                        }
                    if (j == merged.size()) merged.push_back(i);
                }
                std::vector<HStrain> kept;
                std::vector<char> keep(level_strains.size(), 0);
                for (int j : merged) { kept.push_back(level_strains[j]); keep[j] = 1; }
                for (size_t i = 0; i < level_strains.size(); i++) if (!keep[i]) drop(level_strains[i]);
                level_strains.swap(kept);
                final_strains = level_strains;
            }
        }
    }
    void run_level(int mode, int e0, int e1, int Q, int n_sweeps, bool do_update, const std::vector<HStrain>& sv,
                              bool has_dups, bool any_multi) {
        LevelParams& P = *w.Ph;
        const int S = (int)sv.size();
        LevelHdr H{};
        H.mode = mode; H.S = S; H.e0 = e0; H.e1 = e1; H.has_dups = has_dups; H.any_multi = any_multi; H.Q = Q;
        H.n_sweeps = n_sweeps; H.do_update = do_update ? 1 : 0;
        H.n_copy = (int)pending_copies.size();
        H.copy_n = do_update ? level_hi[(size_t)cur_level] : n_reads;
        for (int c = 0; c < H.n_copy; c++) { P.copy_src[c] = pending_copies[c].first; P.copy_dst[c] = pending_copies[c].second; }
        pending_copies.clear();
        {
            uint64_t seen[2] = {0, 0};
            for (int s = 0; s < S; s++) {
                const int r = sv[s].slot;
                if (r < 0 || r >= MAXS || (seen[r >> 6] >> (r & 63)) & 1) throw ScError(SC_ERR_INTERNAL, "two candidates share a read_loglik row");
                seen[r >> 6] |= 1ull << (r & 63);
            }
        }
        for (int s = 0; s < S; s++) {
            const int nd = sv[s].node;
            if (nd >= 0) { __builtin_prefetch(&f.node_lab_off[(size_t)nd]); __builtin_prefetch(&f.node_lab_len[(size_t)nd]); }
            if (do_update) {
                const Model& hm = models[(size_t)sv[s].model];
                __builtin_prefetch(&hm.dirty); __builtin_prefetch(&hm.stale[0]);
                for (int o = 0; o < K * K; o += 8) __builtin_prefetch(&hm.lpc[o]);
            }
        }
        ld za = 0;
        for (int s = 0; s < S; s++) za += sv[s].abundance;
        for (int s = 0; s < S; s++) {
            StrainParam& sp = P.sp[s];
            sp.slot = sv[s].slot;
            sp.lab_off = sv[s].node >= 0 ? f.node_lab_off[sv[s].node] : 0;
            sp.lab_len = sv[s].node >= 0 ? f.node_lab_len[sv[s].node] : 0;
            la_cache[s] = (sp.lab_len == 1) ? (int)f.labels[(size_t)sp.lab_off] : -1;
            sp.pad = 0;
            sp.a0 = (double)sv[s].abundance;
            sp.logpri = (mode == MODE_HARD) ? (double)logl(sv[s].abundance / za) : 0.0;
            if (!do_update) continue;
            Model& hm = models[(size_t)sv[s].model];
            for (int a = 0; a < K; a++) {
                if (!(hm.dirty & (1u << a))) continue;
                const ld lc = logl(a < 6 ? hm.comp[a] : (ld)0);
                for (int b = 0; b < K; b++) {
                    if (hm.stale[a] & (1u << b)) hm.lsub[a * K + b] = logl(hm.sub[a * K + b]);
                    hm.lpc[a * K + b] = (double)(hm.lsub[a * K + b] - lc);
                }
                hm.stale[a] = 0;
            }
            hm.dirty = 0;
            double* dst = P.lpt + (size_t)s * K * K;
            std::memcpy(dst, hm.lpc, sizeof(double) * (size_t)K * K);
        }
        const bool chain = (mode == MODE_SAMPLE) && S > 1 && n_sweeps > 0;
        if (mode == MODE_SAMPLE && (long)n_sweeps * Q > jd.dlog_cap) throw ScError(SC_ERR_INTERNAL, "a level draws more than the region's draw log holds");
        const bool timed = chain && pa.want_timing && !w.grid;
        if (level_wants_grid(jd, H)) {
            const size_t bytes = offsetof(LevelParams, lpt) + sizeof(double) * (size_t)S * K * K;
            HIPCHK(hipMemcpyAsync(w.Pd, w.Ph, bytes, hipMemcpyHostToDevice, w.st));
            H.done = launch_level_grid(w.st, jd, H, w.Pd, w.Rd);
            w.sync_stream();
        }
        const int ms = w.mslot.load(std::memory_order_relaxed);
        H.seq = ms >= 0 ? ++w.grid->mail_seq[(size_t)ms] : ++w.seq;
        if (timed) {
            if (w.ev_used + 2 > w.ev_pool.size()) {
                hipEvent_t a = nullptr, b = nullptr;
                HIPCHK(hipEventCreate(&a)); HIPCHK(hipEventCreate(&b));
                w.ev_pool.push_back(a); w.ev_pool.push_back(b);
            }
            w.ev0 = w.ev_pool[w.ev_used]; w.ev1 = w.ev_pool[w.ev_used + 1];
            w.ev_used += 2;
        }
        const double t_launched = level_log ? now_ms() : 0.0;
        lap(0);
        const LevelItem it = w.level_item(jd_dev, H, K);
        w.complete_level(it, timed);
        t_mark = now_ms();
        sc_stats& stats = job.stats;
        stats.level_launches++;
        if (chain) {
            stats.sampler_launches++; stats.sampler_read_copies += Q;
            stats.draws += (long)Rh->n_draws; stats.exact_draws += (long)Rh->n_exact; stats.slow_draws += (long)Rh->n_slow;
            stats.sampler_strains += S; stats.chain_passes += (long)Rh->n_pass;
            stats.chain_cycles += (long)Rh->chain_cycles; stats.chain_wall_ticks += (long)Rh->chain_wall;
        }
        stats.level_kernel_ticks += (long)Rh->level_wall;
        if (chain) stats.sampler_level_ticks += (long)Rh->level_wall;
        if (level_log) {
            const double t_done = now_ms();
            fprintf(level_log, "h %d mode %d S %d Q %d n %d level_us %.1f chain_us %.1f cyc %llu passes %llu slow %llu xcc %d ncopy %d multi %d "
                    "ph %.1f %.1f %.1f %.1f %.1f host_us %.1f wait_us %.1f pend_us %.1f batch %d\n", job.handle, mode, S, Q,
                    n_sweeps, Rh->level_wall * 0.01, chain ? Rh->chain_wall * 0.01 : 0.0, chain ? (unsigned long long)Rh->chain_cycles : 0ull,
                    chain ? (unsigned long long)Rh->n_pass : 0ull, chain ? (unsigned long long)Rh->n_slow : 0ull, Rh->xcc, H.n_copy, (int)any_multi,
                    Rh->phase_ticks[0] * 0.01, Rh->phase_ticks[1] * 0.01, Rh->phase_ticks[2] * 0.01, Rh->phase_ticks[3] * 0.01, Rh->phase_ticks[4] * 0.01,
                    1e3 * (t_launched - t_last_done), 1e3 * (t_done - t_launched), 1e3 * (w.t_batch_launched - t_launched), w.batch_n);
            t_last_done = t_done;
        }
        stats.xcd_levels[Rh->xcc & 7]++;
        stats.kind_levels[std::min(std::max(item_kind(it.kind), 0), N_SAMPLER_KINDS)]++;
    }
    void np_bayes_clustering(int e0, int e1, int Q, bool has_dups, bool any_multi) {
        const int S = (int)level_strains.size();
        const int n = level_sweeps(pa, Q);
        int last[MAXS];
        for (int s = 0; s < S; s++) {
            last[s] = s;
            for (int t = S - 1; t > s; t--)
                if (level_strains[t].hash == level_strains[s].hash && level_strains[t].seqlen == level_strains[s].seqlen) { last[s] = t; break; }
        }
        ld prior[MAXS], post[MAXS], a[MAXS];
        for (int s = 0; s < S; s++) prior[s] = level_strains[last[s]].abundance;
        run_level(MODE_SAMPLE, e0, e1, Q, n, true, level_strains, has_dups, any_multi);
        ld (*cnt)[KMAX] = reinterpret_cast<ld (*)[KMAX]>(w.cnt_scratch.data());
        for (int s = 0; s < S; s++) {
            const Model& m_ = models[(size_t)level_strains[s].model];
            __builtin_prefetch(&Rh->cnt[s * KMAX]);
            if ((s & 15) == 0) __builtin_prefetch(&Rh->kdraw[s]);
            __builtin_prefetch(&m_.comp[0]); __builtin_prefetch(&m_.comp[4]); __builtin_prefetch(&m_.stale[0]);
            const int la = la_cache[s];
            if (la >= 0 && la < K) { __builtin_prefetch(&m_.sub[la * K]); __builtin_prefetch(&m_.sub[la * K + 4]); }
        }
        for (int s = 0; s < S; s++) for (int b = 0; b < K; b++) cnt[s][b] = 0;
        if (S == 1 || n <= 0) {
            a[0] = level_strains[0].abundance;
            for (int s = 1; s < S; s++) a[s] = level_strains[s].abundance;
            if (n > 0) {
                const long tot = (long)n * Q;
                a[0] = sc_add_ones(a[0], (unsigned long)tot);
                for (int x = e0; x < e1; x++)
                    if (f.ent_lab_len[x] == 1) cnt[0][f.labels[f.ent_lab_off[x]]] += (ld)n * f.ent_cn[x];
            }
        } else {
            for (int s = 0; s < S; s++) {
                a[s] = sc_add_ones(level_strains[s].abundance, Rh->kdraw[s]);
                for (int b = 0; b < K; b++) cnt[s][b] = (ld)Rh->cnt[s * KMAX + b];
            }
        }
        ld z = 0;
        for (int s = 0; s < S; s++) z += a[s];
        for (int s = 0; s < S; s++) a[s] /= z;
        for (int s = 0; s < S; s++) a[s] *= Q;
        for (int s = 0; s < S; s++) {
            HStrain& st_ = level_strains[s];
            Model& m_ = models[(size_t)st_.model];
            st_.abundance += a[s];
            unsigned changed = 0;
            {
                const int la = la_cache[s];
                if (la >= 0 && la < K) {
                    for (int b = 0; b < K; b++)
                        if (cnt[s][b] > 0) { m_.sub[la * K + b] += cnt[s][b] / n; m_.stale[la] |= (uint16_t)(1u << b); }
                    m_.dirty |= 1u << la;
                    changed = 1u << la;
                }
            }
            recount_rows(m_, changed);
        }
        for (int s = 0; s < S; s++) post[s] = level_strains[last[s]].abundance;
        ld A_delta_max = 0;
        for (int s = 0; s < S; s++) { ld d = post[s] - prior[s]; if (A_delta_max < d) A_delta_max = d; }
        ld Z = 0;
        for (int s = 0; s < S; s++) Z += a[s];
        const ld Zt = Z * tau;
        std::vector<HStrain>& kept = kept_buf;
        kept.clear();
        for (int s = 0; s < S; s++) {
            const ld d = post[s] - prior[s];
            if (a[s] < Zt || d < 0.01 * A_delta_max) drop(level_strains[s]);
            else kept.push_back(level_strains[s]);
        }
        level_strains.swap(kept);
    }
    void hard_clustering(int e0, int e1, int Q, bool has_dups, bool any_multi) {
        const int S = (int)level_strains.size();
        run_level(MODE_HARD, e0, e1, Q, 0, true, level_strains, has_dups, any_multi);
        for (int s = 0; s < S; s++) {
            const Model& m_ = models[(size_t)level_strains[s].model];
            for (int o = 0; o < K * K; o += 8) __builtin_prefetch(&Rh->subst[(size_t)s * K * K + o]);
            for (int o = 0; o < K * K; o += 4) __builtin_prefetch(&m_.sub[o]);
            __builtin_prefetch(&m_.comp[0]); __builtin_prefetch(&m_.comp[4]); __builtin_prefetch(&m_.stale[0]);
            if ((s & 7) == 0) __builtin_prefetch(&Rh->abund[s]);
        }
        for (int s = 0; s < S; s++) {
            HStrain& st_ = level_strains[s];
            Model& m_ = models[(size_t)st_.model];
            st_.abundance += (ld)Rh->abund[s];
            const double* sub_d = Rh->subst + (size_t)s * K * K;
            unsigned changed = 0;
            for (int a = 0; a < K; a++)
                for (int b = 0; b < K; b++) {
                    const double d = sub_d[a * K + b];
                    if (d != 0.0) {
                        m_.sub[a * K + b] += (ld)d;
                        m_.dirty |= 1u << a; m_.stale[a] |= (uint16_t)(1u << b); changed |= 1u << a;
                    }
                }
            recount_rows(m_, changed);
        }
    }
    void extend() {
        branching = false;
        cands.clear();
        for (const HStrain& s : level_strains) __builtin_prefetch(&f.out_ptr[(size_t)s.node]);
        for (const HStrain& s : level_strains) {
            const int ob = f.out_ptr[(size_t)s.node];
            __builtin_prefetch(&f.out_node[(size_t)ob]); __builtin_prefetch(&f.out_support[(size_t)ob]);
        }
        for (int si = 0; si < (int)level_strains.size(); si++) {
            const HStrain& s = level_strains[si];
            const int v = s.node;
            const int ob = f.out_ptr[v], oe = f.out_ptr[v + 1];
            ld oz = 0, moc = 0;
            for (int x = ob; x < oe; x++) { const ld oc0 = f.out_support[x]; oz += oc0; if (moc < oc0) moc = oc0; }
            int dd = 0;
            for (int x = ob; x < oe; x++) {
                const int o = f.out_node[x];
                const ld oc = f.out_support[x];
                if (!f.node_is_end[o] && oz > 0) {
                    if (oc <= 1. && oc < moc) { dd += 1; continue; }
                    ld ab;
                    if (oc > 0) ab = s.abundance * oc / oz;
                    else ab = oz * std::min(0.01, (double)tau);
                    cands.push_back({si, o, ab});
                } else {
                    cands.push_back({si, o, s.abundance});
                }
            }
            if (oe - ob > 1 + dd) branching = true;
        }
        if ((int)cands.size() > pa.max_candidates) {
            std::vector<ld> ssa;
            for (auto& c : cands) ssa.push_back(c.abundance);
            std::sort(ssa.begin(), ssa.end(), [](ld x, ld y) { return x > y; });
            const ld Zt0 = (pa.max_candidates >= (int)ssa.size()) ? ssa.back() : ssa[pa.max_candidates];
            std::vector<Cand> kept;
            for (auto& c : cands) if (!(c.abundance < Zt0)) kept.push_back(c);
            cands.swap(kept);
        }
        if ((int)cands.size() > MAXS) throw ScError(SC_ERR_CAPACITY, "more than 128 candidate strains at one level");
        first_child.assign(level_strains.size(), -1);
        for (int c = 0; c < (int)cands.size(); c++) if (first_child[cands[c].parent] < 0) first_child[cands[c].parent] = c;
        for (size_t p = 0; p < level_strains.size(); p++) if (first_child[p] < 0) drop(level_strains[p]);
        sub_strains.clear();
        for (int c = 0; c < (int)cands.size(); c++) {
            const HStrain& par = level_strains[cands[c].parent];
            HStrain ns = par;
            if (first_child[cands[c].parent] == c) { ns.slot = par.slot; ns.model = par.model; }
            else {
                if (free_slots.empty()) throw ScError(SC_ERR_CAPACITY, "out of read_loglik rows");
                ns.slot = free_slots.back(); free_slots.pop_back();
                pending_copies.push_back({par.slot, ns.slot});
                ns.model = model_new();
                models[(size_t)ns.model] = models[(size_t)par.model];
            }
            arena.push_back({cands[c].node, par.tail});
            ns.tail = (int)arena.size() - 1; ns.node = cands[c].node;
            ns.hash = hash_extend(par.hash, f.node_label_str[cands[c].node]);
            ns.seqlen = par.seqlen + (int)f.node_label_str[cands[c].node].size();
            ns.abundance = cands[c].abundance;
            sub_strains.push_back(ns);
        }
        level_strains.swap(sub_strains);
        sub_strains.clear();
    }
    void read_assign() {
        std::vector<HStrain>& fs = final_strains;
        const int S = (int)fs.size();
        if (S == 0) return;
        const int Q = (int)total_copies;
        const int n = level_sweeps(pa, Q);
        std::vector<ld> a(S);
        if (S == 1 || n <= 0) {
            for (int s = 0; s < S; s++) a[s] = fs[s].abundance;
            if (n > 0) a[0] = sc_add_ones(a[0], (unsigned long)((long)n * Q));
        } else {
            pending_copies.clear();
            run_level(MODE_SAMPLE, final_e0, final_e0 + n_reads, Q, n, false, fs, false, true);
            for (int s = 0; s < S; s++) {
                a[s] = sc_add_ones(fs[s].abundance, Rh->kdraw[s]);
            }
        }
        mail.drop();
        if (w.ctx->gate.split_exec && FiberPool::in_fiber()) FiberPool::yield();
        ld z = 0;
        for (int s = 0; s < S; s++) z += a[s];
        for (int s = 0; s < S; s++) fs[s].abundance = a[s] / z;
        sort_strains(fs);
        for (auto& s : fs) {
            job.seqs.push_back(path_seq(s, true));
            job.abund.push_back((double)s.abundance);
        }
    }
    void report() {
        for (size_t k = 0; k + 1 < w.ev_used; k += 2) {
            float ms = 0;
            HIPCHK(hipEventSynchronize(w.ev_pool[k + 1]));
            HIPCHK(hipEventElapsedTime(&ms, w.ev_pool[k], w.ev_pool[k + 1]));
            job.stats.sampler_kernel_ms += ms;
        }
        w.ev_used = 0;
        for (int k = 0; k < 3; k++) job.stats.host_us[k] = 1e3 * host_acc[k];
        for (int k = 0; k < 2; k++) { job.stats.wake_us[k] = 1e3 * w.wake_acc[k]; w.wake_acc[k] = 0; }
    }

    int model_new() {
        if (!free_models.empty()) { const int m = free_models.back(); free_models.pop_back(); return m; }
        models.emplace_back();
        return (int)models.size() - 1;
    }
    void drop(const HStrain& s) { free_slots.push_back(s.slot); free_models.push_back(s.model); }
    void lap(int k) { const double t = now_ms(); host_acc[k] += t - t_mark; t_mark = t; }
    std::string path_seq(const HStrain& s, bool plain) const {
        std::vector<int> rev;
        for (int t = s.tail; t >= 0; t = arena[t].parent) rev.push_back(arena[t].node);
        std::string q;
        for (auto it = rev.rbegin(); it != rev.rend(); ++it) {
            const std::string& pl = f.node_label_str[*it];
            if (!plain || (pl != "^" && pl != "$" && pl != "-" && pl != "=")) q += pl;
        }
        return q;
    }
    void trace_dump(const char* when, int level, const std::vector<HStrain>& sv) {
        if (!want_trace || sv.empty()) return;
        std::string& tr = job.trace;
        tr += "------------------------------\n"; tr += when; tr += "\nlevel: "; tr += std::to_string(level); tr += "\n";
        for (const auto& s : sv) { tr += path_seq(s, false); tr += "\t"; fmt_g17(tr, (double)s.abundance); tr += "\n"; }
    }
    static void sort_strains(std::vector<HStrain>& sv) {
        std::vector<int> perm(sv.size());
        for (size_t i = 0; i < sv.size(); i++) perm[i] = (int)i;
        std_sort_perm(perm, [&](int a, int b) { return sv[a].abundance > sv[b].abundance; });
        std::vector<HStrain> t;
        t.reserve(sv.size());
        for (int i : perm) t.push_back(sv[i]);
        sv.swap(t);
    }
    static ld seq_identity(const std::string& a, const std::string& b) {
        int iden = 0, len = 0;
        for (size_t i = 0; i < a.size(); ++i) {
            const char x = a[i], y = i < b.size() ? b[i] : 0;
            if (x == '-' && y == '-') continue;
            else if (x == '=' && y == '=') continue;
            else if (x == '=' && y == '-') continue;
            else if (x == '-' && y == '=') continue;
            else if (x == '^' && y == '^') continue;
            else if (x == y) iden += 1;
            len += 1;
        }
        return (ld)((iden + 0.0) / len);
    }
};

void walk_levels(Worker& w, Job& job, const FlatGraph& f, const JobDev& jd, const JobDev* jd_dev, const std::vector<int>& level_hi,
                 int final_e0, long total_copies, MailHold& mail) {
    LevelWalk(w, job, f, jd, jd_dev, level_hi, final_e0, total_copies, mail).run();
}

}
```

Measured before the change: 15000.

## Offload slot and weight-row phases to grid kernels before lone sampler launch

Moves the per-level slot setup and the weight-row computation out of the single-block sampler kernel into separate wide grid kernels (k_level_entries, k_level_rows). The sampler then skips those phases when the done flags say so, and copies precomputed rows into LDS instead. For the single-worker path, these grid kernels are launched back to back on the same stream with no host sync, and a device timestamp is stored in a JobBlock. It also splits the update kernel into contiguous per-block ranges and bounds the copy to copy_n. The aim is to parallelise serial prologue work across the GPU. The cost is extra kernel launches and a global round trip for the rows.

Result: faster. 15160, median of 6 (+1.0%).

```diff
diff --git a/rambl_amd/capi.py b/rambl_amd/capi.py
--- a/rambl_amd/capi.py
+++ b/rambl_amd/capi.py
@@ -509,7 +509,7 @@
         U = np.ascontiguousarray(U, dtype=np.float64)
         kdraw = np.zeros(S, dtype=np.uint32)
         cnt = np.zeros((S, 16), dtype=np.uint32)
-        out = (C.c_long * 5)()
+        out = (C.c_long * 6)()
 
         def ptr(x, t):
             return x.ctypes.data_as(C.POINTER(t))
@@ -519,7 +519,7 @@
                                       ptr(kdraw, C.c_uint), ptr(cnt, C.c_uint), out)
         if rc != SC_OK:
             raise self._err(rc)
-        return dict(kdraw=kdraw, cnt=cnt, n_draws=out[0], n_slow=out[1], n_exact=out[2], n_pass=out[3], kind=out[4])
+        return dict(kdraw=kdraw, cnt=cnt, n_draws=out[0], n_slow=out[1], n_exact=out[2], n_pass=out[3], kind=out[4], done=out[5])
 
     def msa_align(self, seqs):
         txt, off = _pack(seqs)
diff --git a/rambl_amd/csrc/sc_api.cpp b/rambl_amd/csrc/sc_api.cpp
--- a/rambl_amd/csrc/sc_api.cpp
+++ b/rambl_amd/csrc/sc_api.cpp
@@ -308,7 +308,7 @@
         DevBuf b_u, b_uf;
         jd.U = upload(w.passthrough, b_u, u, st);
         jd.Uf = upload(w.passthrough, b_uf, uf, st);
-        const JobDev* jd_dev = (const JobDev*)w.b_jobdev.ensure(sizeof(JobDev));
+        const JobDev* jd_dev = (const JobDev*)w.b_jobdev.ensure(sizeof(JobBlock));
         HIPCHK(hipMemcpyAsync((void*)jd_dev, &jd, sizeof jd, hipMemcpyHostToDevice, st));
 
         LevelParams& P = *w.Ph;
@@ -317,17 +317,16 @@
         H.mode = MODE_SAMPLE; H.S = S; H.e0 = e0; H.e1 = E; H.Q = (int)Q; H.n_sweeps = n_sweeps;
         H.n_copy = 0; H.do_update = 0; H.seq = 1;
         std::memset(w.Rh, 0, sizeof(LevelResult));
-        LevelBatch batch;
-        batch.it[0] = w.level_item(jd_dev, H, KMAX);
-        const int kind = item_kind(batch.it[0].kind);
-        launch_level_batch(st, kind, batch, 1);
+        const LevelItem it = w.level_item(jd_dev, H, KMAX);
+        const int kind = item_kind(it.kind);
+        const int done = launch_level(st, it, n_reads);
         HIPCHK(hipGetLastError());
         HIPCHK(hipStreamSynchronize(st));
         const LevelResult& R = *w.Rh;
         if (R.seq != 1u || R.error) throw ScError(SC_ERR_INTERNAL, "the sampler level did not complete");
         for (int s = 0; s < S; s++) kdraw[s] = R.kdraw[s];
         std::memcpy(cnt, R.cnt, sizeof(unsigned) * (size_t)S * KMAX);
-        out[0] = (long)R.n_draws; out[1] = (long)R.n_slow; out[2] = (long)R.n_exact; out[3] = (long)R.n_pass; out[4] = kind;
+        out[0] = (long)R.n_draws; out[1] = (long)R.n_slow; out[2] = (long)R.n_exact; out[3] = (long)R.n_pass; out[4] = kind; out[5] = done;
         return SC_OK;
     } catch (const ScError& ex) { std::lock_guard<std::mutex> lk(ctx->mu); ctx->last_error = ex.what(); return ex.code; }
     catch (const std::exception& ex) { std::lock_guard<std::mutex> lk(ctx->mu); ctx->last_error = ex.what(); return SC_ERR_HIP; }
diff --git a/rambl_amd/csrc/sc_ctx.hpp b/rambl_amd/csrc/sc_ctx.hpp
--- a/rambl_amd/csrc/sc_ctx.hpp
+++ b/rambl_amd/csrc/sc_ctx.hpp
@@ -22,8 +22,9 @@
 void launch_msa(hipStream_t st, const MsaDev& d);
 void launch_thread(hipStream_t st, const ThreadDev& d, int* pool_sorted);
 int init_graph_kernels();
-bool level_wants_grid(const JobDev& job, const LevelHdr& h);
-int launch_level_grid(hipStream_t st, const JobDev& job, const LevelHdr& h, const LevelParams* Pd, LevelResult* R);
+bool level_wants_grid(int n_reads, const LevelHdr& h);
+int launch_level_grid(hipStream_t st, const JobDev* job, int n_reads, const LevelHdr& h, int kind, const LevelParams* P, LevelResult* R, bool lone);
+int launch_level(hipStream_t st, const LevelItem& it, int n_reads);
 int level_kind(const LevelHdr& h);
 int level_lds_kb(const LevelHdr& h, int K);
 int level_table_capacity();
@@ -182,6 +183,7 @@
     std::atomic<double> t_posted{0};
     double t_batch_launched = 0;
     int batch_n = 0;
+    int level_done = 0;
     hipEvent_t ev0 = nullptr, ev1 = nullptr;
     std::vector<hipEvent_t> ev_pool;
     size_t ev_used = 0;
@@ -209,7 +211,7 @@
     void init_private(Ctx* c);
     void run();
     void process(Job& job);
-    void complete_level(const LevelItem& it, bool timed);
+    void complete_level(const LevelItem& it, int n_reads, bool timed);
     void wait_level();
     void finish_level(int state, const char* err = nullptr);
     void sync_stream();
diff --git a/rambl_amd/csrc/sc_device.hpp b/rambl_amd/csrc/sc_device.hpp
--- a/rambl_amd/csrc/sc_device.hpp
+++ b/rambl_amd/csrc/sc_device.hpp
@@ -40,6 +40,11 @@
     long qcap;
     uint8_t* dlog;
     long dlog_cap;
+};
+
+struct JobBlock {
+    JobDev job;
+    unsigned long long t0;
 };
 
 struct LevelHdr {
diff --git a/rambl_amd/csrc/sc_level.hip b/rambl_amd/csrc/sc_level.hip
--- a/rambl_amd/csrc/sc_level.hip
+++ b/rambl_amd/csrc/sc_level.hip
@@ -16,7 +16,7 @@
 static_assert(LDS_SMALL >= (int)(sizeof(double) * 2 * MAXS + sizeof(StrainParam) * MAXS + sizeof(unsigned) * MAXS * KMAX + sizeof(int) * 6 * MAXS + 64), "LDS_SMALL");
 static_assert(LDS_BIG >= (int)(sizeof(double) * MAXS * 64), "LDS_BIG");
 
-enum { LV_COPIES_DONE = 1, LV_ITEMS_DONE = 2, LV_HAS_DONE = 4, LV_HARD_DONE = 8 };
+enum { LV_COPIES_DONE = 1, LV_ITEMS_DONE = 2, LV_HAS_DONE = 4, LV_HARD_DONE = 8, LV_SLOTS_DONE = 16, LV_ROWS_DONE = 32, LV_TICKED = 64 };
 typedef const __attribute__((address_space(4))) JobDev KJob;
 
 __device__ __forceinline__ void stage_params(const LevelHdr& h, const LevelParams* __restrict__ P, StrainParam* s_sp, int* s_copy,
@@ -184,13 +184,13 @@
 }
 
 
-template <class JD>
-__device__ __forceinline__ void zero_unseen_mates(const JD& job, const LevelHdr& h, const StrainParam* sp, int first, int step) {
+template <class JD, class SL>
+__device__ __forceinline__ void zero_unseen_mates(const JD& job, const LevelHdr& h, SL slot_of, int first, int step) {
     const long stride = job.ll_stride;
     for (int q = first; q < h.Q; q += step) {
         const int uid = job.quid[q];
         if (uid >= 0 && !job.has[uid])
-            for (int s = 0; s < h.S; s++) job.ll[(long)sp[s].slot * stride + uid] = 0.0;
+            for (int s = 0; s < h.S; s++) job.ll[(long)slot_of(s) * stride + uid] = 0.0;
     }
 }
 
@@ -218,6 +218,59 @@
         double v = acc[b];
         for (int off = 32; off > 0; off >>= 1) v += __shfl_down(v, off);
         acc[b] = v;
+    }
+}
+
+template <int NB, class JD, class PUT>
+__device__ __forceinline__ void weight_rows(const JD& job, const LevelHdr& h, const int* s_slot, PUT put4, int first, int step) {
+    constexpr int SR = (NB <= 2) ? 16 * NB : 16;
+    const int S = h.S, Q = h.Q, e0 = h.e0;
+    const int stride = chain_w_stride(S);
+    const long lstride = job.ll_stride;
+    const float qnanf = __int_as_float(0x7fc00000);
+    for (int q = first; q < Q; q += step) {
+        const int rid = job.ent_rid[e0 + job.qent[q]], uid = job.quid[q];
+        const bool hr = h.do_update ? true : job.has[rid] != 0;
+        const bool hu = uid >= 0 && job.has[uid] != 0;
+        const long Lf = (long)q * stride;
+        auto cell = [&](int sx) __attribute__((always_inline)) -> double {
+            const double* row = job.ll + (long)s_slot[sx] * lstride;
+            double v = hr ? row[rid] : 0.0;
+            if (hu) v += row[uid];
+            return v;
+        };
+        double m = -INFINITY;
+        double x[SR];
+        if (NB <= 2) {
+#pragma unroll
+            for (int i = 0; i < SR; i++) { x[i] = -INFINITY; if (i < S) { x[i] = cell(i); m = fmax(m, x[i]); } }
+        } else {
+            for (int s0 = 0; s0 < S; s0 += SR) {
+#pragma unroll
+                for (int i = 0; i < SR; i++) if (s0 + i < S) m = fmax(m, cell(s0 + i));
+            }
+        }
+        const bool flag = !(m >= -600.0);
+        for (int s0 = 0; s0 < stride; s0 += SR) {
+            if (NB > 2) {
+#pragma unroll
+                for (int i = 0; i < SR; i++) x[i] = (s0 + i < S) ? cell(s0 + i) : -INFINITY;
+            }
+#pragma unroll
+            for (int i = 0; i < SR; i += 4) {
+                if (s0 + i < stride) {
+                    f4v w;
+#pragma unroll
+                    for (int k = 0; k < 4; k++) {
+                        const int sx = s0 + i + k;
+                        const float wk = sx < S ? (flag ? qnanf : exp_weight(x[i + k] - m)) : 0.0f;
+                        if (k == 0) w.x = wk; else if (k == 1) w.y = wk; else if (k == 2) w.z = wk; else w.w = wk;
+                    }
+                    put4(Lf + s0 + i, w);
+                }
+            }
+        }
+        if (q == Q - 1) for (int i = 0; i < 16; i += 4) put4(Lf + stride + i, f4v{0.0f, 0.0f, 0.0f, 0.0f});
     }
 }
 
@@ -252,6 +305,10 @@
     return h;
 }
 template <class IT>
+__device__ __forceinline__ unsigned long long level_wall0(const IT& it) {
+    return (it.h.done & LV_TICKED) ? reinterpret_cast<const JobBlock*>(it.job)->t0 : wall_clock64();
+}
+template <class IT>
 __device__ __forceinline__ LevelHdr begin_level(const IT& it, const LevelLds& l, unsigned long long wall0, int tid, int nt) {
     const LevelHdr h = load_hdr(it);
     KJob& job = *(KJob*)it.job;
@@ -265,7 +322,7 @@
 }
 template <int NB, bool ROWS_LDS, bool STAY, class IT>
 __device__ __forceinline__ void level_sample_body(const IT& it, unsigned char* s_raw) {
-    const unsigned long long wall0 = wall_clock64();
+    const unsigned long long wall0 = level_wall0(it);
     KJob& job = *(KJob*)it.job;
     LevelResult* __restrict__ R = it.R;
     const LevelLds l = level_lds(s_raw);
@@ -274,7 +331,7 @@
     const int tid = threadIdx.x;
     int nt = blockDim.x;
     const LevelHdr h = begin_level(it, l, wall0, tid, nt);
-    const int S = h.S, Q = h.Q, e0 = h.e0, Rn = h.e1 - h.e0;
+    const int S = h.S, Q = h.Q, Rn = h.e1 - h.e0;
     const int stride = chain_w_stride(S);
     const bool upd = h.do_update && Rn > 0;
     for (int i = tid; i < MAXS * KMAX; i += nt) l.s_cnt[i] = 0;
@@ -286,66 +343,25 @@
     }
     phase_copies(job, h, l.s_copy, tid, nt);
     if (tid == 0) R->phase_ticks[1] = (unsigned)(wall_clock64() - wall0);
+    const bool slots = !(h.done & LV_SLOTS_DONE);
     if (upd) {
-        phase_slots<false>(job, h, tid, nt);
+        if (slots) phase_slots<false>(job, h, tid, nt);
         phase_update(job, h, l.s_sp, l.s_lab, reinterpret_cast<const double*>(l.s_big), tid, nt);
     }
     if (tid == 0) R->phase_ticks[2] = (unsigned)(wall_clock64() - wall0);
-    if (!upd) phase_slots(job, h, tid, nt);
+    if (!upd && slots) phase_slots(job, h, tid, nt);
     if (tid == 0) R->phase_ticks[3] = (unsigned)(wall_clock64() - wall0);
 
-    {
-        constexpr int SR = (NB <= 2) ? 16 * NB : 16;
-        const long lstride = job.ll_stride;
+    if (!(h.done & LV_ROWS_DONE)) {
         SC_GLOBAL float* rows_g = (SC_GLOBAL float*)job.tabLf;
-        auto put4 = [&](long idx, f4v v) __attribute__((always_inline)) {
+        weight_rows<NB>(job, h, l.s_slot, [&](long idx, f4v v) __attribute__((always_inline)) {
             if (ROWS_LDS) *(f4v*)(s_rows + idx) = v; else *(SC_GLOBAL f4v*)(rows_g + idx) = v;
-        };
-        const float qnanf = __int_as_float(0x7fc00000);
-        for (int q = tid; q < Q; q += nt) {
-            const int rid = job.ent_rid[e0 + job.qent[q]], uid = job.quid[q];
-            const bool hr = h.do_update ? true : job.has[rid] != 0;
-            const bool hu = uid >= 0 && job.has[uid] != 0;
-            const long Lf = (long)q * stride;
-            auto cell = [&](int sx) __attribute__((always_inline)) -> double {
-                const double* row = job.ll + (long)l.s_slot[sx] * lstride;
-                double v = hr ? row[rid] : 0.0;
-                if (hu) v += row[uid];
-                return v;
-            };
-            double m = -INFINITY;
-            double x[SR];
-            if (NB <= 2) {
-#pragma unroll
-                for (int i = 0; i < SR; i++) { x[i] = -INFINITY; if (i < S) { x[i] = cell(i); m = fmax(m, x[i]); } }
-            } else {
-                for (int s0 = 0; s0 < S; s0 += SR) {
-#pragma unroll
-                    for (int i = 0; i < SR; i++) if (s0 + i < S) m = fmax(m, cell(s0 + i));
-                }
-            }
-            const bool flag = !(m >= -600.0);
-            for (int s0 = 0; s0 < stride; s0 += SR) {
-                if (NB > 2) {
-#pragma unroll
-                    for (int i = 0; i < SR; i++) x[i] = (s0 + i < S) ? cell(s0 + i) : -INFINITY;
-                }
-#pragma unroll
-                for (int i = 0; i < SR; i += 4) {
-                    if (s0 + i < stride) {
-                        f4v w;
-#pragma unroll
-                        for (int k = 0; k < 4; k++) {
-                            const int sx = s0 + i + k;
-                            const float wk = sx < S ? (flag ? qnanf : exp_weight(x[i + k] - m)) : 0.0f;
-                            if (k == 0) w.x = wk; else if (k == 1) w.y = wk; else if (k == 2) w.z = wk; else w.w = wk;
-                        }
-                        put4(Lf + s0 + i, w);
-                    }
-                }
-            }
-            if (q == Q - 1) for (int i = 0; i < 16; i += 4) put4(Lf + stride + i, f4v{0.0f, 0.0f, 0.0f, 0.0f});
-        }
+        }, tid, nt);
+    } else if (ROWS_LDS) {
+        const f4v* src = reinterpret_cast<const f4v*>(job.tabLf);
+        f4v* dst = reinterpret_cast<f4v*>(s_rows);
+        const int n4 = (Q * stride + 16) >> 2;
+        for (int i = tid; i < n4; i += nt) dst[i] = src[i];
     }
     __syncthreads();
     if (tid == 0) R->phase_ticks[4] = (unsigned)(wall_clock64() - wall0);
@@ -365,7 +381,7 @@
 
 template <class IT>
 __device__ __forceinline__ void level_plain_body(const IT& it, unsigned char* s_raw) {
-    const unsigned long long wall0 = wall_clock64();
+    const unsigned long long wall0 = level_wall0(it);
     KJob& job = *(KJob*)it.job;
     LevelResult* __restrict__ R = it.R;
     const LevelLds l = level_lds(s_raw);
@@ -385,7 +401,7 @@
     if (tid == 0) R->phase_ticks[3] = (unsigned)(wall_clock64() - wall0);
 
     const int Q = h.Q;
-    zero_unseen_mates(job, h, l.s_sp, tid, nt);
+    zero_unseen_mates(job, h, [&](int s) { return l.s_sp[s].slot; }, tid, nt);
     __syncthreads();
     for (int q = tid; q < Q; q += nt) { const int uid = job.quid[q]; if (uid >= 0) job.has[uid] = 1; }
     __syncthreads();
@@ -541,32 +557,44 @@
         __hip_atomic_store(&mb->state, s_cmd == 2 ? 3u : 2u, __ATOMIC_RELEASE, __HIP_MEMORY_SCOPE_SYSTEM);
     }
 }
-__global__ __launch_bounds__(256) void k_level_copy(JobDev job, const LevelParams* __restrict__ P) {
+__device__ __forceinline__ void grid_tick(unsigned long long* t0) {
+    if (t0 && blockIdx.x == 0 && blockIdx.y == 0 && threadIdx.x == 0) *t0 = wall_clock64();
+}
+
+__global__ __launch_bounds__(256) void k_level_copy(const JobDev* jp, LevelHdr h, const LevelParams* __restrict__ P, unsigned long long* t0) {
+    grid_tick(t0);
+    KJob& job = *(KJob*)jp;
     const int c = blockIdx.y;
     const double2* src = reinterpret_cast<const double2*>(job.ll + (long)P->copy_src[c] * job.ll_stride);
     double2* dst = reinterpret_cast<double2*>(job.ll + (long)P->copy_dst[c] * job.ll_stride);
-    const int n2 = (job.n_reads + 1) >> 1;
+    const int n2 = ((h.copy_n < job.n_reads ? h.copy_n : job.n_reads) + 1) >> 1;
     for (int i = blockIdx.x * blockDim.x + threadIdx.x; i < n2; i += gridDim.x * blockDim.x) dst[i] = src[i];
 }
 
-__global__ __launch_bounds__(256) void k_level_update(JobDev job, LevelHdr h, const LevelParams* __restrict__ P) {
+__global__ __launch_bounds__(256) void k_level_update(const JobDev* jp, LevelHdr h, const LevelParams* __restrict__ P, unsigned long long* t0) {
     __shared__ double s_row[MAXS * KMAX];
     __shared__ double s_diag[MAXS * KMAX];
     __shared__ int s_slot[MAXS], s_lab[MAXS];
-    const int tid = threadIdx.x;
+    grid_tick(t0);
+    KJob& job = *(KJob*)jp;
+    const int tid = threadIdx.x, nt = blockDim.x;
     const int S = h.S, K = job.K, e0 = h.e0, Rn = h.e1 - h.e0, codeN = job.code_N;
-    for (int s = tid; s < S; s += blockDim.x) { s_slot[s] = P->sp[s].slot; s_lab[s] = job.labels[P->sp[s].lab_off]; }
-    __syncthreads();
-    for (int i = tid; i < S * KMAX; i += blockDim.x) {
+    const long total = (long)S * Rn;
+    const long per = ((total + gridDim.x - 1) / gridDim.x + nt - 1) / nt * nt;
+    const long lo = (long)blockIdx.x * per, hi = lo + per < total ? lo + per : total;
+    if (lo >= hi) return;
+    const int sa = (int)(lo / Rn), sb = (int)((hi - 1) / Rn);
+    for (int s = sa + tid; s <= sb; s += nt) { s_slot[s] = P->sp[s].slot; s_lab[s] = job.labels[P->sp[s].lab_off]; }
+    __syncthreads();
+    for (int i = sa * KMAX + tid; i < (sb + 1) * KMAX; i += nt) {
         const int sx = i / KMAX, b = i % KMAX, a = s_lab[sx];
         const double* lp = P->lpt + (long)sx * K * K;
         s_row[i] = (a < K && b < K) ? lp[a * K + b] : 0.0;
         s_diag[i] = (b < K) ? lp[b * K + b] : 0.0;
     }
     __syncthreads();
-    const long total = (long)S * Rn;
     const long stride = job.ll_stride;
-    for (long idx = (long)blockIdx.x * blockDim.x + tid; idx < total; idx += (long)gridDim.x * blockDim.x) {
+    for (long idx = lo + tid; idx < hi; idx += nt) {
         const int sx = (int)(idx / Rn), e = e0 + (int)(idx % Rn);
         const int rid = job.ent_rid[e];
         const int b = job.labels[job.ent_lab_off[e]];
@@ -581,19 +609,37 @@
     }
 }
 
-__global__ __launch_bounds__(256) void k_level_has(JobDev job, LevelHdr h) {
-    mark_present(job, h, blockIdx.x * blockDim.x + threadIdx.x, gridDim.x * blockDim.x);
-}
-
-__global__ __launch_bounds__(256) void k_hard_slots(JobDev job, LevelHdr h) {
-    phase_slots<false>(job, h, blockIdx.x * blockDim.x + threadIdx.x, gridDim.x * blockDim.x);
-}
-__global__ __launch_bounds__(256) void k_hard_mates(JobDev job, LevelHdr h, const LevelParams* __restrict__ P) {
-    zero_unseen_mates(job, h, P->sp, blockIdx.x * blockDim.x + threadIdx.x, gridDim.x * blockDim.x);
-}
-__global__ __launch_bounds__(256) void k_hard_resp(JobDev job, LevelHdr h, const LevelParams* __restrict__ P) {
+__global__ __launch_bounds__(256) void k_level_entries(const JobDev* jp, LevelHdr h, int has, int slots, unsigned long long* t0) {
+    grid_tick(t0);
+    KJob& job = *(KJob*)jp;
+    const int first = blockIdx.x * blockDim.x + threadIdx.x, step = gridDim.x * blockDim.x;
+    if (has) mark_present(job, h, first, step);
+    if (slots) phase_slots<false>(job, h, first, step);
+}
+
+template <int NB>
+__global__ __launch_bounds__(64) void k_level_rows(const JobDev* jp, LevelHdr h, const LevelParams* __restrict__ P, unsigned long long* t0) {
+    __shared__ int s_slot[MAXS];
+    grid_tick(t0);
+    KJob& job = *(KJob*)jp;
+    for (int s = threadIdx.x; s < h.S; s += blockDim.x) s_slot[s] = P->sp[s].slot;
+    __syncthreads();
+    SC_GLOBAL float* rows_g = (SC_GLOBAL float*)job.tabLf;
+    weight_rows<NB>(job, h, s_slot, [&](long idx, f4v v) __attribute__((always_inline)) { *(SC_GLOBAL f4v*)(rows_g + idx) = v; },
+                    blockIdx.x * blockDim.x + threadIdx.x, gridDim.x * blockDim.x);
+}
+
+__global__ __launch_bounds__(256) void k_hard_mates(const JobDev* jp, LevelHdr h, const LevelParams* __restrict__ P) {
+    __shared__ int s_slot[MAXS];
+    KJob& job = *(KJob*)jp;
+    for (int s = threadIdx.x; s < h.S; s += blockDim.x) s_slot[s] = P->sp[s].slot;
+    __syncthreads();
+    zero_unseen_mates(job, h, [&](int s) { return s_slot[s]; }, blockIdx.x * blockDim.x + threadIdx.x, gridDim.x * blockDim.x);
+}
+__global__ __launch_bounds__(256) void k_hard_resp(const JobDev* jp, LevelHdr h, const LevelParams* __restrict__ P) {
     __shared__ int s_slot[MAXS];
     __shared__ double s_logpri[MAXS];
+    KJob& job = *(KJob*)jp;
     const int S = h.S, e0 = h.e0;
     for (int s = threadIdx.x; s < S; s += blockDim.x) { s_slot[s] = P->sp[s].slot; s_logpri[s] = P->sp[s].logpri; }
     __syncthreads();
@@ -613,7 +659,8 @@
         normalise_column(col, job.qcap, S, m);
     }
 }
-__global__ __launch_bounds__(64) void k_hard_sums(JobDev job, LevelHdr h, const LevelParams* __restrict__ P, LevelResult* __restrict__ R) {
+__global__ __launch_bounds__(64) void k_hard_sums(const JobDev* jp, LevelHdr h, const LevelParams* __restrict__ P, LevelResult* __restrict__ R) {
+    KJob& job = *(KJob*)jp;
     const int s = blockIdx.x, lane = threadIdx.x, K = job.K, K2 = K * K, Q = h.Q;
     double acc[KMAX + 1];
     strain_sums(job.tabA + (long)s * job.qcap, job.qcode, Q, lane, acc);
@@ -643,49 +690,68 @@
 constexpr long GRID_ITEMS = 1L << 17;
 constexpr long GRID_COPY_WORDS = 1L << 19;
 constexpr long GRID_HARD = 1L << 18;
+constexpr long WIDE_ITEMS = 1L << 12;
 static long grid_min(long dflt) {
     static const long forced = [] { const char* e = getenv("SC_GRID_MIN"); return e ? atol(e) : -1L; }();
     return forced >= 0 ? forced : dflt;
 }
+static long wide_min() {
+    static const long forced = [] { const char* e = getenv("SC_WIDE_MIN"); return e ? atol(e) : -1L; }();
+    return forced >= 0 ? forced : WIDE_ITEMS;
+}
 static bool hard_on_grid(const LevelHdr& h) {
     return h.mode == MODE_HARD && h.do_update && (long)h.S * (h.e1 - h.e0) > grid_min(GRID_ITEMS) && !h.has_dups && !h.any_multi &&
            (long)h.S * h.Q > grid_min(GRID_HARD) && h.e1 > h.e0;
 }
-bool level_wants_grid(const JobDev& job, const LevelHdr& h) {
+bool level_wants_grid(int n_reads, const LevelHdr& h) {
     const long items = (long)h.S * (h.e1 - h.e0);
-    return (h.do_update && items > grid_min(GRID_ITEMS) && !h.has_dups && !h.any_multi) || (long)h.n_copy * job.n_reads > grid_min(GRID_COPY_WORDS);
-}
-int launch_level_grid(hipStream_t st, const JobDev& job, const LevelHdr& h, const LevelParams* Pd, LevelResult* R) {
+    return (h.do_update && items > grid_min(GRID_ITEMS) && !h.has_dups && !h.any_multi) || (long)h.n_copy * n_reads > grid_min(GRID_COPY_WORDS);
+}
+static int grid_blocks(long n, int per, int most) {
+    const long g = (n + per - 1) / per;
+    return (int)(g < 1 ? 1 : (g > most ? most : g));
+}
+int launch_level_grid(hipStream_t st, const JobDev* job, int n_reads, const LevelHdr& h, int kind, const LevelParams* P, LevelResult* R, bool lone) {
     const int S = h.S, Rn = h.e1 - h.e0;
+    const long items = (long)S * Rn;
+    const bool upd = h.do_update && Rn > 0;
+    const bool wide = lone && items > wide_min() && Rn > 0 && S > 0;
+    const bool update_on_grid = upd && !h.has_dups && !h.any_multi && (items > grid_min(GRID_ITEMS) || wide);
+    const bool rows_on_grid = wide && kind_has_sampler(kind) && h.Q > 0 && (update_on_grid || !upd);
+    const bool hard = update_on_grid && hard_on_grid(h);
     int done = 0;
-    const bool update_on_grid = h.do_update && (long)S * Rn > grid_min(GRID_ITEMS) && !h.has_dups && !h.any_multi;
-    if (h.n_copy > 0 && ((long)h.n_copy * job.n_reads > grid_min(GRID_COPY_WORDS) || update_on_grid)) {
-        const int n2 = (job.n_reads + 1) >> 1;
-        int bx = (n2 + 1023) / 1024;
-        bx = bx < 1 ? 1 : (bx > 256 ? 256 : bx);
-        hipLaunchKernelGGL(k_level_copy, dim3(bx, h.n_copy), dim3(256), 0, st, job, Pd);
+    unsigned long long* t0 = lone ? &reinterpret_cast<JobBlock*>(const_cast<JobDev*>(job))->t0 : nullptr;
+    if (h.n_copy > 0 && ((long)h.n_copy * n_reads > grid_min(GRID_COPY_WORDS) || update_on_grid || rows_on_grid)) {
+        const int n = h.copy_n < n_reads ? h.copy_n : n_reads;
+        hipLaunchKernelGGL(k_level_copy, dim3(grid_blocks((n + 1) >> 1, 1024, 256), h.n_copy), dim3(256), 0, st, job, h, P, t0);
+        t0 = nullptr;
         done |= LV_COPIES_DONE;
     }
-    const long items = (long)S * Rn;
     if (update_on_grid) {
-        int g = (int)((items + 511) / 512);
-        g = g < 1 ? 1 : (g > 1024 ? 1024 : g);
-        hipLaunchKernelGGL(k_level_update, dim3(g), dim3(256), 0, st, job, h, Pd);
-        done |= LV_ITEMS_DONE;
-        int gh = (Rn + 255) / 256;
-        hipLaunchKernelGGL(k_level_has, dim3(gh < 1 ? 1 : (gh > 1024 ? 1024 : gh)), dim3(256), 0, st, job, h);
-        done |= LV_HAS_DONE;
-        if (hard_on_grid(h)) {
-            int gq = (h.Q + 255) / 256;
-            gq = gq < 1 ? 1 : (gq > 2048 ? 2048 : gq);
-            hipLaunchKernelGGL(k_hard_slots, dim3(gh < 1 ? 1 : (gh > 1024 ? 1024 : gh)), dim3(256), 0, st, job, h);
-            hipLaunchKernelGGL(k_hard_mates, dim3(gq), dim3(256), 0, st, job, h, Pd);
-            hipLaunchKernelGGL(k_hard_resp, dim3(gq), dim3(256), 0, st, job, h, Pd);
-            hipLaunchKernelGGL(k_hard_sums, dim3(S), dim3(64), 0, st, job, h, Pd, R);
-            done |= LV_HARD_DONE;
-        }
-    }
-    return done;
+        hipLaunchKernelGGL(k_level_update, dim3(grid_blocks(items, 512, 1024)), dim3(256), 0, st, job, h, P, t0);
+        t0 = nullptr;
+        done |= LV_ITEMS_DONE | LV_HAS_DONE;
+    }
+    const bool slots = rows_on_grid || hard;
+    if (update_on_grid || slots) {
+        hipLaunchKernelGGL(k_level_entries, dim3(grid_blocks(Rn, 256, 1024)), dim3(256), 0, st, job, h, update_on_grid ? 1 : 0, slots ? 1 : 0, t0);
+        t0 = nullptr;
+        if (slots) done |= LV_SLOTS_DONE;
+    }
+    if (rows_on_grid) {
+        with_sampler_variant(kind, [&](auto nb, auto) {
+            hipLaunchKernelGGL((k_level_rows<decltype(nb)::value>), dim3(grid_blocks(h.Q, 64, 128)), dim3(64), 0, st, job, h, P, t0);
+        });
+        done |= LV_ROWS_DONE;
+    }
+    if (hard) {
+        const int gq = grid_blocks(h.Q, 256, 2048);
+        hipLaunchKernelGGL(k_hard_mates, dim3(gq), dim3(256), 0, st, job, h, P);
+        hipLaunchKernelGGL(k_hard_resp, dim3(gq), dim3(256), 0, st, job, h, P);
+        hipLaunchKernelGGL(k_hard_sums, dim3(S), dim3(64), 0, st, job, h, P, R);
+        done |= LV_HARD_DONE;
+    }
+    return done ? (done | (lone ? LV_TICKED : 0)) : 0;
 }
 int level_kind(const LevelHdr& h) {
     const int S = h.S, Q = h.Q, Rn = h.e1 - h.e0;
@@ -730,6 +796,14 @@
         hipLaunchKernelGGL((k_level_sample<decltype(nb)::value, decltype(rows_lds)::value>), dim3(n), dim3(CHAIN_THREADS), lds, st, b);
     });
 }
+int launch_level(hipStream_t st, const LevelItem& it, int n_reads) {
+    LevelBatch batch;
+    batch.it[0] = it;
+    LevelItem& b = batch.it[0];
+    b.h.done |= launch_level_grid(st, b.job, n_reads, b.h, item_kind(b.kind), b.P, b.R, true);
+    launch_level_batch(st, item_kind(b.kind), batch, 1);
+    return b.h.done;
+}
 void launch_resident(hipStream_t st, const ResidentArgs& a, int slots) {
     hipLaunchKernelGGL(k_level_resident, dim3(slots), dim3(CHAIN_THREADS), LDS_TOTAL, st, a);
 }
diff --git a/rambl_amd/csrc/sc_region.cpp b/rambl_amd/csrc/sc_region.cpp
--- a/rambl_amd/csrc/sc_region.cpp
+++ b/rambl_amd/csrc/sc_region.cpp
@@ -207,7 +207,7 @@
     HIPCHK(hipMemsetAsync(jd.has, 0, (size_t)n_reads + 8, st));
     jd.U = ctx->U.d.p;
     jd.Uf = ctx->U.f.p;
-    const JobDev* jd_dev = (const JobDev*)b_jobdev.ensure(sizeof(JobDev));
+    const JobDev* jd_dev = (const JobDev*)b_jobdev.ensure(sizeof(JobBlock));
     stage->h2d((void*)jd_dev, &jd, sizeof jd, st);
 
     {
diff --git a/rambl_amd/csrc/sc_sched.cpp b/rambl_amd/csrc/sc_sched.cpp
--- a/rambl_amd/csrc/sc_sched.cpp
+++ b/rambl_amd/csrc/sc_sched.cpp
@@ -339,8 +339,9 @@
     level_state.store(state, std::memory_order_release);
     ctx->pool->make_ready(fib);
 }
-void Worker::complete_level(const LevelItem& it, bool timed) {
+void Worker::complete_level(const LevelItem& it, int n_reads, bool timed) {
     const unsigned want = it.h.seq;
+    level_done = it.h.done;
     const bool alone = ctx->workers.size() == 1;
     if (grid) {
         const int m = mslot.load(std::memory_order_relaxed);
@@ -365,12 +366,10 @@
         }
         __atomic_store_n(&grid->mail_done[(size_t)m], want, __ATOMIC_RELEASE);
     } else if (alone) {
-        LevelBatch batch;
-        batch.it[0] = it;
         hipStream_t ls = ctx->launch->st;
         if (timed) HIPCHK(hipEventRecord(ev0, ls));
         (void)hipGetLastError();
-        launch_level_batch(ls, item_kind(it.kind), batch, 1);
+        level_done = launch_level(ls, it, n_reads);
         { const hipError_t le = hipGetLastError(); if (le != hipSuccess) throw HipError(std::string("level kernel launch: ") + hipGetErrorString(le)); }
         if (timed) HIPCHK(hipEventRecord(ev1, ls));
         t_batch_launched = now_ms(); batch_n = 1;
diff --git a/rambl_amd/csrc/sc_walk.cpp b/rambl_amd/csrc/sc_walk.cpp
--- a/rambl_amd/csrc/sc_walk.cpp
+++ b/rambl_amd/csrc/sc_walk.cpp
@@ -267,10 +267,11 @@
         const bool chain = (mode == MODE_SAMPLE) && S > 1 && n_sweeps > 0;
         if (mode == MODE_SAMPLE && (long)n_sweeps * Q > jd.dlog_cap) throw ScError(SC_ERR_INTERNAL, "a level draws more than the region's draw log holds");
         const bool timed = chain && pa.want_timing && !w.grid;
-        if (level_wants_grid(jd, H)) {
+        const bool lone = !w.grid && w.ctx->workers.size() == 1;
+        if (!lone && level_wants_grid(jd.n_reads, H)) {
             const size_t bytes = offsetof(LevelParams, lpt) + sizeof(double) * (size_t)S * K * K;
             HIPCHK(hipMemcpyAsync(w.Pd, w.Ph, bytes, hipMemcpyHostToDevice, w.st));
-            H.done = launch_level_grid(w.st, jd, H, w.Pd, w.Rd);
+            H.done = launch_level_grid(w.st, jd_dev, jd.n_reads, H, level_kind(H), w.Pd, w.Rd, false);
             w.sync_stream();
         }
         const int ms = w.mslot.load(std::memory_order_relaxed);
@@ -287,7 +288,7 @@
         const double t_launched = level_log ? now_ms() : 0.0;
         lap(0);
         const LevelItem it = w.level_item(jd_dev, H, K);
-        w.complete_level(it, timed);
+        w.complete_level(it, jd.n_reads, timed);
         t_mark = now_ms();
         sc_stats& stats = job.stats;
         stats.level_launches++;
@@ -301,10 +302,10 @@
         if (chain) stats.sampler_level_ticks += (long)Rh->level_wall;
         if (level_log) {
             const double t_done = now_ms();
-            fprintf(level_log, "h %d mode %d S %d Q %d n %d level_us %.1f chain_us %.1f cyc %llu passes %llu slow %llu xcc %d ncopy %d multi %d "
+            fprintf(level_log, "h %d mode %d S %d Q %d n %d level_us %.1f chain_us %.1f cyc %llu passes %llu slow %llu xcc %d ncopy %d copyn %d multi %d done %d "
                     "ph %.1f %.1f %.1f %.1f %.1f host_us %.1f wait_us %.1f pend_us %.1f batch %d\n", job.handle, mode, S, Q,
                     n_sweeps, Rh->level_wall * 0.01, chain ? Rh->chain_wall * 0.01 : 0.0, chain ? (unsigned long long)Rh->chain_cycles : 0ull,
-                    chain ? (unsigned long long)Rh->n_pass : 0ull, chain ? (unsigned long long)Rh->n_slow : 0ull, Rh->xcc, H.n_copy, (int)any_multi,
+                    chain ? (unsigned long long)Rh->n_pass : 0ull, chain ? (unsigned long long)Rh->n_slow : 0ull, Rh->xcc, H.n_copy, H.copy_n, (int)any_multi, w.level_done,
                     Rh->phase_ticks[0] * 0.01, Rh->phase_ticks[1] * 0.01, Rh->phase_ticks[2] * 0.01, Rh->phase_ticks[3] * 0.01, Rh->phase_ticks[4] * 0.01,
                     1e3 * (t_launched - t_last_done), 1e3 * (t_done - t_launched), 1e3 * (w.t_batch_launched - t_launched), w.batch_n);
             t_last_done = t_done;
```
